# richarddurbin/modimizer

Measured on AMD Instinct MI355X. Metric: Gbp/s hashed+sketched (k=21,d=64), higher is better.
Workload: dtype u64; 1 GPU; BASELINE config 2: 10 Gbp synthetic ONT-like reads (log-normal N50 20 kb, 5% subs, 30x of a 333 Mbp genome), k=21 d=64 seed=17, seqhash scan + modset build (table bits 30); reads_per_gpu=598835, bases_per_gpu=10000000000, modimizers_per_gpu=156043826, modset_entries=102967436, k=21, d=64, table_bits=30, parallelism=reads sharded x1, modset per GPU

## Files before the change

### include/modgpu.h

```cpp
#ifndef MODGPU_H
#define MODGPU_H

#include <stdio.h>
#include <stdint.h>
#include <stdbool.h>
#include <stddef.h>

#if defined (MODGPU_WITH_REFERENCE_HEADERS) || defined (MS_MINOR)
#ifdef __cplusplus
extern "C" {
#endif
void mgSeqhashDestroy (Seqhash *sh) ;
void mgSeqhashRCiteratorDestroy (SeqhashRCiterator *si) ;
#ifdef __cplusplus
}
#endif
#else
#include "modgpu_compat.h"
#endif

#ifdef __cplusplus
extern "C" {
#endif


typedef enum {
  MG_OK = 0,
  MG_ERR_NO_DEVICE = 1,
  MG_ERR_HIP = 2,
  MG_ERR_ARG = 3,
  MG_ERR_CAPACITY = 4,
  MG_ERR_NOMEM = 5
} MgStatus ;

const char *mgLastError (void) ;
int  mgDeviceCount (void) ;
MgStatus mgSetDevice (int device) ;
const char *mgVersion (void) ;
const char *mgSourceHash (void) ;

U64 *mgIterScanHost (const Seqhash *sh, const char *s, int len) ;
void mgReloadKnobs (void) ;
int  mgIterHostBelow (int below) ;

MgStatus mgDeviceAlloc (void **dptr, size_t bytes) ;
MgStatus mgDeviceFree (void *dptr) ;
MgStatus mgMemcpyH2D (void *dst, const void *src, size_t bytes, void *stream) ;
MgStatus mgMemcpyD2H (void *dst, const void *src, size_t bytes, void *stream) ;
MgStatus mgMemsetD (void *dst, int byte, size_t bytes, void *stream) ;
MgStatus mgStreamSynchronize (void *stream) ;
MgStatus mgCopyD2HBig (void *hostDst, const void *devSrc, size_t bytes) ;
MgStatus mgCopyH2DBig (void *devDst, const void *hostSrc, size_t bytes) ;

#define MG_PACK_PAD 8
size_t   mgPackedWords (U64 nBases) ;
void     mgPackHost (const char *bases, U64 nBases, U32 *words) ;
MgStatus mgPackDevice (const U8 *dBases, U64 nBases, U32 *dWords, void *stream) ;
MgStatus mgUnpackDevice (const U32 *dWords, U64 nBases, U8 *dBases, void *stream) ;
MgStatus mgUploadPack (const char *bases, U64 nBases, U32 *dPacked, void *stream) ;

#define MG_POS_MASK 0x7fffffffu
#define MG_FWD_BIT  0x80000000u
size_t   mgScanWorkBytes (U64 totalBases, U32 nReads, U64 capacity) ;
MgStatus seqhashScanBatchDevice (const Seqhash *sh, const U32 *dPacked, U64 totalBases,
                                 const U64 *dReadOffsets, U32 nReads,
                                 U64 *dKmer, U32 *dPosF, U32 *dReadId, U64 capacity,
                                 U64 *dCount, void *dWork, void *stream) ;

int64_t seqhashScanBatch (const Seqhash *sh, const char *bases, const int64_t *readOffsets, int nReads,
                          U64 **kmer, int **pos, bool **isF, int64_t **survStart) ;

MgStatus seqhashMinimizerBatchDevice (const Seqhash *sh, const U32 *dPacked, U64 totalBases,
                                      const U64 *dReadOffsets, U32 nReads,
                                      U64 *dHash, U32 *dPosF, U64 *dReadStart, U64 capacity, U64 *n, void *stream) ;
int64_t seqhashMinimizerBatch (const Seqhash *sh, const char *bases, const int64_t *readOffsets, int nReads,
                               U64 **hash, int **pos, bool **isF, int64_t **start) ;

MgStatus modsetAddBatchDevice (Modset *ms, const U64 *dKmer, U64 n, U32 *dIndexOut, int withDepth, void *stream) ;
MgStatus modsetFindBatchDevice (Modset *ms, const U64 *dKmer, U64 n, U32 *dIndexOut, void *stream) ;

MgStatus modsetSyncToHost (Modset *ms, int wantIndex) ;
int      mgXferThreadCount (void) ;
MgStatus mgModsetDeviceRelease (Modset *ms) ;
void     mgModsetHostChanged (Modset *ms) ;
MgStatus mgModsetClear (Modset *ms, void *stream) ;

U64 mgModsetDeviceSlots (Modset *ms) ;

MgStatus mgTableCheckLayout (Modset *ms, U64 *out6) ;
MgStatus mgTableDiag (Modset *ms, U64 *out9) ;

MgStatus modsetDepthHistogramDevice (Modset *ms, U64 *dHist65536, void *stream) ;

MgStatus mgAddReadsDevice (Modset *ms, const U32 *dPacked, U64 totalBases,
                           const U64 *dReadOffsets, U32 nReads, U64 *nHash, void *stream) ;
MgStatus mgQueryReadsDevice (Modset *ms, const U32 *dPacked, U64 totalBases,
                             const U64 *dReadOffsets, U32 nReads,
                             U32 *dSeedIndex, U32 *dSeedPosF, U32 *dSeedRead, U64 capacity,
                             U64 *nSeeds, void *stream) ;

MgStatus mgQueryReadsDeviceAsync (Modset *ms, const U32 *dPacked, U64 totalBases, const U64 *dReadOffsets, U32 nReads,
                                  U32 *dSeedIndex, U32 *dSeedPosF, U32 *dSeedRead, U64 capacity, void **ticket, void *stream) ;
MgStatus mgQueryReadsDeviceWait (void *ticket, U64 *nSeeds, void *stream) ;

MgStatus mgInsertReadsDevice (Modset *ms, const U32 *dPacked, U64 totalBases,
                              const U64 *dReadOffsets, U32 nReads,
                              U32 *dSeedIndex, U32 *dSeedPosF, U32 *dSeedRead, U64 capacity,
                              U64 *nSeeds, void *stream) ;

bool mgModsetMergeArrays (Modset *ms1, U64 *value2, U16 *depth2, U8 *info2, U32 n2) ;
bool mgModsetMergeDeviceArrays (Modset *ms1, const U64 *dValue2, const U16 *dDepth2, const U8 *dInfo2, U32 n2) ;

typedef struct MgComm MgComm ;
MgStatus mgCommInitAll (MgComm **comms , int nDev, const int *devices ) ;
MgStatus mgCommGetUniqueId (void *id128) ;
MgStatus mgCommInitRank (MgComm **comm, int nRanks, int rank, const void *id128, int device) ;
int      mgCommRank (const MgComm *c) ;
int      mgCommSize (const MgComm *c) ;
void     mgCommDestroy (MgComm *c) ;
MgStatus mgHistogramAllReduce (Modset *ms, U64 *hist65536, MgComm *c) ;
MgStatus mgDepthAllReduce (Modset *ms, MgComm *c) ;
MgStatus mgModsetMergeRankOrder (Modset *ms, MgComm *c, int root) ;

int64_t mgAddSequenceBatch (Modset *ms, const char *bases, const int64_t *readOffsets, int nReads) ;
void    mgDepthHistogram (Modset *ms, FILE *f) ;
int     mgAddSequences (Modset *ms, const char *bases, const int64_t *readOffsets, int nReads, FILE *out) ;
void    mgModsetWriteText (Modset *ms, FILE *f) ;

typedef struct {
  Modset *ms ;
  U32 size ;
  U32 max ;
  U32 *index, *offset, *id ;
  U32 *depth ;
  U32 *rev, *loc ;
  int nSeq ;
  char **names ;
  U32 *len ;
} MgReference ;
MgReference *mgReferenceCreate (Modset *ms, U32 size) ;
void mgReferenceDestroy (MgReference *ref) ;
int  mgReferenceRead (MgReference *ref, const char *bases, const int64_t *offsets, int nSeq,
                      const char **names, bool isAdd, FILE *out) ;
void mgReferenceWrite (MgReference *ref, const char *root) ;
FILE *mgGzipOpenWrite (const char *name) ;
FILE *mgGzipOpenRead (const char *name) ;
FILE *mgFzOpen (const char *name, const char *mode) ;
MgReference *mgReferenceLoad (const char *root) ;
int  mgQueryProcess (MgReference *ref, const char *bases, const int64_t *offsets, int nReads,
                     const char **names, FILE *out) ;
void mgSetVerbose (int on) ;

typedef struct {
  Modset *ms ;
  int nReads, capReads ;
  int *len, *nHit, *nMiss ;
  int (*nCopy)[4] ;
  U64 *hitStart ;
  U32 *hit ; U16 *dx ;
  U64 totHit, capHit ;
  U64 *invStart ;
  U32 *invSpace ;
} MgReadset ;
MgReadset *mgReadsetCreate (Modset *ms) ;
void mgReadsetDestroy (MgReadset *rs) ;
int  mgReadsetRead (MgReadset *rs, const char *bases, const int64_t *offsets, int nReads) ;
int  mgReadsetFileRead (MgReadset *rs, const char *filename) ;
void mgReadsetStats (MgReadset *rs, FILE *out) ;
void mgReadsetWrite (MgReadset *rs, const char *root) ;
MgReadset *mgReadsetLoad (const char *root) ;
int  mgReadsetCleanMods (MgReadset *rs, FILE *out) ;
int  mgReadsetCleanModsPath (void) ;
int  mgReadsetProperties (MgReadset *rs, FILE *out) ;
int  mgReadsetPropertiesPath (void) ;

typedef struct {
  Modset *ms ;
  int len ;
  int *pos ;
  bool *isF ;
  int ownsMs ;
} MgRepRef ;
MgRepRef *mgRepRefCreate (const char *seqFile, const char *modFile, FILE *err) ;
MgRepRef *mgRepRefFromArrays (Modset *ms, const char *bases, int64_t len, FILE *err) ;
void mgRepRefDestroy (MgRepRef *ref) ;

typedef struct MgRepRun MgRepRun ;
typedef struct {
  int nRead, nBad, nGood ;
  int *n, *seqF, *seqR ;
  bool *bad, *isF ;
  U32 max ;
  int *modN, *modNPre ;
  int *goodI, *goodLen ;
  U64 *hitStart ;
  int *hitK, *hitX ;
  int nMod, nDup, tDup, minMax ;
} MgRepResult ;
void mgRepResultFree (MgRepResult *res) ;
MgRepRun *mgRepRunBegin (MgRepRef *ref, Modset *ms) ;
int  mgRepRunAdd (MgRepRun *run, const char *bases, const int64_t *offsets, int nReads, FILE *out) ;
int  mgRepRunFinish (MgRepRun *run, FILE *err, MgRepResult *res) ;
int  mgRepAnalyze3File (MgRepRef *ref, const char *seqFile, const char *modFile, FILE *out, FILE *err, MgRepResult *res) ;
int  mgRepPath (void) ;

typedef struct MgSeqReader MgSeqReader ;
typedef struct { char *bases ; int64_t *offsets ; char **names ; int nSeq ; int64_t total ; int isFastq ; int64_t basesCap ; } MgSeqBatch ;
MgSeqReader *mgSeqOpen (const char *filename) ;
int  mgSeqNextBatch (MgSeqReader *r, int64_t maxBases, MgSeqBatch *out) ;
void mgSeqBatchFree (MgSeqBatch *b) ;
void mgSeqClose (MgSeqReader *r) ;
void mgSeqReleaseBuffers (void) ;
void mgReleaseBuffers (void) ;
int  mgTextParseFileDevice (const char *filename, char **bases, int64_t **offsets, int64_t *nSeq) ;
int  mgAddSequenceFile (Modset *ms, const char *filename, FILE *out) ;
int  mgReferenceFastaRead (MgReference *ref, const char *filename, bool isAdd, FILE *out) ;
int  mgQueryFile (MgReference *ref, const char *filename, FILE *out) ;
int  mgReportDepths (Modset *ms, Modset **others, int nOthers, FILE *f) ;
int  mgRefPaint (Modset *ms, const char *bases, const int64_t *offsets, int nSeq, const char **names, FILE *out) ;
int  mgRefPaintFile (Modset *ms, const char *filename, FILE *out) ;
int     mgModsetWriteTextDevice (Modset *ms, FILE *f) ;
Modset *mgModsetReadText (const char *filename) ;
int     mgModsetReadTextPath (void) ;
int  mgFormatF2 (char *buf64, double x) ;

MgStatus mgSynthGenome (U32 *dPacked, U64 nBases, U64 seed, void *stream) ;
MgStatus mgSynthReads (const U32 *dGenomePacked, U64 genomeBases,
                       const U64 *dReadStart, const U64 *dReadOffsets, const U8 *dStrand, U32 nReads,
                       U64 totalBases, double errRate, U64 seed, U32 *dPackedOut, void *stream) ;

void     mgProfileEnable (int on) ;
void     mgProfileOnly (int kernelId) ;
void     mgProfileReset (void) ;
int      mgProfileKernels (void) ;
MgStatus mgProfileGet (int id, const char **name, double *totalMs, U64 *launches) ;

#ifdef __cplusplus
}
#endif
#endif
```

### modimizer_amd/__init__.py

```python
import contextlib
import ctypes as C
import os
import subprocess

import numpy as np

_HERE = os.path.dirname(os.path.abspath(__file__))
LIB_PATH = os.environ.get("MODGPU_LIB") or os.path.join(_HERE, "libmodgpu.so")
CSRC = os.path.join(_HERE, "csrc")

U64P = C.POINTER(C.c_uint64)
U32P = C.POINTER(C.c_uint32)

MG_POS_MASK = 0x7FFFFFFF
MG_FWD_BIT = 0x80000000


class Seqhash(C.Structure):
    _fields_ = [("seed", C.c_int), ("k", C.c_int), ("w", C.c_int), ("mask", C.c_uint64),
                ("shift1", C.c_int), ("shift2", C.c_int), ("factor1", C.c_uint64),
                ("factor2", C.c_uint64), ("patternRC", C.c_uint64 * 4)]


class SeqhashRCiterator(C.Structure):
    _fields_ = [("sh", C.POINTER(Seqhash)), ("s", C.c_void_p), ("sEnd", C.c_void_p),
                ("h", C.c_uint64), ("hRC", C.c_uint64), ("hashBuf", C.c_void_p), ("fBuf", C.c_void_p),
                ("base", C.c_int), ("iStart", C.c_int), ("iMin", C.c_int), ("isDone", C.c_bool)]


class Modset(C.Structure):
    _fields_ = [("hasher", C.POINTER(Seqhash)), ("tableBits", C.c_int), ("size", C.c_uint32),
                ("tableSize", C.c_uint64), ("tableMask", C.c_uint64), ("index", U32P),
                ("value", U64P), ("depth", C.POINTER(C.c_uint16)), ("info", C.POINTER(C.c_uint8)),
                ("max", C.c_uint32)]


class MgReference(C.Structure):
    _fields_ = [("ms", C.POINTER(Modset)), ("size", C.c_uint32), ("max", C.c_uint32),
                ("index", U32P), ("offset", U32P), ("id", U32P), ("depth", U32P), ("rev", U32P), ("loc", U32P),
                ("nSeq", C.c_int), ("names", C.POINTER(C.c_char_p)), ("len", U32P)]


class MgReadset(C.Structure):
    _fields_ = [("ms", C.POINTER(Modset)), ("nReads", C.c_int), ("capReads", C.c_int),
                ("len", C.POINTER(C.c_int)), ("nHit", C.POINTER(C.c_int)), ("nMiss", C.POINTER(C.c_int)),
                ("nCopy", C.POINTER(C.c_int * 4)), ("hitStart", U64P), ("hit", U32P), ("dx", C.POINTER(C.c_uint16)),
                ("totHit", C.c_uint64), ("capHit", C.c_uint64), ("invStart", U64P), ("invSpace", U32P)]


class MgRepRef(C.Structure):
    _fields_ = [("ms", C.POINTER(Modset)), ("len", C.c_int), ("pos", C.POINTER(C.c_int)), ("isF", C.POINTER(C.c_bool)), ("ownsMs", C.c_int)]


class MgRepResult(C.Structure):
    _fields_ = [("nRead", C.c_int), ("nBad", C.c_int), ("nGood", C.c_int),
                ("n", C.POINTER(C.c_int)), ("seqF", C.POINTER(C.c_int)), ("seqR", C.POINTER(C.c_int)),
                ("bad", C.POINTER(C.c_bool)), ("isF", C.POINTER(C.c_bool)), ("max", C.c_uint32),
                ("modN", C.POINTER(C.c_int)), ("modNPre", C.POINTER(C.c_int)),
                ("goodI", C.POINTER(C.c_int)), ("goodLen", C.POINTER(C.c_int)), ("hitStart", U64P),
                ("hitK", C.POINTER(C.c_int)), ("hitX", C.POINTER(C.c_int)),
                ("nMod", C.c_int), ("nDup", C.c_int), ("tDup", C.c_int), ("minMax", C.c_int)]


class MgSeqBatch(C.Structure):
    _fields_ = [("bases", C.POINTER(C.c_int8)), ("offsets", C.POINTER(C.c_int64)), ("names", C.POINTER(C.c_char_p)),
                ("nSeq", C.c_int), ("total", C.c_int64), ("isFastq", C.c_int), ("basesCap", C.c_int64)]


EXPORTS = [
    "seqhashCreate", "seqhashWrite", "seqhashRead", "seqhashReport", "modRCiterator", "modRCnext",
    "minimizerRCiterator", "minimizerRCnext", "seqString", "mgSeqhashDestroy", "mgSeqhashRCiteratorDestroy",
    "modsetCreate", "modsetDestroy", "modsetWrite", "modsetRead", "modsetIndexFind", "modsetSummary",
    "modsetPack", "modsetDepthPrune", "modsetMerge",
    "mgLastError", "mgDeviceCount", "mgSetDevice", "mgVersion", "mgSourceHash", "mgDeviceAlloc", "mgDeviceFree",
    "mgMemcpyH2D", "mgMemcpyD2H", "mgMemsetD", "mgStreamSynchronize",
    "mgPackedWords", "mgPackHost", "mgPackDevice", "mgUnpackDevice", "mgUploadPack",
    "mgScanWorkBytes", "seqhashScanBatchDevice", "seqhashScanBatch", "seqhashMinimizerBatchDevice", "seqhashMinimizerBatch",
    "modsetAddBatchDevice", "modsetFindBatchDevice", "modsetSyncToHost", "mgXferThreadCount", "mgCopyD2HBig", "mgCopyH2DBig", "mgModsetDeviceRelease",
    "mgModsetHostChanged", "modsetDepthHistogramDevice", "mgTableCheckLayout", "mgTableDiag", "mgAddReadsDevice", "mgQueryReadsDevice", "mgQueryReadsDeviceAsync", "mgQueryReadsDeviceWait",
    "mgAddSequenceBatch", "mgDepthHistogram", "mgSynthGenome", "mgSynthReads",
    "mgInsertReadsDevice", "mgAddSequences", "mgModsetWriteText", "mgReferenceCreate", "mgReferenceDestroy",
    "mgReferenceRead", "mgQueryProcess", "mgReferenceWrite", "mgGzipOpenWrite", "mgFzOpen", "mgGzipOpenRead", "mgReferenceLoad",
    "mgCommInitAll", "mgCommGetUniqueId", "mgCommInitRank", "mgCommRank", "mgCommSize", "mgCommDestroy", "mgHistogramAllReduce", "mgDepthAllReduce", "mgModsetMergeRankOrder",
    "mgReadsetCreate", "mgReadsetDestroy", "mgReadsetRead", "mgReadsetFileRead", "mgReadsetStats", "mgReadsetWrite", "mgReadsetLoad",
    "mgReadsetCleanMods", "mgReadsetCleanModsPath", "mgReadsetProperties", "mgReadsetPropertiesPath",
    "mgRepRefCreate", "mgRepRefFromArrays", "mgRepRefDestroy", "mgRepRunBegin", "mgRepRunAdd", "mgRepRunFinish", "mgRepResultFree", "mgRepAnalyze3File", "mgRepPath",
    "mgSeqOpen", "mgSeqNextBatch", "mgSeqBatchFree", "mgSeqClose", "mgSeqReleaseBuffers", "mgReleaseBuffers", "mgTextParseFileDevice", "mgAddSequenceFile", "mgReferenceFastaRead", "mgQueryFile",
    "mgReportDepths", "mgRefPaint", "mgRefPaintFile", "mgModsetWriteTextDevice", "mgModsetReadText", "mgModsetReadTextPath",
    "mgIterScanHost", "mgIterHostBelow", "mgReloadKnobs", "mgFormatF2", "mgModsetMergeArrays", "mgModsetMergeDeviceArrays", "mgModsetClear", "mgModsetDeviceSlots", "mgSetVerbose", "mgProfileEnable", "mgProfileOnly", "mgProfileReset", "mgProfileKernels", "mgProfileGet",
]


@contextlib.contextmanager
def knobs(**kv):
    old = {}
    for k, v in kv.items():
        name = "MODGPU_" + k
        old[name] = os.environ.get(name)
        if v is None:
            os.environ.pop(name, None)
        else:
            os.environ[name] = str(v)
    lib().mgReloadKnobs()
    try:
        yield
    finally:
        for name, v in old.items():
            if v is None:
                os.environ.pop(name, None)
            else:
                os.environ[name] = v
        lib().mgReloadKnobs()


def source_hash():
    import hashlib
    names = sorted(f for f in os.listdir(CSRC) if f.endswith((".hip", ".c", ".h"))) + ["Makefile", "../../include/modgpu.h", "../../include/modgpu_compat.h"]
    inc = os.path.join(_HERE, "..", "include")
    path = lambda n: os.path.join(inc, os.path.basename(n)) if n.startswith("../") else os.path.join(CSRC, n)
    listing = "".join("%s  %s\n" % (hashlib.sha256(open(path(n), "rb").read()).hexdigest(), n) for n in names)
    return hashlib.sha256(listing.encode()).hexdigest()[:16]


def binary_hash(path=None):
    import re
    try:
        m = re.search(rb"MODGPU_SRC_HASH=([0-9a-f]{16})", open(path or LIB_PATH, "rb").read())
    except OSError:
        return None
    return m.group(1).decode() if m else None


def build(force=False):
    import fcntl
    if os.environ.get("MODGPU_LIB"):
        return LIB_PATH
    def make_if_stale():
        if force or binary_hash() != source_hash():
            subprocess.check_call(["make", "-C", CSRC, "-j8", "-s"] + (["-B"] if force else []))
            if binary_hash() != source_hash():
                raise RuntimeError("libmodgpu.so does not carry the hash of its sources after make: %s != %s" % (binary_hash(), source_hash()))
    try:
        lk = open(os.path.join(CSRC, ".build.lock"), "w")
    except OSError:
        make_if_stale()
        return LIB_PATH
    with lk:
        fcntl.flock(lk, fcntl.LOCK_EX)
        make_if_stale()
    return LIB_PATH


_lib = None


def lib():
    global _lib
    if _lib is not None:
        return _lib
    if os.environ.get("MODGPU_NO_TORCH", "0") != "1":
        try:
            import torch
        except Exception:
            pass
    build()
    L = C.CDLL(LIB_PATH, mode=C.RTLD_GLOBAL)
    if not os.environ.get("MODGPU_LIB"):
        L.mgSourceHash.restype = C.c_char_p
        if L.mgSourceHash().decode() != source_hash():
            raise RuntimeError("the loaded libmodgpu.so was not built from the sources in this tree")
    vp, u64, u32, i32, i64 = C.c_void_p, C.c_uint64, C.c_uint32, C.c_int, C.c_int64
    SH, MS, IT = C.POINTER(Seqhash), C.POINTER(Modset), C.POINTER(SeqhashRCiterator)

    def sig(name, res, *args):
        if os.environ.get("MODGPU_LIB") and not hasattr(L, name):
            return
        f = getattr(L, name); f.restype = res; f.argtypes = list(args)
    sig("seqhashCreate", SH, i32, i32, i32)
    sig("seqhashWrite", None, SH, vp); sig("seqhashRead", SH, vp); sig("seqhashReport", None, SH, vp)
    sig("modRCiterator", IT, SH, vp, i32)
    sig("modRCnext", C.c_bool, IT, U64P, C.POINTER(i32), C.POINTER(C.c_bool))
    sig("minimizerRCiterator", IT, SH, vp, i32)
    sig("mgIterScanHost", vp, SH, vp, i32); sig("mgIterHostBelow", i32, i32); sig("mgReloadKnobs", None)
    sig("mgFormatF2", i32, C.c_char_p, C.c_double)
    sig("minimizerRCnext", C.c_bool, IT, U64P, C.POINTER(i32), C.POINTER(C.c_bool))
    sig("seqString", C.c_char_p, u64, i32)
    sig("mgSeqhashDestroy", None, SH); sig("mgSeqhashRCiteratorDestroy", None, IT)
    sig("modsetCreate", MS, SH, i32, u32); sig("modsetDestroy", None, MS)
    sig("modsetWrite", None, MS, vp); sig("modsetRead", MS, vp)
    sig("modsetIndexFind", u32, MS, u64, i32); sig("modsetSummary", None, MS, vp)
    sig("modsetPack", C.c_bool, MS); sig("modsetDepthPrune", None, MS, i32, i32)
    sig("modsetMerge", C.c_bool, MS, MS)
    sig("mgLastError", C.c_char_p); sig("mgDeviceCount", i32); sig("mgSetDevice", i32, i32)
    sig("mgVersion", C.c_char_p)
    sig("mgSourceHash", C.c_char_p)
    sig("mgDeviceAlloc", i32, C.POINTER(vp), C.c_size_t); sig("mgDeviceFree", i32, vp)
    sig("mgMemcpyH2D", i32, vp, vp, C.c_size_t, vp); sig("mgMemcpyD2H", i32, vp, vp, C.c_size_t, vp)
    sig("mgMemsetD", i32, vp, i32, C.c_size_t, vp); sig("mgStreamSynchronize", i32, vp)
    sig("mgPackedWords", C.c_size_t, u64); sig("mgPackHost", None, vp, u64, vp)
    sig("mgUploadPack", i32, vp, u64, vp, vp); sig("mgPackDevice", i32, vp, u64, vp, vp); sig("mgUnpackDevice", i32, vp, u64, vp, vp)
    sig("mgScanWorkBytes", C.c_size_t, u64, u32, u64)
    sig("seqhashScanBatchDevice", i32, SH, vp, u64, vp, u32, vp, vp, vp, u64, vp, vp, vp)
    sig("seqhashScanBatch", i64, SH, vp, vp, i32, C.POINTER(vp), C.POINTER(vp), C.POINTER(vp), C.POINTER(vp))
    sig("seqhashMinimizerBatchDevice", i32, SH, vp, u64, vp, u32, vp, vp, vp, u64, U64P, vp)
    sig("seqhashMinimizerBatch", i64, SH, vp, vp, i32, C.POINTER(vp), C.POINTER(vp), C.POINTER(vp), C.POINTER(vp))
    sig("modsetAddBatchDevice", i32, MS, vp, u64, vp, i32, vp)
    sig("modsetFindBatchDevice", i32, MS, vp, u64, vp, vp)
    sig("modsetSyncToHost", i32, MS, i32); sig("mgXferThreadCount", i32); sig("mgCopyD2HBig", i32, vp, vp, C.c_size_t); sig("mgCopyH2DBig", i32, vp, vp, C.c_size_t); sig("mgModsetDeviceRelease", i32, MS)
    sig("mgModsetHostChanged", None, MS)
    sig("modsetDepthHistogramDevice", i32, MS, vp, vp); sig("mgTableCheckLayout", i32, MS, U64P); sig("mgTableDiag", i32, MS, U64P)
    sig("mgAddReadsDevice", i32, MS, vp, u64, vp, u32, U64P, vp)
    sig("mgQueryReadsDevice", i32, MS, vp, u64, vp, u32, vp, vp, vp, u64, U64P, vp)
    sig("mgQueryReadsDeviceAsync", i32, MS, vp, u64, vp, u32, vp, vp, vp, u64, C.POINTER(vp), vp); sig("mgQueryReadsDeviceWait", i32, vp, U64P, vp)
    sig("mgAddSequenceBatch", i64, MS, vp, vp, i32); sig("mgDepthHistogram", None, MS, vp)
    sig("mgSynthGenome", i32, vp, u64, u64, vp)
    sig("mgSynthReads", i32, vp, u64, vp, vp, vp, u32, u64, C.c_double, u64, vp, vp)
    sig("mgInsertReadsDevice", i32, MS, vp, u64, vp, u32, vp, vp, vp, u64, U64P, vp)
    sig("mgAddSequences", i32, MS, vp, vp, i32, vp); sig("mgModsetWriteText", None, MS, vp)
    sig("mgReferenceCreate", vp, MS, u32); sig("mgReferenceDestroy", None, vp)
    sig("mgReferenceRead", i32, vp, vp, vp, i32, C.POINTER(C.c_char_p), C.c_bool, vp)
    sig("mgQueryProcess", i32, vp, vp, vp, i32, C.POINTER(C.c_char_p), vp)
    RS = C.POINTER(MgReadset)
    sig("mgReadsetCreate", RS, MS); sig("mgReadsetDestroy", None, RS)
    sig("mgReadsetRead", i32, RS, vp, vp, i32); sig("mgReadsetFileRead", i32, RS, C.c_char_p)
    sig("mgReadsetStats", None, RS, vp); sig("mgReadsetWrite", None, RS, C.c_char_p); sig("mgReadsetLoad", RS, C.c_char_p)
    sig("mgReadsetCleanMods", i32, RS, vp); sig("mgReadsetCleanModsPath", i32); sig("mgReadsetProperties", i32, RS, vp); sig("mgReadsetPropertiesPath", i32)
    RR, RES = C.POINTER(MgRepRef), C.POINTER(MgRepResult)
    sig("mgRepRefCreate", RR, C.c_char_p, C.c_char_p, vp); sig("mgRepRefFromArrays", RR, MS, vp, i64, vp); sig("mgRepRefDestroy", None, RR)
    sig("mgRepRunBegin", vp, RR, MS); sig("mgRepRunAdd", i32, vp, vp, vp, i32, vp); sig("mgRepRunFinish", i32, vp, vp, RES); sig("mgRepResultFree", None, RES)
    sig("mgRepAnalyze3File", i32, RR, C.c_char_p, C.c_char_p, vp, vp, RES); sig("mgRepPath", i32)
    sig("mgSeqOpen", vp, C.c_char_p); sig("mgSeqNextBatch", i32, vp, C.c_int64, C.POINTER(MgSeqBatch))
    sig("mgSeqBatchFree", None, C.POINTER(MgSeqBatch)); sig("mgSeqClose", None, vp); sig("mgSeqReleaseBuffers", None); sig("mgReleaseBuffers", None)
    sig("mgTextParseFileDevice", i32, C.c_char_p, C.POINTER(vp), C.POINTER(vp), C.POINTER(i64))
    sig("mgAddSequenceFile", i32, MS, C.c_char_p, vp); sig("mgReferenceFastaRead", i32, vp, C.c_char_p, C.c_bool, vp)
    sig("mgQueryFile", i32, vp, C.c_char_p, vp)
    sig("mgReportDepths", i32, MS, C.POINTER(MS), i32, vp)
    sig("mgRefPaint", i32, MS, vp, vp, i32, C.POINTER(C.c_char_p), vp); sig("mgRefPaintFile", i32, MS, C.c_char_p, vp)
    sig("mgModsetWriteTextDevice", i32, MS, vp); sig("mgModsetReadText", MS, C.c_char_p); sig("mgModsetReadTextPath", i32)
    sig("mgReferenceWrite", None, vp, C.c_char_p); sig("mgGzipOpenWrite", vp, C.c_char_p); sig("mgGzipOpenRead", vp, C.c_char_p); sig("mgFzOpen", vp, C.c_char_p, C.c_char_p);
    sig("mgCommInitAll", i32, C.POINTER(vp), i32, C.POINTER(i32)); sig("mgCommGetUniqueId", i32, vp); sig("mgCommInitRank", i32, C.POINTER(vp), i32, i32, vp, i32)
    sig("mgCommRank", i32, vp); sig("mgCommSize", i32, vp); sig("mgCommDestroy", None, vp)
    sig("mgHistogramAllReduce", i32, MS, vp, vp); sig("mgDepthAllReduce", i32, MS, vp); sig("mgModsetMergeRankOrder", i32, MS, vp, i32)
    sig("mgReferenceLoad", C.POINTER(MgReference), C.c_char_p)
    sig("mgModsetMergeArrays", C.c_bool, MS, vp, vp, vp, u32)
    sig("mgModsetMergeDeviceArrays", C.c_bool, MS, vp, vp, vp, u32)
    sig("mgModsetClear", i32, MS, vp); sig("mgModsetDeviceSlots", u64, MS); sig("mgSetVerbose", None, i32)
    sig("mgProfileEnable", None, i32); sig("mgProfileOnly", None, i32); sig("mgProfileReset", None); sig("mgProfileKernels", i32)
    sig("mgProfileGet", i32, i32, C.POINTER(C.c_char_p), C.POINTER(C.c_double), U64P)
    _lib = L
    return L


class ModgpuError(RuntimeError):
    pass


def check(status):
    if status != 0:
        raise ModgpuError("libmodgpu status %d: %s" % (status, lib().mgLastError().decode()))


_libc = C.CDLL(None)
_libc.free.argtypes = [C.c_void_p]
_libc.fopen.restype = C.c_void_p
_libc.fopen.argtypes = [C.c_char_p, C.c_char_p]
_libc.fclose.argtypes = [C.c_void_p]


class CFile:

    def __init__(self, path, mode="w"):
        self.f = _libc.fopen(path.encode(), mode.encode())
        if not self.f:
            raise OSError("cannot open " + path)

    def __enter__(self):
        return C.c_void_p(self.f)

    def __exit__(self, *a):
        _libc.fclose(self.f)



def seqhashCreate(k, w, seed=17):
    if k < 1 or k >= 32:
        raise ValueError("seqhash k %d must be between 1 and 32" % k)
    if w < 1:
        raise ValueError("seqhash w %d must be positive" % w)
    return lib().seqhashCreate(k, w, seed)


def modsetCreate(sh, bits, size=0):
    if bits < 20 or bits > 34:
        raise ValueError("table bits %d must be between 20 and 34" % bits)
    if size >= (1 << bits) >> 2:
        raise ValueError("Modset size %u is too big for %d bits" % (size, bits))
    return lib().modsetCreate(sh, bits, size)


def iterate(sh, bases, minimizer=False):
    L = lib()
    bases = np.ascontiguousarray(bases, dtype=np.uint8)
    mk, nx = (L.minimizerRCiterator, L.minimizerRCnext) if minimizer else (L.modRCiterator, L.modRCnext)
    it = mk(sh, bases.ctypes.data, len(bases))
    u = C.c_uint64(); p = C.c_int(); f = C.c_bool()
    ks, ps, fs = [], [], []
    while nx(it, C.byref(u), C.byref(p), C.byref(f)):
        ks.append(u.value); ps.append(p.value); fs.append(int(f.value))
    L.mgSeqhashRCiteratorDestroy(it)
    return np.array(ks, np.uint64), np.array(ps, np.int32), np.array(fs, np.uint8)


def scan_batch(sh, bases, offsets):
    L = lib()
    bases = np.ascontiguousarray(bases, dtype=np.uint8)
    offsets = np.ascontiguousarray(offsets, dtype=np.int64)
    n_reads = len(offsets) - 1
    pk, pp, pf, ps = C.c_void_p(), C.c_void_p(), C.c_void_p(), C.c_void_p()
    n = L.seqhashScanBatch(sh, bases.ctypes.data, offsets.ctypes.data, n_reads,
                           C.byref(pk), C.byref(pp), C.byref(pf), C.byref(ps))
    if n < 0:
        raise ModgpuError("seqhashScanBatch failed: " + L.mgLastError().decode())

    def take(ptr, ctype, count, dtype):
        a = np.ctypeslib.as_array(C.cast(ptr, C.POINTER(ctype)), (max(count, 1),))[:count].astype(dtype, copy=True)
        _libc.free(ptr)
        return a
    kmer = take(pk, C.c_uint64, n, np.uint64)
    pos = take(pp, C.c_int, n, np.int32)
    isf = take(pf, C.c_bool, n, np.uint8)
    st = take(ps, C.c_int64, n_reads + 1, np.int64)
    return kmer, pos, isf, st


def minimizer_batch(sh, bases, offsets):
    L = lib()
    bases = np.ascontiguousarray(bases, dtype=np.uint8)
    offsets = np.ascontiguousarray(offsets, dtype=np.int64)
    n_reads = len(offsets) - 1
    pk, pp, pf, ps = C.c_void_p(), C.c_void_p(), C.c_void_p(), C.c_void_p()
    n = L.seqhashMinimizerBatch(sh, bases.ctypes.data, offsets.ctypes.data, n_reads,
                                C.byref(pk), C.byref(pp), C.byref(pf), C.byref(ps))
    if n < 0:
        raise ModgpuError("seqhashMinimizerBatch failed: " + L.mgLastError().decode())

    def take(ptr, ctype, count, dtype):
        a = np.ctypeslib.as_array(C.cast(ptr, C.POINTER(ctype)), (max(count, 1),))[:count].astype(dtype, copy=True)
        _libc.free(ptr)
        return a
    return (take(pk, C.c_uint64, n, np.uint64), take(pp, C.c_int, n, np.int32), take(pf, C.c_bool, n, np.uint8),
            take(ps, C.c_int64, n_reads + 1, np.int64))


class DeviceBuffer:

    def __init__(self, nbytes):
        self.ptr = C.c_void_p()
        self.nbytes = int(nbytes)
        check(lib().mgDeviceAlloc(C.byref(self.ptr), self.nbytes))

    @classmethod
    def from_numpy(cls, arr):
        arr = np.ascontiguousarray(arr)
# ... 173 lines not shown
```

### modimizer_amd/csrc/mg_api.hip

```cpp
#include <stdarg.h>
#include <stdlib.h>
#include <string.h>
#include <mutex>
#include <unordered_map>
#include "mg_common.h"
#include "mg_internal.h"
#include "mg_xfer.h"


static thread_local char gErr[512] = "";

void mgSetError (const char *fmt, ...)
{ va_list ap; va_start (ap, fmt); vsnprintf (gErr, sizeof (gErr), fmt, ap); va_end (ap); }

extern "C" const char *mgLastError (void) { return gErr; }

MgStatus mgHipFail (hipError_t e, const char *what)
{ mgSetError ("HIP error %d (%s) in %s", (int) e, hipGetErrorString (e), what); return MG_ERR_HIP; }

extern "C" int mgDeviceCount (void)
{ int n = 0; if (hipGetDeviceCount (&n) != hipSuccess) { (void) hipGetLastError (); return 0; } return n; }

MgStatus mgEnsureDevice (void)
{
// ... 703 lines not shown
static MgStatus mgAddChunk (Modset *ms, MgDev *d, const U64 *dKmer, U64 n, U32 *dIndexOut, int withDepth,
                            void *scratch, hipStream_t st, const MgHistReq *counted = 0, const MgSegSrc *segSrc = 0)
{
  MgTable &t = d->t;
  MgStatus s;
  MG_HIP (hipMemsetAsync (t.counters, 0, 16, st));
  if ((s = mgTableAdd (&t, dKmer, n, withDepth, scratch, st, counted, segSrc))) return s;
  volatile U64 *c = d->hPin;
  MG_HIP (hipMemcpyAsync (d->hPin, t.counters, 16, hipMemcpyDeviceToHost, st));
  MG_HIP (hipStreamSynchronize (st));
  U64 newMax = (U64) t.max + c[0];
  if (c[1] || newMax >= t.size)
    {
      if ((s = mgTableRollback (&t, st))) return s;
      mgSetError ("hashTableSize %u is too small for %llu", t.size, (unsigned long long) newMax);
      return MG_ERR_CAPACITY;
    }
  t.max = (U32) newMax;
  ms->max = t.max;
  if (n >= 4096) t.newPct = (int) (c[0] * 100 / n);
  if (dIndexOut && (s = mgTableFind (&t, dKmer, n, dIndexOut, st))) return s;
  return MG_OK;
}

static MgStatus mgAddBatch (Modset *ms, MgDev *d, const U64 *dKmer, U64 n, U32 *dIndexOut, int withDepth,
                            bool arenaLive, hipStream_t st, const MgHistReq *counted, const MgSegSrc *segSrc)
{
  if (!n) return MG_OK;
  if (d->ticketsOut) { mgSetError ("a query batch of this modset is in flight (mgQueryReadsDeviceAsync without its mgQueryReadsDeviceWait)"); return MG_ERR_ARG; }
  U64 chunk = n < MG_ADD_CHUNK ? n : MG_ADD_CHUNK;
  MgStatus s = mgTableEnsure (&d->t, chunk, st); if (s) return s;
  size_t need = mgTableAddScratchBytes (&d->t, chunk) + 4096;
  if (!arenaLive)
    { if ((s = d->arena.reserve (need))) return s;
      d->arena.reset ();
    }
  else if (d->arena.bytes - d->arena.used < need)
    { mgSetError ("internal: arena too small for insert temporaries"); return MG_ERR_NOMEM; }
  void *scratch = d->arena.take (mgTableAddScratchBytes (&d->t, chunk));
  for (U64 off = 0 ; off < n && !s ; off += chunk)
    { U64 m = n - off < chunk ? n - off : chunk;
      if (off) s = mgTableEnsure (&d->t, m, st);
      if (!s) s = mgAddChunk (ms, d, dKmer + off, m, dIndexOut ? dIndexOut + off : 0, withDepth, scratch, st,
                              (counted && n <= chunk) ? counted : 0,
                              n <= chunk ? segSrc : 0);
    }
  return s;
}

extern "C" MgStatus modsetAddBatchDevice (Modset *ms, const U64 *dKmer, U64 n, U32 *dIndexOut, int withDepth, void *stream)
{
  hipStream_t st = (hipStream_t) stream;
  MgDev *d; MgStatus s = mgDevGet (ms, &d, st); if (s) return s;
  return mgAddBatch (ms, d, dKmer, n, dIndexOut, withDepth, false, st);
}

extern "C" MgStatus modsetFindBatchDevice (Modset *ms, const U64 *dKmer, U64 n, U32 *dIndexOut, void *stream)
{
  hipStream_t st = (hipStream_t) stream;
  MgDev *d; MgStatus s = mgDevGet (ms, &d, st); if (s) return s;
  d->t.loadPct = MG_LOOKUP_LOAD_PCT;
  if (d->t.slots && (s = mgTableEnsure (&d->t, 0, st))) return s;
  return mgTableFind (&d->t, dKmer, n, dIndexOut, st);
}

extern "C" MgStatus modsetSyncToHost (Modset *ms, int wantIndex)
{
  MgDev *d = mgDevLookup (ms);
  if (!d) return MG_OK;
  MgOnDevice here (d->device);
  MgTable &t = d->t;
  hipStream_t st = 0;
  MgStatus s;
  MG_HIP (hipDeviceSynchronize ());
  if (d->ticketsOut && (t.pendingDepth || (wantIndex && d->hostIndexMax < t.max)))
    { mgSetError ("a query batch of this modset is in flight (its scratch is what a sync would use)"); return MG_ERR_ARG; }
  if (t.max > t.syncedMax)
    { const U32 first = t.syncedMax + 1;
      if ((s = mgXferD2H (ms->value + first, t.value + first, (size_t) (t.max - first + 1) * sizeof (U64), MG_XFER_COPY))) return s;
      t.syncedMax = t.max;
    }
  ms->max = t.max;
  if (t.max && t.pendingDepth)
    {
      if ((s = d->arena.reserve (mgAl256 ((size_t) t.max * sizeof (U16)) + 4096))) return s;
      d->arena.reset ();
      U16 *dDelta = (U16 *) d->arena.take ((size_t) t.max * sizeof (U16));
      if ((s = mgTableExportDepth (&t, dDelta, st))) return s;
      MG_HIP (hipStreamSynchronize (st));
      if ((s = mgXferD2H (ms->depth + 1, dDelta, (size_t) t.max * sizeof (U16), MG_XFER_SATADD16))) return s;
    }
  if (wantIndex && d->hostIndexMax < t.max)
    { if ((s = d->arena.reserve (mgAl256 (ms->tableSize * sizeof (U32)) + 4096))) return s;
      d->arena.reset ();
      U32 *dIndex = (U32 *) d->arena.take (ms->tableSize * sizeof (U32));
      if ((s = mgTableReplayIndex (&t, mgMakeParams (ms->hasher), ms->tableBits, dIndex, st))) return s;
      MG_HIP (hipStreamSynchronize (st));
      if ((s = mgXferD2H (ms->index, dIndex, ms->tableSize * sizeof (U32), MG_XFER_COPY))) return s;
      d->hostIndexMax = t.max;
    }
  return MG_OK;
}

extern "C" MgStatus mgModsetAdoptDepthDevice (Modset *ms, const U16 *dDepth16)
{
  MgDev *d = mgDevLookup (ms);
  if (!d || !d->built) return MG_OK;
  MgTable &t = d->t;
  if (t.pendingDepth || t.max != ms->max) { mgModsetHostChanged (ms); return MG_OK; }
  MG_HIP (hipMemcpy (t.baseDepth, dDepth16, ((size_t) t.max + 1) * sizeof (U16), hipMemcpyDeviceToDevice));
  t.baseZero = false; t.liveHistValid = false;
  return MG_OK;
}

extern "C" int mgHookDeviceView (Modset *ms, const U64 **dValue1, const U16 **dDepth1, U32 *max)
{
  MgDev *d = mgDevLookup (ms);
  if (!d || !d->built || d->ticketsOut) return -1;
  { int cur = -1; if (hipGetDevice (&cur) != hipSuccess || cur != d->device) return -1; }
  if (hipDeviceSynchronize () != hipSuccess || mgFoldCounts (d, 0, ms)) return -1;
  *dValue1 = d->t.value + 1; *dDepth1 = d->t.baseDepth + 1; *max = d->t.max;
  return 0;
}

extern "C" int mgHookDeviceViewMake (Modset *ms, const U64 **dValue1, const U16 **dDepth1, U32 *max)
{
  MgDev *d; if (mgDevGet (ms, &d, 0)) return -1;
  return mgHookDeviceView (ms, dValue1, dDepth1, max);
}

extern "C" U64 mgModsetDeviceSlots (Modset *ms) { MgDev *d = mgDevLookup (ms); return d && d->built ? d->t.nSlots : 0; }

extern "C" MgStatus mgTableCheckLayout (Modset *ms, U64 *out6)
{
  MgDev *d; MgStatus s = mgDevGet (ms, &d, 0); if (s) return s;
  MgDevScratch scratch ("mgTableCheckLayout");
  U64 *dOut;
  if (scratch.get (&dOut, 4)) return MG_ERR_HIP;
  s = mgTableLayoutCheck (&d->t, dOut, 0);
  if (!s && (hipMemcpy (out6, dOut, 32, hipMemcpyDeviceToHost) || hipMemcpy (out6 + 4, d->t.counters + 4, 16, hipMemcpyDeviceToHost))) s = MG_ERR_HIP;
  return s;
}

extern "C" MgStatus mgTableDiag (Modset *ms, U64 *out9)
{
  memset (out9, 0, 9 * sizeof (U64));
  MgDev *d = mgDevLookup (ms);
  if (!d || !d->built) return MG_OK;
  out9[0] = (U64) d->t.log2NB; out9[1] = d->t.R;
  for (int i = 0 ; i < 7 ; ++i) out9[2 + i] = d->t.diag[i];
  return MG_OK;
}

extern "C" MgStatus modsetDepthHistogramDevice (Modset *ms, U64 *dHist, void *stream)
{
  hipStream_t st = (hipStream_t) stream;
  MgDev *d; MgStatus s = mgDevGet (ms, &d, st); if (s) return s;
  return mgTableHistogram (&d->t, dHist, st);
}


struct MgScanBufs { U64 *kmer; U32 *posF; U32 *rid; void *work; U64 *count; U64 cap; MgHistReq counted;
                    MgSegSrc seg; bool lazy; void *findScratch, *findScratch2; };

struct MgScanReq { const Seqhash *sh; const U32 *dPacked; U64 totalBases; const U64 *dReadOffsets; U32 nReads; bool wantPos; size_t extraPerSurvivor;
                   U32 *outPosF, *outRid; U64 outCap; bool lazy; };
static inline MgArena &mgArenaOf (MgDev *d, int slot) { return slot ? d->arena2 : d->arena; }
static inline U64 *mgCountPin (MgDev *d, int slot) { return d->hPin + 8 + 8 * slot; }

static MgStatus mgScanStart (MgDev *d, int slot, const MgScanReq &q, U64 cap, MgScanBufs *b, hipStream_t st)
{
  b->lazy = false; b->seg.nSegs = 0; b->seg.segKmer = 0; b->findScratch = 0; b->findScratch2 = 0;
  MgArena &ar = mgArenaOf (d, slot);
  const long fp = mgKnobs ()->findPath;
  const bool lookupHist = q.lazy && q.wantPos && !q.extraPerSurvivor && d->t.slots && fp != 'd'
                          && (fp == 'p' || fp == '2' || (cap >= ((U64) 1 << 24) && d->t.nSlots >= ((U64) 1 << 24) && d->t.log2NB > 9));
  const bool lookup2 = lookupHist && fp != 'p';
  MgHashParams p = mgMakeParams (q.sh);
  const size_t perS = 8 + (q.wantPos ? 8 : 0) + q.extraPerSurvivor;
  const size_t need = mgAl256 (cap * perS) + 4 * 4096 + 512 * MG_HIST_STRIDE * 4 + mgAl256 (mgScanWorkBytes (q.totalBases, q.nReads, cap))
                      + (q.extraPerSurvivor ? mgTableAddScratchBytes (&d->t, cap < MG_ADD_CHUNK ? cap : MG_ADD_CHUNK) + 8192 : 0) + 8 * 256
                      + (lookupHist ? mgTableFindPartScratchBytes (cap) + 8192 : 0) + (lookup2 ? mgTableFindPart2ScratchBytes (cap) + 8192 : 0);
  MgStatus s = ar.reserve (need); if (s) return s;
  ar.reset ();
  b->cap = cap;
  b->kmer = (U64 *) ar.take (cap * 8);
  const bool direct = q.wantPos && q.outPosF && q.outRid && q.outCap >= cap;
  b->posF = !q.wantPos ? 0 : (direct ? q.outPosF : (U32 *) ar.take (cap * 4));
  b->rid = !q.wantPos ? 0 : (direct ? q.outRid : (U32 *) ar.take (cap * 4));
  b->work = ar.take (mgScanWorkBytes (q.totalBases, q.nReads, cap));
  b->count = (U64 *) ar.take (8 * MG_COUNT_WORDS);
  b->counted.log2NB = 0; b->counted.kbits = 64; b->counted.binCount = 0; b->counted.hiB = 0;
  if (q.extraPerSurvivor || lookupHist)
    { b->counted.binCount = (U32 *) ar.take (512 * MG_HIST_STRIDE * sizeof (U32));
      b->counted.log2NB = d->t.log2NB; b->counted.kbits = d->t.kbits;
      if (lookupHist) b->counted.hiB = mgTableFindDigitBits (&d->t);
    }
  b->findScratch = lookupHist ? ar.take (mgTableFindPartScratchBytes (cap)) : 0;
  b->findScratch2 = lookup2 ? ar.take (mgTableFindPart2ScratchBytes (cap)) : 0;
  const bool lz = q.lazy && (q.wantPos ? q.extraPerSurvivor == 0 : b->counted.binCount != 0);
  if ((s = mgLaunchScan (p, q.dPacked, q.totalBases, q.dReadOffsets, q.nReads, b->kmer, b->posF, b->rid, cap, b->count, b->work, st,
                         b->counted.binCount ? &b->counted : 0, lz ? &b->seg : 0))) return s;
  b->lazy = lz;
  MG_HIP (hipMemcpyAsync (mgCountPin (d, slot), b->count, MG_COUNT_WORDS * sizeof (U64), hipMemcpyDeviceToHost, st));
  return MG_OK;
}
static MgStatus mgScanFinish (MgDev *d, int slot, const MgScanBufs *b, U64 *nOut, U64 *retryCap, hipStream_t st, hipEvent_t done = 0)
{
  volatile U64 *c = mgCountPin (d, slot);
  if (done) MG_HIP (hipEventSynchronize (done));
  else MG_HIP (hipStreamSynchronize (st));
  *retryCap = 0;
  if (!c[1] && c[0] <= b->cap) { *nOut = c[0]; return MG_OK; }
  *nOut = c[0]; *retryCap = c[3];
  return MG_OK;
}

static MgStatus mgScanIntoArena (MgDev *d, const Seqhash *sh, const U32 *dPacked, U64 totalBases,
                                 const U64 *dReadOffsets, U32 nReads, bool wantPos, size_t extraPerSurvivor,
                                 MgScanBufs *b, U64 *nOut, hipStream_t st,
                                 U32 *outPosF = 0, U32 *outRid = 0, U64 outCap = 0, bool lazy = false)
{
  if (d->ticketsOut) { mgSetError ("a query batch of this modset is in flight (mgQueryReadsDeviceAsync without its mgQueryReadsDeviceWait)"); return MG_ERR_ARG; }
  MgScanReq q = { sh, dPacked, totalBases, dReadOffsets, nReads, wantPos, extraPerSurvivor, outPosF, outRid, outCap, lazy };
  U64 cap = mgSurvivorGuess (sh, totalBases);
  if (extraPerSurvivor)
    {
      U64 expect = totalBases / (U64) (sh->w > 0 ? sh->w : 1) + 1;
      if (expect > MG_ADD_CHUNK) expect = MG_ADD_CHUNK;
      MgStatus es = mgTableEnsure (&d->t, expect, st); if (es) return es;
    }
  for (int attempt = 0 ; attempt < 3 ; ++attempt)
    { MgStatus s = mgScanStart (d, 0, q, cap, b, st); if (s) return s;
      U64 retry = 0;
      if ((s = mgScanFinish (d, 0, b, nOut, &retry, st))) return s;
      if (!retry) return MG_OK;
      cap = retry;
    }
  mgSetError ("scan capacity could not be established");
  return MG_ERR_CAPACITY;
}

extern "C" MgStatus mgAddReadsDevice (Modset *ms, const U32 *dPacked, U64 totalBases,
                                      const U64 *dReadOffsets, U32 nReads, U64 *nHash, void *stream)
{
  hipStream_t st = (hipStream_t) stream;
  MgDev *d; MgStatus s = mgDevGet (ms, &d, st); if (s) return s;
  if (nHash) *nHash = 0;
  if (!totalBases || !nReads) return MG_OK;
  MgScanBufs b; U64 n = 0;
  d->t.loadPct = 75;
  if ((s = mgScanIntoArena (d, ms->hasher, dPacked, totalBases, dReadOffsets, nReads, false, 4, &b, &n, st, 0, 0, 0, true))) return s;
  if (nHash) *nHash = n;
  if (!n) return MG_OK;
  if (b.lazy)
    { const U64 chunk = n < MG_ADD_CHUNK ? n : MG_ADD_CHUNK;
      if ((s = mgTableEnsure (&d->t, chunk, st))) return s;
      if (n <= MG_ADD_CHUNK && mgTableAddTakesSegments (&d->t, n, &b.counted))
        return mgAddBatch (ms, d, 0, n, 0, 1, true, st, &b.counted, &b.seg);
      if ((s = mgLaunchSegCompact (b.seg, b.kmer, b.cap, b.count, st))) return s;
    }
  return mgAddBatch (ms, d, b.kmer, n, 0, 1, true, st, &b.counted);
}

static MgStatus mgSeedReads (Modset *ms, const Seqhash *scanWith, int mode, const U32 *dPacked, U64 totalBases,
                             const U64 *dReadOffsets, U32 nReads,
                             U32 *dSeedIndex, U32 *dSeedPosF, U32 *dSeedRead, U64 capacity,
                             U64 *nSeeds, hipStream_t st)
{
  MgDev *d; MgStatus s = mgDevGet (ms, &d, st); if (s) return s;
  if (nSeeds) *nSeeds = 0;
  if (!scanWith) scanWith = ms->hasher;
  if ((s = mgCheckHasher (scanWith))) return s;
  if (scanWith->k != ms->hasher->k) { mgSetError ("a batch scanned with k %d cannot be looked up in a set of k %d", scanWith->k, ms->hasher->k); return MG_ERR_ARG; }
  if (!totalBases || !nReads) return MG_OK;
  MgScanBufs b; U64 n = 0;
  d->t.loadPct = MG_LOOKUP_LOAD_PCT;
  if (mode == 0 && d->t.slots && (s = mgTableEnsure (&d->t, 0, st))) return s;
  const int timing = mgKnobs ()->seedTiming == 1;
  struct timespec q0, q1, q2; if (timing) clock_gettime (CLOCK_MONOTONIC, &q0);
  if ((s = mgScanIntoArena (d, scanWith, dPacked, totalBases, dReadOffsets, nReads, true, mode ? 4 : 0, &b, &n, st,
                            dSeedPosF, dSeedRead, capacity, mode == 0))) return s;
  if (timing) clock_gettime (CLOCK_MONOTONIC, &q1);
  if (nSeeds) *nSeeds = n;
  if (n > capacity)
    { mgSetError ("%llu seeds exceed the caller's capacity %llu", (unsigned long long) n, (unsigned long long) capacity); return MG_ERR_CAPACITY; }
  if (mode == 0)
    { if (b.lazy && b.findScratch && mgTableFindTakesPartition (&d->t, n, &b.counted))
        s = mgTableFindPartitioned (&d->t, b.seg, n, &b.counted, dSeedIndex, b.kmer, b.findScratch, st, b.findScratch2);
      else s = b.lazy ? mgTableFindSegments (&d->t, b.seg, n, dSeedIndex, st) : mgTableFind (&d->t, b.kmer, n, dSeedIndex, st);
    }
  else s = mgAddBatch (ms, d, b.kmer, n, dSeedIndex, 0, true, st, &b.counted);
  if (s) return s;
  if (dSeedPosF && b.posF != dSeedPosF) MG_HIP (hipMemcpyAsync (dSeedPosF, b.posF, n * 4, hipMemcpyDeviceToDevice, st));
  if (dSeedRead && b.rid != dSeedRead) MG_HIP (hipMemcpyAsync (dSeedRead, b.rid, n * 4, hipMemcpyDeviceToDevice, st));
  MG_HIP (hipStreamSynchronize (st));
  if (timing)
    { clock_gettime (CLOCK_MONOTONIC, &q2);
      fprintf (stderr, "mgSeedReads: scan+count %.2f ms, lookup+sync %.2f ms\n", (q1.tv_sec - q0.tv_sec) * 1e3 + (q1.tv_nsec - q0.tv_nsec) * 1e-6,
               (q2.tv_sec - q1.tv_sec) * 1e3 + (q2.tv_nsec - q1.tv_nsec) * 1e-6);
    }
  return MG_OK;
}

extern "C" MgStatus mgQueryReadsDevice (Modset *ms, const U32 *dPacked, U64 totalBases,
                                        const U64 *dReadOffsets, U32 nReads,
// ... 349 lines not shown
```

### modimizer_amd/csrc/mg_common.h

```cpp
#ifndef MG_COMMON_H
#define MG_COMMON_H
#include "mg_knobs.h"

#include <hip/hip_runtime.h>
#include <stdint.h>
#include <time.h>
#include <algorithm>
#include <vector>
#include "modgpu.h"

#define MG_WAVE 64

#define MG_SCAN_THREADS   256
#define MG_POS_PER_THREAD 64
#define MG_TILE_BASES     (64 * MG_POS_PER_THREAD)
#define MG_TILE_WORDS     (MG_TILE_BASES / 16)

struct MgHashParams {
  U64 factor1;
  U64 mask;
  int k;
  int shift1;
  U32 d;
  int dShift;
// ... 45 lines not shown
  { if (cap >= want) return MG_OK;
    drop ();
    const hipError_t e = hipMalloc ((void **) &p, alloc * sizeof (T)); if (e != hipSuccess) { p = 0; return mgHipFail (e, what); }
    cap = alloc; return MG_OK;
  }
  void drop () { if (p) (void) hipFree (p); p = 0; cap = 0; }
};

#ifdef __HIPCC__
__device__ __forceinline__ bool mgDivisible (U64 x, const MgHashParams &p)
{
  if (x & (((U64) 1 << p.dShift) - 1)) return false;
  return ((x >> p.dShift) * p.dOddInv) <= p.dOddLim;
}

__device__ __forceinline__ bool mgDivisibleOdd32 (U64 h, const MgHashParams &p)
{
  const U32 lo = (U32) h, hi = (U32) (h >> 32);
  const U32 a = __builtin_amdgcn_alignbit (hi, lo, 24);
  const U32 t = __umul24 (a, p.c24) + (lo & 0xffffffu);
  return t * p.inv32 <= p.lim32;
}

__device__ __forceinline__ U32 mgRevComp16 (U32 w)
{
  const U32 x = __brev (w);
  return __builtin_amdgcn_bitop3_b32 (x << 1, x >> 1, 0x55555555u, 0x27);
}

__device__ __forceinline__ U64 mgRevComp (U64 f, int shift1)
{
  const U64 x = ((U64) mgRevComp16 ((U32) f) << 32) | mgRevComp16 ((U32) (f >> 32));
  return x >> shift1;
}
struct MgGeom { U32 R; int log2NB; int kbits; };
__device__ __forceinline__ U64 mgMixBits (U64 x, int b)
{
  if (b <= 32)
    { U32 y = (U32) x;
      const U32 m32 = b >= 32 ? ~0u : (((U32) 1 << b) - 1);
      const int h32 = (b + 1) >> 1;
      y ^= y >> h32; y = (y * 0xed558ccdu) & m32;
      y ^= y >> h32; y = (y * 0x1a85ec53u) & m32;
      y ^= y >> h32;
      return y;
    }
  const U64 mask = b >= 64 ? ~0ull : (((U64) 1 << b) - 1);
  const int h = (b + 1) >> 1;
  x ^= x >> h; x = (x * 0xff51afd7ed558ccdull) & mask;
  x ^= x >> h; x = (x * 0xc4ceb9fe1a85ec53ull) & mask;
  x ^= x >> h;
  return x;
}
#define MG_MIX_TOP 10
#define MG_MIX_MUL 0x9E3779B1u
__device__ __forceinline__ U64 mgMixK (U64 x, int b)
{
  if (b < 24) return mgMixBits (x, b);
  const int lb = b - MG_MIX_TOP;
  const U64 L = x & (((U64) 1 << lb) - 1), A = x >> lb;
  const U32 low = lb >= 32 ? (U32) L : ((U32) L & (((U32) 1 << lb) - 1));
  const U32 g = (low * MG_MIX_MUL) >> (32 - MG_MIX_TOP);
  return ((A ^ (U64) g) << lb) | mgMixBits (L, lb);
}
__device__ __forceinline__ U32 mgMixTopOfKmer (U64 x, int b, int hiB)
{
  const int lb = b - MG_MIX_TOP;
  const U32 low = lb >= 32 ? (U32) x : ((U32) x & (((U32) 1 << lb) - 1));
  return (U32) (x >> (b - hiB)) ^ ((low * MG_MIX_MUL) >> (32 - hiB));
}
__device__ __forceinline__ U32 mgBucketOfM (U64 m, const MgGeom &g)
{
  if (!g.log2NB) return 0u;
  const int s = g.kbits - g.log2NB;
  return s >= 0 ? (U32) (m >> s) : ((U32) m << (-s));
}
__device__ __forceinline__ U32 mgHomeOfM (U64 m, const MgGeom &g)
{
  U32 x = (U32) m;
  if (g.kbits >= 24) x ^= (U32) (m >> (g.kbits - MG_MIX_TOP)) * 0x9E5u;
  return __umulhi (x * 0x85EBCA6Bu, g.R);
}
__device__ __forceinline__ U32 mgNextSlot (U32 at, U32 R) { return at + 1 == R ? 0u : at + 1; }
#endif

static inline unsigned mgGrid (U64 n, unsigned per = 256, unsigned cap = 4096)
{ U64 b = (n + per - 1) / per; if (b > cap) b = cap; if (b < 1) b = 1; return (unsigned) b; }
static inline size_t mgAl256 (size_t n) { return (n + 255) & ~(size_t) 255; }
static inline double mgNowS (void) { struct timespec ts; clock_gettime (CLOCK_MONOTONIC, &ts); return ts.tv_sec + 1e-9 * ts.tv_nsec; }

static inline void mgPartSplit (int log2NB, int *hiB, int *loB)
{ if (log2NB <= 9) { *hiB = log2NB; *loB = 0; } else { *loB = log2NB / 2; *hiB = log2NB - *loB; } }

#define MG_HIST_STRIDE 16
struct MgHistReq { int log2NB; int kbits; U32 *binCount; int hiB; };

struct MgSegSrc { const U64 *segKmer; const U64 *segCount; const U64 *segStart; U64 segCap; U32 nSegs; };


MgStatus mgLaunchPack (const U8 *dBases, U64 nBases, U32 *dWords, hipStream_t st);
MgStatus mgLaunchUnpack (const U32 *dWords, U64 nBases, U8 *dBases, hipStream_t st);
MgStatus mgLaunchScan (const MgHashParams &p, const U32 *dPacked, U64 totalBases,
                       const U64 *dReadOffsets, U32 nReads,
                       U64 *dKmer, U32 *dPosF, U32 *dReadId, U64 capacity,
                       U64 *dCount, void *dWork, hipStream_t st, const MgHistReq *hist = 0, MgSegSrc *lazy = 0);

U64      mgScanTiles (U64 totalBases);
size_t   mgScanInfoBytes (U64 totalBases);
MgStatus mgScanPrepare (const U64 *dReadOffsets, U32 nReads, U64 totalBases, void *dInfo, hipStream_t st);
size_t   mgScanRangeWorkBytes (U64 nTilesRange, U64 capacity);
MgStatus mgLaunchSegCompact (const MgSegSrc &src, U64 *dKmer, U64 capacity, const U64 *dCount, hipStream_t st);
MgStatus mgLaunchScanRange (const MgHashParams &p, const U32 *dPacked, U64 totalBases,
                            const U64 *dReadOffsets, U32 nReads, const void *dInfo, U64 tile0, U64 tile1,
                            U64 *dKmer, U32 *dPosF, U32 *dReadId, U64 capacity,
                            U64 *dCount, void *dWork, hipStream_t st, const MgHistReq *hist = 0, MgSegSrc *lazy = 0);

U64      mgIterMaxBases (void);
U64      mgIterSegEntries (void);
MgStatus mgLaunchIterScan (const MgHashParams &p, const U32 *dPacked, U64 totalBases, const U64 *dReadOff,
                           U64 *dSegKmer, U32 *dSegPosF, U64 *out, U64 capEntries, U64 *flag, U64 seq, hipStream_t st);

MgStatus mgLaunchMinimizers (const MgHashParams &p, U32 w, const U32 *dPacked, const U64 *dReadOffsets, U32 nReads,
                             U64 *dHash, U32 *dPosF, U64 *dReadStart, U64 capacity, U64 *totalOut, hipStream_t st);

struct MgSlot { U64 key; U32 ord; U32 cnt; };
struct MgTable {
  MgSlot *slots; U64 nSlots;
  U64 capSlots;
  U32 capNB;
  U32 R; int log2NB;
  int kbits;
  U32 *occ;
  U64 *value;
  U16 *baseDepth;
  bool baseZero;
  U64 *liveHist;
  bool liveHistValid;
  U32 size;
  U32 max;
  U32 syncedMax;
  U64 *counters;
  bool pendingDepth;
  bool dirty;
  U64 *find8;
  U64 find8Cap;
  U64 find8Version, version;
  bool empty;
  U64 *pin;
  int newPct;
  int loadPct;
  int  maxLog2Slots;
  U32  wantR;
  U64  diag[7];
  int  tightPct;
};
MgStatus mgTableAlloc (MgTable *t, U64 slotsWanted, hipStream_t st);
MgStatus mgTableEnsure (MgTable *t, U64 nIncoming, hipStream_t st);
MgStatus mgTableRollback (MgTable *t, hipStream_t st);
MgStatus mgTableClean (MgTable *t, hipStream_t st);
void     mgTableForget (MgTable *t, hipStream_t st);
size_t   mgTableAddScratchBytes (const MgTable *t, U64 n);
bool     mgTableUseBuckets (const MgTable *t, U64 n);
MgStatus mgTableAdd (MgTable *t, const U64 *dKmer, U64 n, int withDepth, void *scratch, hipStream_t st,
                     const MgHistReq *counted = 0,
                     const MgSegSrc *segSrc = 0);
bool     mgTableAddTakesSegments (const MgTable *t, U64 n, const MgHistReq *counted);
MgStatus mgTableMarkOccupied (MgTable *t, const U64 *dKmer, U64 n, hipStream_t st);
MgStatus mgTableFind (MgTable *t, const U64 *dKmer, U64 n, U32 *dIndexOut, hipStream_t st);
MgStatus mgTableLayoutCheck (MgTable *t, U64 *dOut4, hipStream_t st);
enum { MG_DIAG_FIND_DIRECT = 0, MG_DIAG_FIND_PART1, MG_DIAG_FIND_PART2_16, MG_DIAG_FIND_PART2_8, MG_DIAG_PACK8, MG_DIAG_REHASH_BUCKET, MG_DIAG_REHASH_ATOMIC };
size_t   mgTableFindPartScratchBytes (U64 n);
int      mgTableFindDigitBits (const MgTable *t);
bool     mgTableFindTakesPartition (const MgTable *t, U64 n, const MgHistReq *counted);
size_t   mgTableFindPart2ScratchBytes (U64 n);
MgStatus mgTableFindPartitioned (MgTable *t, const MgSegSrc &segSrc, U64 n, const MgHistReq *counted, U32 *dIndexOut, U64 *el, void *scratch, hipStream_t st,
                                 void *scratch2 = 0);
MgStatus mgTableFindSegments (MgTable *t, const MgSegSrc &src, U64 n, U32 *dIndexOut, hipStream_t st);
MgStatus mgTableLoadHost (MgTable *t, const U64 *dValue, U32 first, U32 last, hipStream_t st);
MgStatus mgTableExportDepth (MgTable *t, U16 *dDelta, hipStream_t st);
MgStatus mgTableHistogram (MgTable *t, U64 *dHist, hipStream_t st);
MgStatus mgTableReplayIndex (MgTable *t, const MgHashParams &p, int tableBits, U32 *dIndex, hipStream_t st);
MgStatus mgTableMergeApply (const U32 *dIdx, const U16 *dDepth2, const U8 *dInfo2, U32 n2, U16 *dBaseDepth, U8 *dInfo1, hipStream_t st);
size_t   mgTablePruneScratchBytes (U32 n);
MgStatus mgTablePrune (MgTable *t, const U8 *dInfo, int lo, int hi, U64 *dNewValue, U16 *dNewDepth, U8 *dNewInfo,
                       void *scratch, hipStream_t st);
#define MG_COUNT_WORDS 4

MgStatus mgLaunchSynthGenome (U32 *dPacked, U64 nBases, U64 seed, hipStream_t st);
MgStatus mgLaunchSynthReads (const U32 *dGenome, U64 genomeBases, const U64 *dReadStart,
                             const U64 *dReadOffsets, const U8 *dStrand, U32 nReads, U64 totalBases,
                             double errRate, U64 seed, U32 *dOut, hipStream_t st);

#endif
```

### modimizer_amd/csrc/mg_knobs.c

```c
#define _GNU_SOURCE
#include <pthread.h>
#include <sched.h>
#include <stdio.h>
#include <stdlib.h>
#include <string.h>
#include <unistd.h>
#include <sys/mman.h>
#include "mg_knobs.h"

static MgKnobs gKnobs;
static pthread_once_t gOnce = PTHREAD_ONCE_INIT;

static long num (const char *name)
{ const char *e = getenv (name); return e && *e ? atol (e) : MG_KNOB_UNSET; }

static void readAll (void)
{
  MgKnobs k;
  const char *e = getenv ("MODGPU_TABLE_PATH");
  k.tablePath = e && *e ? (long) e[0] : MG_KNOB_UNSET;
  e = getenv ("MODGPU_FIND_PATH");
  k.findPath = e && *e ? (long) e[0] : MG_KNOB_UNSET;
  k.partPacked = num ("MODGPU_PART_PACKED");       k.partBig = num ("MODGPU_PART_BIG");
  k.addChunk = num ("MODGPU_ADD_CHUNK");           k.scanGrid = num ("MODGPU_SCAN_GRID");
  k.scanGeneric = num ("MODGPU_SCAN_GENERIC");     k.scanHist = num ("MODGPU_SCAN_HIST");
  k.scanDiv64 = num ("MODGPU_SCAN_DIV64");        k.minTiled = num ("MODGPU_MIN_TILED");
  k.minTile = num ("MODGPU_MIN_TILE");
  k.noSegmentInput = num ("MODGPU_NO_SEGMENT_INPUT");
  k.rankSliceShift = num ("MODGPU_RANK_SLICE_SHIFT");
  k.flagPolarity = num ("MODGPU_FLAG_POLARITY");   k.mergeSlots = num ("MODGPU_MERGE_SLOTS");
  k.mergePlace = num ("MODGPU_MERGE_PLACE");
  k.bucketR = num ("MODGPU_BUCKET_R");             k.bucketT = num ("MODGPU_BUCKET_T");
  e = getenv ("MODGPU_HOT_SPLIT");
  k.hotSplit = e && *e ? atol (e) : MG_KNOB_UNSET;
  { const char *c = e ? strchr (e, ',') : 0; k.hotChunk = c ? atol (c + 1) : MG_KNOB_UNSET; }
  k.noAvx2 = num ("MODGPU_NO_AVX2");               k.textHost = num ("MODGPU_TEXT_HOST");
  k.textWindowKb = num ("MODGPU_TEXT_WINDOW_KB");
  k.fileBatchMbp = num ("MODGPU_FILE_BATCH_MBP");  k.fileBatchBases = num ("MODGPU_FILE_BATCH_BASES");
  k.queryHostChain = num ("MODGPU_QUERY_HOST_CHAIN");
  k.iterHostBelow = num ("MODGPU_ITER_HOST_BELOW");
  k.readsetHost = num ("MODGPU_READSET_HOST");
  k.segSlack = num ("MODGPU_SEG_SLACK");
  k.partDigits = num ("MODGPU_PART_DIGITS");
  k.findBits = num ("MODGPU_FIND_BITS");
  k.scatterGrid = num ("MODGPU_SCATTER_GRID");     k.tableLoad = num ("MODGPU_TABLE_LOAD");
  k.tightLoad = num ("MODGPU_TIGHT_LOAD");         k.find8 = num ("MODGPU_FIND8");
  k.packThreads = num ("MODGPU_PACK_THREADS");     k.parseThreads = num ("MODGPU_PARSE_THREADS");
  k.xferThreads = num ("MODGPU_XFER_THREADS");       k.gzipThreads = num ("MODGPU_GZIP_THREADS");
  k.xferPieceKb = num ("MODGPU_XFER_PIECE_KB");      k.xferStreams = num ("MODGPU_XFER_STREAMS");
  k.seedTiming = num ("MODGPU_SEED_TIMING");       k.uploadTiming = num ("MODGPU_UPLOAD_TIMING");
  k.textTiming = num ("MODGPU_TEXT_TIMING");       k.parseTiming = getenv ("MODGPU_PARSE_TIMING") ? 1 : MG_KNOB_UNSET;
  k.scanDebug = num ("MODGPU_SCAN_DEBUG");         k.bucketDebug = num ("MODGPU_BUCKET_DEBUG");
  gKnobs = k;
}

const MgKnobs *mgKnobs (void) { pthread_once (&gOnce, readAll); return &gKnobs; }
void mgIterKnobsReloaded (void) __attribute__ ((weak));
void mgReloadKnobs (void) { pthread_once (&gOnce, readAll); readAll (); if (mgIterKnobsReloaded) mgIterKnobsReloaded (); }

static int gCpuBudget;
static pthread_once_t gCpuOnce = PTHREAD_ONCE_INIT;
static void cpuBudgetOnce (void)
{
  long v = sysconf (_SC_NPROCESSORS_ONLN);
  cpu_set_t set;
  if (sched_getaffinity (0, sizeof (set), &set) == 0 && CPU_COUNT (&set) < v) v = CPU_COUNT (&set);
  FILE *q = fopen ("/sys/fs/cgroup/cpu.max", "r");
  if (q)
    { char a[64]; long per = 0;
      if (fscanf (q, "%63s %ld", a, &per) == 2 && strcmp (a, "max") && per > 0) { const long c = (atol (a) + per - 1) / per; if (c < v) v = c; }
      fclose (q);
    }
  gCpuBudget = v < 1 ? 1 : (int) v;
}
int mgCpuBudget (void) { pthread_once (&gCpuOnce, cpuBudgetOnce); return gCpuBudget; }

void mgHugeHint (void *p, size_t n)
{
#ifdef MADV_HUGEPAGE
  if (p && n >= ((size_t) 8 << 20))
    { const size_t pg = 4096;
      char *a = (char *) (((size_t) p + pg - 1) & ~(pg - 1)), *e = (char *) (((size_t) p + n) & ~(pg - 1));
      if (e > a) (void) madvise (a, (size_t) (e - a), MADV_HUGEPAGE);
    }
#else
  (void) p; (void) n;
#endif
}
void *mgAllocBig (size_t n) { void *p = malloc (n ? n : 1); mgHugeHint (p, n); return p; }
```

### modimizer_amd/csrc/mg_knobs.h

```cpp
#ifndef MG_KNOBS_H
#define MG_KNOBS_H
#include <limits.h>
#ifdef __cplusplus
extern "C" {
#endif
#define MG_KNOB_UNSET LONG_MIN
typedef struct {
  long findPath;
  long tablePath;
  long partPacked;
  long partBig;
  long addChunk;
  long scanGrid;
  long scanGeneric;
  long minTile;
  long minTiled;
  long scanDiv64;
  long scanHist;
  long noSegmentInput;
  long rankSliceShift;
  long flagPolarity;
  long mergeSlots;
  long mergePlace;
  long bucketR, bucketT;
  long hotSplit, hotChunk;
  long noAvx2;
  long textHost;
  long textWindowKb;
  long fileBatchMbp;
  long fileBatchBases;
  long readsetHost;
  long queryHostChain;
  long iterHostBelow;
  long scatterGrid;
  long segSlack;
  long partDigits;
  long findBits;
  long tableLoad;
  long find8;
  long tightLoad;
  long packThreads;
  long parseThreads;
  long gzipThreads;
  long xferPieceKb;
  long xferStreams;
  long xferThreads;
  long seedTiming, uploadTiming, textTiming, parseTiming;
  long scanDebug, bucketDebug;
} MgKnobs;
const MgKnobs *mgKnobs (void);
void mgReloadKnobs (void);
int mgCpuBudget (void);
#include <stddef.h>
void mgHugeHint (void *p, size_t n);
void *mgAllocBig (size_t n);
#ifdef __cplusplus
}
#endif
#endif
```

### modimizer_amd/csrc/mg_table.hip

```cpp
#include <stdlib.h>
#include <string.h>
#include "mg_prefix.h"

#define MG_ASSIGNED 0x80000000u
#define MG_R_QUANTUM 64u
#ifdef MG_BUILD_PRIO
#define MG_BUILD_PRIO() __builtin_amdgcn_s_setprio (3)
#else
#define MG_BUILD_PRIO() do { } while (0)
#endif
#ifdef MG_ABLATE
#define MG_ABLATE_AND(x) && (x)
#else
#define MG_ABLATE_AND(x)
#endif
__device__ __forceinline__ U32 mgToken (U64 o) { return 0x7fffffffu - (U32) o; }
__device__ __forceinline__ bool mgIsAssigned (U32 v) { return (v & MG_ASSIGNED) != 0; }
__device__ __forceinline__ U64 mgKeyOf (const uint4 &v) { return ((U64) v.y << 32) | v.x; }
__device__ __forceinline__ U32 mgIndexOf (U32 ordWord) { return mgIsAssigned (ordWord) ? (ordWord & ~MG_ASSIGNED) : 0; }
__device__ __forceinline__ bool mgLiveEntry (const uint4 &v, U32 keepMax) { return (v.x | v.y) && mgIsAssigned (v.z) && (v.z & ~MG_ASSIGNED) <= keepMax; }




// ... 562 lines not shown
      __syncthreads ();
    }
  if (t < nBins)
    { U64 st = segStart[seg] + (sS[t] - c);
      binStart[(U64) seg * nBins + t] = st;
      cursor[((U64) seg * nBins + t) * cstride] = st;
    }
  if (seg == nSeg - 1 && t == 0) binStart[(U64) nSeg * nBins] = n;
}

#ifndef MG_PART_THREADS
#define MG_PART_THREADS 1024
#endif
#define MG_PART_SUB_BIG (2 * MG_PART_SUB)
#define MG_PART_BIG_BINS 256
template <int INMODE, int SUB>
__device__ __forceinline__ void mgPartFetch (U64 *km, U32 *tk, const U64 *__restrict__ kIn, const U32 *__restrict__ tIn,
                                             const MgSegSrc &src, const MgSubSeg *__restrict__ subSeg, U64 sub, U64 subHi, int tid)
{
  if (INMODE == MG_EL_SEG)
    { const U32 wave = (U32) __builtin_amdgcn_readfirstlane (tid >> 6);
      const int lane = tid & 63;
      MgSegCursor cur;
      mgSegCursorFrom (subSeg, sub / MG_PART_SUB, &cur);
#pragma unroll
      for (int j = 0 ; j < SUB / MG_PART_THREADS ; ++j)
        { const U64 o0 = sub + (U64) j * MG_PART_THREADS + (U64) wave * 64;
          if (o0 >= subHi) break;
          mgSegCursorSeek (src, &cur, o0);
          const U64 i = o0 + (U64) lane;
          const U64 *at = mgSegAddr (src, cur, i, o0 + 63 < subHi ? o0 + 63 : subHi - 1);
          if (i < subHi) km[j] = *at;
        }
      return;
    }
#pragma unroll
  for (int j = 0 ; j < SUB / MG_PART_THREADS ; ++j)
    { U64 i = sub + (U64) j * MG_PART_THREADS + tid;
      if (i < subHi) { km[j] = kIn[i]; if (INMODE == MG_EL_WIDE) tk[j] = tIn[i]; }
    }
}

template <int INMODE, bool PACKOUT, int SUB>
__global__ __launch_bounds__ (MG_PART_THREADS)
void mgPartScatterKernel (const U64 *__restrict__ kIn, const U32 *__restrict__ tIn, const MgSegSrc src, const MgSubSeg *__restrict__ subSeg,
                          MgGeom g, MgPartFmt f, int shift, U32 nBins,
                          const U64 *__restrict__ segStart, const U32 *__restrict__ chunkBase, U32 nSeg, U32 chunkElems,
                          unsigned long long *__restrict__ cursor, U32 cstride, U64 *__restrict__ kOut, U32 *__restrict__ tOut,
                          unsigned long long *__restrict__ runTab, int runMode, unsigned char *__restrict__ dOut, int dShift, U32 dMask)
{
  MG_BUILD_PRIO ();
  constexpr bool WIDE = !PACKOUT;
  constexpr bool BIG = SUB > MG_PART_SUB;
  constexpr int PER = SUB / MG_PART_THREADS;
  constexpr int BINS = BIG ? MG_PART_BIG_BINS : MG_PART_MAXBINS;
  static_assert (!BIG || PACKOUT, "large sub-chunks: packed elements only");
  typedef typename std::conditional<BIG, unsigned char, unsigned short>::type Digit;
  __shared__ U64 stK[SUB];
  __shared__ U32 stT[WIDE ? SUB : 1];
  __shared__ Digit stB[SUB];
  __shared__ U32 sH[BINS], sOff[BINS];
  __shared__ unsigned long long sBase[BINS];
  __shared__ U32 sWave[MG_PART_THREADS / 64];
  const int tid = threadIdx.x, lane = tid & 63, wave = tid >> 6;
  const U64 remMask = f.remBits >= 64 ? ~0ull : (((U64) 1 << f.remBits) - 1);
  U32 c = blockIdx.x, seg; U64 lo, hi;
  bool have = mgChunkRange (segStart, chunkBase, nSeg, chunkElems, c, &seg, &lo, &hi);
  U64 sub = have ? lo : 0;
  U64 km[PER]; U32 tk[PER];
#pragma unroll
  for (int j = 0 ; j < PER ; ++j) { km[j] = 0; tk[j] = 0; }
  if (have)
    { const U64 subHi = sub + SUB < hi ? sub + SUB : hi;
      mgPartFetch<INMODE, SUB> (km, tk, kIn, tIn, src, subSeg, sub, subHi, tid);
    }
  while (have)
    { const U64 subHi = sub + SUB < hi ? sub + SUB : hi;
      const U32 cnt = (U32) (subHi - sub);
      U32 nc = c, nseg = seg; U64 nlo = lo, nhi = hi, nsub = sub + SUB; bool nhave = true;
      if (nsub >= hi) { nc = c + gridDim.x; nhave = mgChunkRange (segStart, chunkBase, nSeg, chunkElems, nc, &nseg, &nlo, &nhi); nsub = nlo; }
      for (U32 b = tid ; b < nBins ; b += MG_PART_THREADS) sH[b] = 0;
      __syncthreads ();
      U32 dr[PER];
#pragma unroll
      for (int j = 0 ; j < PER ; ++j)
        { U64 i = sub + (U64) j * MG_PART_THREADS + tid;
          dr[j] = 0xffffffffu;
          if (i < subHi)
            { constexpr bool FIRST = INMODE == MG_EL_DENSE || INMODE == MG_EL_SEG;
              if (FIRST)
                { km[j] = mgMixK (km[j], g.kbits); tk[j] = (U32) i; }
              U32 d = mgDigitOf<(FIRST ? MG_EL_WIDE : INMODE)> (km[j], g, f, shift, nBins - 1);
              dr[j] = (d << 16) | atomicAdd (&sH[d], 1u);
              if (FIRST && PACKOUT) km[j] = ((km[j] & remMask) << f.ordBits) | (U64) tk[j];
              if (INMODE == MG_EL_PACKED && runMode == 1) km[j] = ((km[j] >> f.ordBits) << f.ordBits) | i;
            }
        }
      __syncthreads ();
      unsigned long long base0 = 0, base1 = 0;
      { U32 c0 = (U32) (2 * tid) < nBins ? sH[2 * tid] : 0, c1 = (U32) (2 * tid + 1) < nBins ? sH[2 * tid + 1] : 0;
        const U32 pair = c0 + c1, incl = mgWaveInclusiveSum (pair);
        if (lane == 63) sWave[wave] = incl;
        __syncthreads ();
        U32 wb = 0;
#pragma unroll
        for (int w = 0 ; w < MG_PART_THREADS / 64 ; ++w) if (w < wave) wb += sWave[w];
        U32 ex = wb + incl - pair;
        if ((U32) (2 * tid) < nBins)
          { sOff[2 * tid] = ex;
            if (c0) base0 = atomicAdd (&cursor[((U64) seg * nBins + 2 * tid) * cstride], (unsigned long long) c0);
          }
        if ((U32) (2 * tid + 1) < nBins)
          { sOff[2 * tid + 1] = ex + c0;
            if (c1) base1 = atomicAdd (&cursor[((U64) seg * nBins + 2 * tid + 1) * cstride], (unsigned long long) c1);
          }
      }
      __syncthreads ();
#pragma unroll
      for (int j = 0 ; j < PER ; ++j)
        if (dr[j] != 0xffffffffu)
          { U32 d = dr[j] >> 16, p = sOff[d] + (dr[j] & 0xffffu);
            stK[p] = km[j]; if (WIDE) stT[p] = tk[j]; stB[p] = (Digit) d;
          }
      if ((U32) (2 * tid) < nBins) sBase[2 * tid] = base0;
      if ((U32) (2 * tid + 1) < nBins) sBase[2 * tid + 1] = base1;
      if (runTab)
        { const U64 row = (runMode == 1 ? 2 * (U64) c + (sub - lo) / SUB : sub / SUB) * nBins;
          if ((U32) (2 * tid) < nBins) runTab[row + 2 * tid] = base0 | ((unsigned long long) sH[2 * tid] << 40);
          if ((U32) (2 * tid + 1) < nBins) runTab[row + 2 * tid + 1] = base1 | ((unsigned long long) sH[2 * tid + 1] << 40);
        }
      if (nhave)
        { const U64 nsubHi = nsub + SUB < nhi ? nsub + SUB : nhi;
          mgPartFetch<INMODE, SUB> (km, tk, kIn, tIn, src, subSeg, nsub, nsubHi, tid);
        }
      __syncthreads ();
      for (U32 p = tid ; p < cnt ; p += MG_PART_THREADS)
        { U32 d = stB[p];
          U64 at = sBase[d] + (p - sOff[d]);
          kOut[at] = stK[p];
          if (WIDE) tOut[at] = stT[p];
          if (dOut) dOut[at] = (unsigned char) mgDigitOf<(PACKOUT ? MG_EL_PACKED : MG_EL_WIDE)> (stK[p], g, f, dShift, dMask);
        }
      __syncthreads ();
      c = nc; seg = nseg; lo = nlo; hi = nhi; sub = nsub; have = nhave;
    }
}



struct MgBucketArgs {
  MgSlot *slots; MgGeom g; U32 nBuckets;
  const U64 *bucketStart;
  U64 *pK; U32 *pT; U32 *pC;
  MgPartFmt f;
  U32 *uniqCount;
  U32 *occ;
  unsigned char *flags;
  const MgRankGrp *grp; U32 baseMax; U32 size;
  unsigned short *sliceOff;
  U32 nSlices; int sliceShift;
  int slotShift;
  int place;
  int markDup;
  int withDepth;
  U64 *counters;
  U32 hotSplit, hotChunk;
  U64 *hotItems; unsigned long long *hotCount;
  U32 *hotBuckets;
#ifdef MG_ABLATE
  int debug;
#endif
  unsigned long long *liveHist;
};

extern __shared__ __attribute__ ((aligned (16))) unsigned char mgDynLds[];

__device__ __forceinline__ U32 mgLdsClaim (unsigned long long *sKey, U32 R, U32 home, unsigned long long key)
{
  U32 at = home;
  for (U32 probes = 0 ; probes < R ; ++probes)
    { const unsigned long long cur = atomicCAS (&sKey[at], 0ull, key);
      if (cur == 0 || cur == key) return at;
      at = mgNextSlot (at, R);
    }
  return R;
}

#ifndef MG_BUCKET_PREFETCH
#define MG_BUCKET_PREFETCH 3
#endif
#ifndef MG_MERGE_PREFETCH
#define MG_MERGE_PREFETCH 2
#endif
#ifndef MG_HOT_DEPTH
#define MG_HOT_DEPTH 4
#endif
#define MG_PLACE_KEEP 4
#define MG_RANK_GROUPS 64
#define MG_SLOT_SHIFT 48
#define MG_DEDUP_PER 4
#define MG_DEDUP_PER_BIG 8
#define MG_LIVE_BINS 256

template <bool PACKED>
__device__ __forceinline__ void mgOccurrence (const MgBucketArgs &a, U32 b, U64 x, U32 t, U64 *m, U32 *ord)
{
  if (PACKED)
    { *ord = (U32) (x & (((U64) 1 << a.f.ordBits) - 1));
      *m = ((U64) (b >> a.f.loB) << a.f.remBits) | (x >> a.f.ordBits);
    }
  else { *m = x; *ord = t; }
}

__device__ __forceinline__ void mgDedupCount (const MgBucketArgs &a, U32 *sOrd, U32 *sCnt, U32 at, U32 ord)
{
  const U32 tok = mgToken (ord);
  if (a.markDup)
    { const U32 old = atomicMax (&sOrd[at], tok);
      const U32 loser = old > tok ? tok : old;
      if (loser MG_ABLATE_AND (!(a.debug & 1))) a.flags[0x7fffffffu - loser] = 0;
    }
  else atomicMax (&sOrd[at], tok);
  atomicAdd (&sCnt[at], 1u);
}
__device__ __forceinline__ U32 mgWavePrefixMax (U32 v)
{
#define MG_MAX_DPP(ctrl, rows) do { const U32 o_ = (U32) __builtin_amdgcn_update_dpp (0, (int) v, ctrl, rows, 0xf, false); v = o_ > v ? o_ : v; } while (0)
  MG_MAX_DPP (0x111, 0xf); MG_MAX_DPP (0x112, 0xf); MG_MAX_DPP (0x114, 0xf); MG_MAX_DPP (0x118, 0xf); MG_MAX_DPP (0x142, 0xa); MG_MAX_DPP (0x143, 0xc);
#undef MG_MAX_DPP
  return v;
}
__device__ __forceinline__ U32 mgWaveMax (U32 v) { return (U32) __builtin_amdgcn_readlane ((int) mgWavePrefixMax (v), 63); }
__device__ __forceinline__ void mgDedupCountWave (const MgBucketArgs &a, U32 *sOrd, U32 *sCnt, U32 R, bool live, U32 at, U32 ord)
{
  live = live && at < R;
  const U32 at0 = (U32) __builtin_amdgcn_readfirstlane ((int) at);
  const bool mine = live && at == at0;
  const U32 n = (U32) __popcll (__ballot (mine));
  if (n > 1)
    { const U32 tok = mgToken (ord);
      const U32 best = mgWaveMax (mine ? tok : 0u);
      if (mine)
        { if (tok == best)
            { const U32 old = atomicMax (&sOrd[at], tok);
              if (a.markDup) { const U32 loser = old > tok ? tok : old; if (loser) a.flags[0x7fffffffu - loser] = 0; }
              atomicAdd (&sCnt[at], n);
            }
          else if (a.markDup) a.flags[ord] = 0;
        }
      else if (live) mgDedupCount (a, sOrd, sCnt, at, ord);
    }
  else if (live) mgDedupCount (a, sOrd, sCnt, at, ord);
}

template <bool PACKED>
__device__ __forceinline__ void mgDedupRun (const MgBucketArgs &a, U32 b, unsigned long long *sKey, U32 *sOrd, U32 *sCnt,
                                            U32 R, U32 T, U32 tid, U64 from, U64 hi)
{
  for (U64 i0 = from ; i0 < hi ; i0 += (U64) MG_HOT_DEPTH * T)
    { U64 x[MG_HOT_DEPTH]; U32 tx[MG_HOT_DEPTH]; bool live[MG_HOT_DEPTH];
#pragma unroll
      for (int j = 0 ; j < MG_HOT_DEPTH ; ++j)
        { const U64 i = i0 + (U64) j * T + tid;
          live[j] = i < hi;
          x[j] = live[j] ? a.pK[i] : 0; tx[j] = (!PACKED && live[j]) ? a.pT[i] : 0;
        }
      const int kShift = PACKED ? a.f.ordBits : 0;
      const U64 x0 = mgUniform64 (x[0]); const U32 tx0 = (U32) __builtin_amdgcn_readfirstlane ((int) tx[0]);
      bool same = true;
#pragma unroll
      for (int j = 0 ; j < MG_HOT_DEPTH ; ++j) if (live[j] && (x[j] >> kShift) != (x0 >> kShift)) same = false;
      const bool first = __builtin_amdgcn_readfirstlane ((int) live[0]) != 0;
      bool done = false;
      if (first && __ballot (!same) == 0 MG_ABLATE_AND (!(a.debug & 6)))
        { U64 m; U32 o0; mgOccurrence<PACKED> (a, b, x0, tx0, &m, &o0);
          const U32 at = mgLdsClaim (sKey, R, mgHomeOfM (m, a.g), m + 1);
          if (at < R)
            { U32 tok[MG_HOT_DEPTH], tmax = 0, cnt = 0;
#pragma unroll
              for (int j = 0 ; j < MG_HOT_DEPTH ; ++j)
                { const U32 ord = PACKED ? (U32) (x[j] & (((U64) 1 << a.f.ordBits) - 1)) : tx[j];
                  tok[j] = live[j] ? mgToken (ord) : 0u;
                  if (tok[j] > tmax) tmax = tok[j];
                  cnt += live[j] ? 1u : 0u;
                }
              const U32 best = mgWaveMax (tmax);
              const U32 total = (U32) __builtin_amdgcn_readlane ((int) mgWaveInclusiveSum (cnt), 63);
              if (cnt && tmax == best)
                { const U32 old = atomicMax (&sOrd[at], best);
                  if (a.markDup) { const U32 loser = old > best ? best : old; if (loser) a.flags[0x7fffffffu - loser] = 0; }
                  atomicAdd (&sCnt[at], total);
                }
              if (a.markDup)
                {
#pragma unroll
                  for (int j = 0 ; j < MG_HOT_DEPTH ; ++j) if (live[j] && tok[j] != best) a.flags[0x7fffffffu - tok[j]] = 0;
                }
              done = true;
            }
        }
      if (!done)
        {
#pragma unroll
          for (int j = 0 ; j < MG_HOT_DEPTH ; ++j)
            { U64 m = 0; U32 ord = 0, at = R;
              if (live[j])
                { mgOccurrence<PACKED> (a, b, x[j], tx[j], &m, &ord);
#ifdef MG_ABLATE
                  if (a.debug & 4) { at = mgHomeOfM (m, a.g); sKey[at] = m + 1; } else
#endif
                  at = mgLdsClaim (sKey, R, mgHomeOfM (m, a.g), m + 1);
                  if (at == R) a.counters[1] = 1;
                }
#ifdef MG_ABLATE
              if (a.debug & 2) { if (live[j] && at < R) { sOrd[at] = mgToken (ord); sCnt[at] = 1; } continue; }
#endif
              mgDedupCountWave (a, sOrd, sCnt, R, live[j], at, ord);
            }
        }
    }
}

#define MG_HOT_SPLIT_DEFAULT 16384u
#define MG_HOT_CHUNK_DEFAULT 4096u
#define MG_HOT_MAXCHUNKS 1024u
__host__ __device__ __forceinline__ U64 mgHotChunkLen (U64 cnt, U32 minChunk)
{ const U64 L = (cnt + MG_HOT_MAXCHUNKS - 1) / MG_HOT_MAXCHUNKS; return L < minChunk ? minChunk : L; }

__global__ __launch_bounds__ (256)
void mgHotPlanKernel (const MgBucketArgs a)
{
  const U32 b = blockIdx.x * 256 + threadIdx.x;
  if (b >= a.nBuckets) return;
  const U64 cnt = a.bucketStart[b + 1] - a.bucketStart[b];
  if (cnt <= a.hotSplit) return;
  const U64 L = mgHotChunkLen (cnt, a.hotChunk);
  const U32 nCh = (U32) ((cnt + L - 1) / L);
  const U64 at = atomicAdd (a.hotCount, (unsigned long long) nCh);
  for (U32 j = 0 ; j < nCh ; ++j) a.hotItems[at + j] = ((U64) b << 32) | j;
  a.hotBuckets[atomicAdd (a.hotCount + 1, 1ull)] = b;
}

template <bool PACKED>
__global__ __launch_bounds__ (1024)
void mgHotReduceKernel (const MgBucketArgs a)
{
  const U32 R = a.g.R, T = blockDim.x, tid = threadIdx.x;
  unsigned long long *sKey = reinterpret_cast<unsigned long long *> (mgDynLds);
  U32 *sOrd = reinterpret_cast<U32 *> (mgDynLds + (size_t) R * 8);
  U32 *sCnt = sOrd + R;
  U32 *sN = sCnt + R;
  const U64 nItems = *a.hotCount;
  if (blockIdx.x >= nItems) return;
  for (U32 i = tid ; i < R ; i += T) { sKey[i] = 0; sOrd[i] = 0; sCnt[i] = 0; }
  if (tid == 0) sN[0] = 0;
  __syncthreads ();
  for (U64 w = blockIdx.x ; w < nItems ; w += gridDim.x)
    { const U64 item = a.hotItems[w];
      const U32 b = (U32) (item >> 32), j = (U32) item;
      const U64 lo = a.bucketStart[b], hi = a.bucketStart[b + 1];
      const U64 L = mgHotChunkLen (hi - lo, a.hotChunk);
      const U64 cs = lo + (U64) j * L, ce = cs + L < hi ? cs + L : hi;
      mgDedupRun<PACKED> (a, b, sKey, sOrd, sCnt, R, T, tid, cs, ce);
      __syncthreads ();
      for (U32 i = tid ; i < R ; i += T)
        { const unsigned long long key = sKey[i];
          if (key)
            { const U32 tok = sOrd[i], c = sCnt[i];
              sKey[i] = 0; sOrd[i] = 0; sCnt[i] = 0;
              const U32 at = atomicAdd (&sN[0], 1u);
              const U32 ord = 0x7fffffffu - tok;
              if (PACKED) a.pK[cs + at] = (((key - 1) & (((U64) 1 << a.f.remBits) - 1)) << a.f.ordBits) | ord;
              else { a.pK[cs + at] = key - 1; a.pT[cs + at] = ord; }
              a.pC[cs + at] = c;
            }
        }
      __syncthreads ();
      if (tid == 0) { const U32 nc = sN[0]; if (cs + nc < ce) a.pC[cs + nc] = 0; sN[0] = 0; }
      __syncthreads ();
    }
}

template <bool PACKED>
__device__ __forceinline__ void mgDedupHotBucket (const MgBucketArgs &a, U32 b, unsigned long long *sKey, U32 *sOrd, U32 *sCnt,
                                                  U32 R, U32 T, U32 tid, U64 lo, U64 hi)
{
  const U64 L = mgHotChunkLen (hi - lo, a.hotChunk);
  const U32 nCh = (U32) ((hi - lo + L - 1) / L);
  const U32 lane = tid & 63;
  for (U32 j = tid >> 6 ; j < nCh ; j += T >> 6)
    { const U64 cs = lo + (U64) j * L, ce = cs + L < hi ? cs + L : hi;
      for (U64 base = cs ; base < ce ; base += 64)
        { const U64 i = base + lane;
          const U32 c = i < ce ? a.pC[i] : 0u;
          const unsigned long long ended = __ballot (c == 0);
          const bool live = c != 0 && (ended == 0 || lane < (U32) __builtin_ctzll (ended));
          if (live)
            { U64 m; U32 ord;
              mgOccurrence<PACKED> (a, b, a.pK[i], PACKED ? 0u : a.pT[i], &m, &ord);
              const U32 at = mgLdsClaim (sKey, R, mgHomeOfM (m, a.g), m + 1);
              if (at == R) a.counters[1] = 1;
              else
                { const U32 tok = mgToken (ord);
                  const U32 old = atomicMax (&sOrd[at], tok);
                  if (a.markDup) { const U32 loser = old > tok ? tok : old; if (loser) a.flags[0x7fffffffu - loser] = 0; }
                  atomicAdd (&sCnt[at], c);
                }
            }
          if (ended) break;
        }
    }
}

template <bool PACKED, bool SLOT, int PER, bool HOT>
__global__ __launch_bounds__ (1024) __attribute__ ((amdgpu_waves_per_eu (PER == MG_DEDUP_PER ? 8 : 4)))
void mgBucketDedupKernel (const MgBucketArgs a, U32 bucketsPerBlock)
{
  MG_BUILD_PRIO ();
  const U32 R = a.g.R, T = blockDim.x, tid = threadIdx.x;
  unsigned long long *sKey = reinterpret_cast<unsigned long long *> (mgDynLds);
  U32 *sOrd = reinterpret_cast<U32 *> (mgDynLds + (size_t) R * 8);
  U32 *sCnt = sOrd + R;
  U32 *sGrp = sCnt + R;
  const U32 nGrp = a.nSlices + 1;
  U32 b = blockIdx.x * bucketsPerBlock, bEnd = b + bucketsPerBlock;
  U64 hotAt = blockIdx.x; const U64 nHot = HOT ? a.hotCount[1] : 0;
  if (HOT) { if (hotAt >= nHot) return; }
  else
    { if (bEnd > a.nBuckets) bEnd = a.nBuckets;
      if (b >= bEnd) return;
    }
  for (U32 i = tid ; i < R ; i += T) { sKey[i] = 0; sOrd[i] = 0; sCnt[i] = 0; }
  if (tid < MG_RANK_GROUPS) sGrp[tid] = 0;
  for ( ; ; )
  {
  if (HOT) { b = a.hotBuckets[hotAt]; bEnd = b + 1; }
  U64 lo = a.bucketStart[b], hi = a.bucketStart[b + 1];
  U32 occNow = a.occ[b];
  U64 ck[MG_BUCKET_PREFETCH]; U32 ct[MG_BUCKET_PREFETCH];
#pragma unroll
  for (int j = 0 ; j < MG_BUCKET_PREFETCH ; ++j)
    { U64 i = lo + (U64) j * T + tid; ck[j] = 0; ct[j] = 0; if (!HOT && i < hi) { ck[j] = __builtin_nontemporal_load (&a.pK[i]); if (!PACKED) ct[j] = __builtin_nontemporal_load (&a.pT[i]); } }
  __syncthreads ();
  for ( ; b < bEnd ; ++b)
    {
      U64 nlo = hi, nhi = hi;
      U64 nk[MG_BUCKET_PREFETCH]; U32 nt[MG_BUCKET_PREFETCH];
#pragma unroll
      for (int j = 0 ; j < MG_BUCKET_PREFETCH ; ++j) { nk[j] = 0; nt[j] = 0; }
      U32 occNext = 0;
      if (b + 1 < bEnd)
        { nhi = a.bucketStart[b + 2];
          occNext = a.occ[b + 1];
#pragma unroll
          for (int j = 0 ; j < MG_BUCKET_PREFETCH ; ++j)
            { U64 i = nlo + (U64) j * T + tid; if (i < nhi) { nk[j] = __builtin_nontemporal_load (&a.pK[i]); if (!PACKED) nt[j] = __builtin_nontemporal_load (&a.pT[i]); } }
        }
      if (hi == lo)
        { if (tid == 0) a.uniqCount[b] = 0;
          if (tid < nGrp + 1) a.sliceOff[(U64) b * (nGrp + 1) + tid] = 0;
        }
      else if (!HOT && hi - lo > a.hotSplit) { }
      else
        { if (occNow)
            { for (U32 i = tid ; i < R ; i += T)
                { uint4 v = *reinterpret_cast<const uint4 *> (&a.slots[(U64) b * R + i]);
                  sKey[i] = mgKeyOf (v); sOrd[i] = v.z;
                }
              __syncthreads ();
            }
          if (HOT) mgDedupHotBucket<PACKED> (a, b, sKey, sOrd, sCnt, R, T, tid, lo, hi);
          else
          {
#pragma unroll
          for (int j = 0 ; j < MG_BUCKET_PREFETCH ; ++j)
            if (lo + (U64) j * T + tid < hi)
              { U64 m; U32 ord; mgOccurrence<PACKED> (a, b, ck[j], ct[j], &m, &ord);
                U32 at;
#ifdef MG_ABLATE
                if (a.debug & 4) { at = mgHomeOfM (m, a.g); sKey[at] = m + 1; } else
#endif
                at = mgLdsClaim (sKey, R, mgHomeOfM (m, a.g), m + 1);
                if (at == R) a.counters[1] = 1;
#ifdef MG_ABLATE
                else if (a.debug & 2) { sOrd[at] = mgToken (ord); sCnt[at] = 1; }
#endif
                else { mgDedupCount (a, sOrd, sCnt, at, ord); }
              }
          mgDedupRun<PACKED> (a, b, sKey, sOrd, sCnt, R, T, tid, lo + (U64) MG_BUCKET_PREFETCH * T, hi);
          }
          __syncthreads ();
          unsigned long long rk[PER]; U32 rc[PER], ro[PER], rp[PER];
#pragma unroll
          for (int j = 0 ; j < PER ; ++j)
            { const U32 i = (U32) j * T + tid;
              rk[j] = 0; rc[j] = 0; ro[j] = 0; rp[j] = 0;
              if (i < R) rk[j] = sKey[i];
              if (rk[j])
                { rc[j] = sCnt[i]; ro[j] = sOrd[i];
                  sKey[i] = 0; sOrd[i] = 0; sCnt[i] = 0;
                  rk[j] = (rk[j] - 1) | (SLOT ? (unsigned long long) i << MG_SLOT_SHIFT : 0ull);
                  if (rc[j]) rp[j] = atomicAdd (&sGrp[mgIsAssigned (ro[j]) ? a.nSlices : ((0x7fffffffu - ro[j]) >> a.sliceShift)], 1u);
                }
            }
          __syncthreads ();
          const int lane = (int) (tid & 63);
          const U32 gv = (U32) lane < nGrp ? sGrp[lane] : 0;
          const U32 gIncl = mgWaveInclusiveSum (gv);
          const U32 gBase = gIncl - gv;
          const U32 total = (U32) __builtin_amdgcn_readlane ((int) gIncl, 63);
          if (tid < 64)
            { if ((U32) lane <= nGrp) a.sliceOff[(U64) b * (nGrp + 1) + lane] = (unsigned short) gBase;
              if (lane == 0) a.uniqCount[b] = total;
            }
#pragma unroll
          for (int j = 0 ; j < PER ; ++j)
            { const U32 grp = mgIsAssigned (ro[j]) ? a.nSlices : ((0x7fffffffu - ro[j]) >> a.sliceShift);
              const U32 at = (U32) __shfl ((int) gBase, (int) (rc[j] ? grp : 0)) + rp[j];
              if (rc[j]) { sKey[at] = rk[j]; sOrd[at] = ro[j]; sCnt[at] = rc[j]; }
            }
          __syncthreads ();
          if (tid < MG_RANK_GROUPS) sGrp[tid] = 0;
          for (U32 i = tid ; i < total ; i += T)
            { const U64 k = sKey[i]; const U32 ord = sOrd[i], c = sCnt[i];
              sKey[i] = 0; sOrd[i] = 0; sCnt[i] = 0;
              if (true MG_ABLATE_AND (!(a.debug & 8)))
                { __builtin_nontemporal_store (k, &a.pK[lo + i]); __builtin_nontemporal_store (ord, &a.pT[lo + i]); __builtin_nontemporal_store (c, &a.pC[lo + i]); }
              if (!a.markDup && !mgIsAssigned (ord) MG_ABLATE_AND (!(a.debug & 1))) a.flags[0x7fffffffu - ord] = 1;
            }
          __syncthreads ();
        }
      lo = nlo; hi = nhi; occNow = occNext;
#pragma unroll
      for (int j = 0 ; j < MG_BUCKET_PREFETCH ; ++j) { ck[j] = nk[j]; ct[j] = nt[j]; }
    }
  if (!HOT) break;
  hotAt += gridDim.x;
  if (hotAt >= nHot) break;
  }
}

__device__ __forceinline__ U32 mgPlaceStarts (U32 *cnt, unsigned short *sStart, int *sWave, U32 R, U32 T, U32 tid, U32 n)
{
  const U32 per = (R + 4 * T - 1) / (4 * T) * 4;
  const U32 j0 = tid * per, j1 = j0 + per < R ? j0 + per : R;
  U32 vS = 0; int vM = 0;
  for (U32 j = j0 ; j < j1 ; j += 4)
    { const uint4 c = *reinterpret_cast<const uint4 *> (&cnt[j]);
      int m = (int) j - (int) vS;               vM = m > vM ? m : vM; vS += c.x;
      m = (int) (j + 1) - (int) vS;             vM = m > vM ? m : vM; vS += c.y;
      m = (int) (j + 2) - (int) vS;             vM = m > vM ? m : vM; vS += c.z;
      m = (int) (j + 3) - (int) vS;             vM = m > vM ? m : vM; vS += c.w;
    }
  const int lane = (int) (tid & 63);
  const U32 wave = (U32) __builtin_amdgcn_readfirstlane ((int) (tid >> 6));
  const U32 inS = mgWaveInclusiveSum (vS), exS = inS - vS;
  const U32 inM = mgWavePrefixMax (vM > (int) exS ? (U32) vM - exS : 0u);
  if (lane == 63) { sWave[2 * wave] = (int) inS; sWave[2 * wave + 1] = (int) inM; }
  U32 exM = (U32) __shfl_up ((int) inM, 1);
  if (lane == 0) exM = 0;
  __syncthreads ();
  U32 wS = 0, wM = 0;
  if ((U32) lane < (T + 63) / 64) { wS = (U32) sWave[2 * lane]; wM = (U32) sWave[2 * lane + 1]; }
  const U32 wInS = mgWaveInclusiveSum (wS), wExS = wInS - wS;
  const U32 wInM = mgWavePrefixMax (wM > wExS ? wM - wExS : 0u);
  const int mAll = __builtin_amdgcn_readlane ((int) wInM, 63);
  U32 beforeS = 0, beforeM = 0;
  if (wave) { beforeS = (U32) __builtin_amdgcn_readlane ((int) wInS, (int) wave - 1); beforeM = (U32) __builtin_amdgcn_readlane ((int) wInM, (int) wave - 1); }
  { const U32 m = exM > beforeS ? exM - beforeS : 0u; beforeM = beforeM > m ? beforeM : m; beforeS += exS; }
  const int over = mAll + (int) n - (int) R;
  const U32 carry = over > 0 ? (U32) over : 0u;
  U32 c = beforeS; int e = beforeM > carry ? (int) beforeM : (int) carry;
  for (U32 j = j0 ; j < j1 ; j += 4)
    { const uint4 k = *reinterpret_cast<const uint4 *> (&cnt[j]);
      *reinterpret_cast<uint4 *> (&cnt[j]) = make_uint4 (0, 0, 0, 0);
      U32 s0, s1, s2, s3; int m;
      m = (int) j - (int) c;       e = m > e ? m : e; s0 = c + (U32) e; c += k.x;
      m = (int) (j + 1) - (int) c; e = m > e ? m : e; s1 = c + (U32) e; c += k.y;
      m = (int) (j + 2) - (int) c; e = m > e ? m : e; s2 = c + (U32) e; c += k.z;
      m = (int) (j + 3) - (int) c; e = m > e ? m : e; s3 = c + (U32) e; c += k.w;
      *reinterpret_cast<uint2 *> (&sStart[j]) = make_uint2 (s0 | (s1 << 16), s2 | (s3 << 16));
    }
  return carry;
}
static inline size_t mgMergeLdsBytes (U32 R) { return (size_t) R * 16 + 16 + MG_LIVE_BINS * 4 + 128 + (size_t) R * 2; }

template <int KEEP>
__global__ __launch_bounds__ (1024) __attribute__ ((amdgpu_waves_per_eu (8)))
void mgBucketMergeKernel (const MgBucketArgs a, U32 bucketsPerBlock)
{
  MG_BUILD_PRIO ();
  const U32 R = a.g.R, T = blockDim.x, tid = threadIdx.x;
  unsigned long long *sKey = reinterpret_cast<unsigned long long *> (mgDynLds);
  U32 *sOrd = reinterpret_cast<U32 *> (mgDynLds + (size_t) R * 8);
  U32 *sCnt = sOrd + R;
  U32 b = blockIdx.x * bucketsPerBlock, bEnd = b + bucketsPerBlock;
  if (bEnd > a.nBuckets) bEnd = a.nBuckets;
  if (b >= bEnd) return;
  for (U32 i = tid ; i < R ; i += T) { sKey[i] = 0; sOrd[i] = 0; sCnt[i] = 0; }
  U32 *sLive = sCnt + R + 4;
  for (U32 i = tid ; i < MG_LIVE_BINS ; i += T) sLive[i] = 0;
  int *sWave = reinterpret_cast<int *> (sLive + MG_LIVE_BINS);
  unsigned short *sStart = reinterpret_cast<unsigned short *> (sWave + 32);
  U32 *sPlaced = sCnt + R;
  if (tid < 2) sPlaced[tid] = 0;
  U32 n1 = 0, n2 = 0;
  U32 nu = a.uniqCount[b];
  U32 nNew = a.sliceOff[(U64) b * (a.nSlices + 2) + a.nSlices];
  U32 occNow = a.occ[b];
  U64 lo = a.bucketStart[b];
  U64 ck[MG_MERGE_PREFETCH]; U32 co[MG_MERGE_PREFETCH], cc[MG_MERGE_PREFETCH];
#pragma unroll
  for (int j = 0 ; j < MG_MERGE_PREFETCH ; ++j)
    { const U32 i = (U32) j * T + tid; ck[j] = 0; co[j] = 0; cc[j] = 0;
      if (i < nu) { ck[j] = __builtin_nontemporal_load (&a.pK[lo + i]); co[j] = __builtin_nontemporal_load (&a.pT[lo + i]); cc[j] = __builtin_nontemporal_load (&a.pC[lo + i]); }
    }
  __syncthreads ();
  for ( ; b < bEnd ; ++b)
    { U32 nnu = 0; U64 nlo = 0; U64 nk[MG_MERGE_PREFETCH]; U32 no[MG_MERGE_PREFETCH], ncc[MG_MERGE_PREFETCH], occNext = 0, nNewNext = 0;
#pragma unroll
      for (int j = 0 ; j < MG_MERGE_PREFETCH ; ++j) { nk[j] = 0; no[j] = 0; ncc[j] = 0; }
      if (b + 1 < bEnd)
        { nnu = a.uniqCount[b + 1]; nlo = a.bucketStart[b + 1]; occNext = a.occ[b + 1];
          nNewNext = a.sliceOff[(U64) (b + 1) * (a.nSlices + 2) + a.nSlices];
#pragma unroll
          for (int j = 0 ; j < MG_MERGE_PREFETCH ; ++j)
            { const U32 i = (U32) j * T + tid;
              if (i < nnu) { nk[j] = __builtin_nontemporal_load (&a.pK[nlo + i]); no[j] = __builtin_nontemporal_load (&a.pT[nlo + i]); ncc[j] = __builtin_nontemporal_load (&a.pC[nlo + i]); }
            }
        }
      if (nu)
        {
          if (occNow)
            { for (U32 i = tid ; i < R ; i += T)
                { uint4 v = *reinterpret_cast<const uint4 *> (&a.slots[(U64) b * R + i]);
                  sKey[i] = mgKeyOf (v); sOrd[i] = v.z; sCnt[i] = v.w;
                }
              __syncthreads ();
            }
          if (!occNow && a.place && !a.slotShift)
            {
              const U32 nScan = nu < (U32) KEEP * T ? nu : (U32) KEEP * T;
              if (nu >= R) { a.counters[1] = 1; }
              else
                { U32 hr[KEEP];
#pragma unroll
                  for (int j = 0 ; j < KEEP ; ++j)
                    { const U32 i = (U32) j * T + tid;
                      hr[j] = 0;
                      if (i < nScan MG_ABLATE_AND (!(a.debug & 512)))
                        { const U64 km = j < MG_MERGE_PREFETCH ? ck[j < MG_MERGE_PREFETCH ? j : 0] : __builtin_nontemporal_load (&a.pK[lo + i]);
                          const U32 home = mgHomeOfM (km, a.g); hr[j] = (home << 16) | atomicAdd (&sOrd[home], 1u);
                        }
                    }
                  __syncthreads ();
                  U32 carry = 0;
#ifdef MG_ABLATE
                  if (a.debug & 1024) { for (U32 i = tid ; i < R ; i += T) { sStart[i] = (unsigned short) i; sOrd[i] = 0; } } else
#endif
                  carry = mgPlaceStarts (sOrd, sStart, sWave, R, T, tid, nScan);
                  if (tid == 0) { ++sPlaced[0]; if (carry) ++sPlaced[1]; }
                  __syncthreads ();
#pragma unroll
                  for (int j = 0 ; j < KEEP ; ++j)
                    { const U32 i = (U32) j * T + tid;
                      if (i < nScan MG_ABLATE_AND (!(a.debug & 2048)))
                        { U64 km; U32 ord, c;
                          if (j < MG_MERGE_PREFETCH) { km = ck[j < MG_MERGE_PREFETCH ? j : 0]; ord = co[j < MG_MERGE_PREFETCH ? j : 0]; c = cc[j < MG_MERGE_PREFETCH ? j : 0]; }
                          else { km = __builtin_nontemporal_load (&a.pK[lo + i]); ord = __builtin_nontemporal_load (&a.pT[lo + i]); c = __builtin_nontemporal_load (&a.pC[lo + i]); }
                          U32 at = (U32) sStart[hr[j] >> 16] + (hr[j] & 0xffffu);
                          if (at >= R) at -= R;
                          sKey[at] = km + 1; sOrd[at] = ord; sCnt[at] = a.withDepth ? c : 0;
                        }
                    }
                  if (nu > nScan)
                    { __syncthreads ();
                      for (U32 i = nScan + tid ; i < nu ; i += T)
                        { const U64 km = __builtin_nontemporal_load (&a.pK[lo + i]);
                          const U32 at = mgLdsClaim (sKey, R, mgHomeOfM (km, a.g), km + 1);
                          if (at == R) { a.counters[1] = 1; continue; }
                          sOrd[at] = __builtin_nontemporal_load (&a.pT[lo + i]); sCnt[at] = a.withDepth ? __builtin_nontemporal_load (&a.pC[lo + i]) : 0;
                        }
                    }
                }
            }
          else
          for (U32 i = tid, jj = 0 ; i < nu ; i += T, ++jj)
            { U64 km; U32 ord, c;
              if (jj < MG_MERGE_PREFETCH)
                { km = ck[0]; ord = co[0]; c = cc[0];
#pragma unroll
                  for (int j = 1 ; j < MG_MERGE_PREFETCH ; ++j) if (jj == (U32) j) { km = ck[j]; ord = co[j]; c = cc[j]; }
                }
              else { km = __builtin_nontemporal_load (&a.pK[lo + i]); ord = __builtin_nontemporal_load (&a.pT[lo + i]); c = __builtin_nontemporal_load (&a.pC[lo + i]); }
              if (!a.withDepth) c = 0;
              U32 at;
              if (a.slotShift)
                { at = (U32) (km >> MG_SLOT_SHIFT); km &= ((U64) 1 << MG_SLOT_SHIFT) - 1;
                  if (i < nNew) { sKey[at] = km + 1; sOrd[at] = ord; sCnt[at] = c; }
                  else if (c) sCnt[at] += c;
                  continue;
                }
#ifdef MG_ABLATE
              if (a.debug & 32) { at = mgHomeOfM (km, a.g); sKey[at] = km + 1; } else
#endif
              at = mgLdsClaim (sKey, R, mgHomeOfM (km, a.g), km + 1);
              if (at == R) { a.counters[1] = 1; continue; }
              if (i < nNew) { sOrd[at] = ord; sCnt[at] = c; }
              else if (c) atomicAdd (&sCnt[at], c);
            }
          __syncthreads ();
          for (U32 i0 = 0 ; i0 < R ; i0 += T)
            { const U32 i = i0 + tid;
              unsigned long long k = 0; U32 dep = 0;
              if (i < R)
                { k = sKey[i];
                  uint4 v; v.x = (U32) k; v.y = (U32) (k >> 32); v.z = sOrd[i]; v.w = sCnt[i];
                  { typedef unsigned v4u __attribute__ ((ext_vector_type (4)));
                    v4u vv = { v.x, v.y, v.z, v.w };
                    if (true MG_ABLATE_AND (!(a.debug & 64)))
                    __builtin_nontemporal_store (vv, reinterpret_cast<v4u *> (&a.slots[(U64) b * R + i]));
                  }
                  dep = v.w > 0xffffu ? 0xffffu : v.w;
                  if (k) { sKey[i] = 0; sOrd[i] = 0; sCnt[i] = 0; }
                }
              if (a.liveHist)
                { n1 += (U32) __popcll (__ballot (k && dep == 1));
                  n2 += (U32) __popcll (__ballot (k && dep == 2));
                  if (k && dep != 1 && dep != 2)
                    { if (dep < MG_LIVE_BINS) atomicAdd (&sLive[dep], 1u); else atomicAdd (&a.liveHist[dep], 1ull); }
                }
            }
          __syncthreads ();
          if (tid == 0 && nNew) a.occ[b] += nNew;
        }
      nu = nnu; lo = nlo; occNow = occNext; nNew = nNewNext;
#pragma unroll
      for (int j = 0 ; j < MG_MERGE_PREFETCH ; ++j) { ck[j] = nk[j]; co[j] = no[j]; cc[j] = ncc[j]; }
    }
  if (tid == 0 && sPlaced[0]) { atomicAdd ((unsigned long long *) &a.counters[4], (unsigned long long) sPlaced[0]); if (sPlaced[1]) atomicAdd ((unsigned long long *) &a.counters[5], (unsigned long long) sPlaced[1]); }
  if (a.liveHist)
    { __syncthreads ();
      if ((tid & 63) == 0) { if (n1) atomicAdd (&sLive[1], n1); if (n2) atomicAdd (&sLive[2], n2); }
      __syncthreads ();
      for (U32 i = tid ; i < MG_LIVE_BINS ; i += T) if (sLive[i]) atomicAdd (&a.liveHist[i], (unsigned long long) sLive[i]);
    }
}

#define MG_LOOKUP_UNROLL 4
__global__ __launch_bounds__ (256)
void mgRankLookupKernel (const MgBucketArgs a, U32 groupsPerSlice)
{
  MG_BUILD_PRIO ();
  const int lane = threadIdx.x & 63;
  const U32 blocksPerSlice = (groupsPerSlice + 3) / 4;
  const U32 xcd = blockIdx.x & 7, k = blockIdx.x >> 3;
  const U32 s = xcd + 8 * (k / blocksPerSlice), g = (k % blocksPerSlice) * 4 + (threadIdx.x >> 6);
  if (s >= a.nSlices || g >= groupsPerSlice) return;
  const U32 b = g * 64 + (U32) lane;
  U64 lo = 0; U32 n = 0;
  if (b < a.nBuckets)
    { const unsigned short *o = a.sliceOff + (U64) b * (a.nSlices + 2) + s;
      const U32 o0 = o[0], o1 = o[1];
      n = o1 - o0; lo = a.bucketStart[b] + o0;
    }
  auto indexOf = [&] (U32 tok, const uint4 &r) -> U32
    { const U64 bits = ((U64) r.y << 32) | r.x;
      const U64 idx = (U64) a.baseMax + 1 + r.z + (U32) __popcll (bits & (((U64) 1 << (tok & 63)) - 1));
      return idx < a.size ? ((U32) idx | MG_ASSIGNED) : 0;
    };
  for (int j = 0 ; j < 64 ; j += MG_LOOKUP_UNROLL)
    { U64 l[MG_LOOKUP_UNROLL]; U32 m[MG_LOOKUP_UNROLL], tok[MG_LOOKUP_UNROLL]; uint4 r[MG_LOOKUP_UNROLL];
#pragma unroll
      for (int u = 0 ; u < MG_LOOKUP_UNROLL ; ++u)
        { l[u] = ((U64) (U32) __shfl ((int) (U32) (lo >> 32), j + u) << 32) | (U32) __shfl ((int) (U32) lo, j + u);
          m[u] = (U32) __shfl ((int) n, j + u);
        }
#pragma unroll
      for (int u = 0 ; u < MG_LOOKUP_UNROLL ; ++u)
        { tok[u] = 0; if ((U32) lane < m[u] MG_ABLATE_AND (!(a.debug & 256))) tok[u] = 0x7fffffffu - __builtin_nontemporal_load (&a.pT[l[u] + lane]); }
#pragma unroll
      for (int u = 0 ; u < MG_LOOKUP_UNROLL ; ++u)
        { r[u] = make_uint4 (0, 0, 0, 0); if ((U32) lane < m[u] MG_ABLATE_AND (!(a.debug & 16))) r[u] = *reinterpret_cast<const uint4 *> (&a.grp[tok[u] >> 6]); }
#pragma unroll
      for (int u = 0 ; u < MG_LOOKUP_UNROLL ; ++u) asm volatile ("" : "+v" (r[u].x), "+v" (r[u].y), "+v" (r[u].z));
#pragma unroll
      for (int u = 0 ; u < MG_LOOKUP_UNROLL ; ++u)
        if ((U32) lane < m[u] MG_ABLATE_AND (!(a.debug & 128))) a.pT[l[u] + lane] = indexOf (tok[u], r[u]);
#pragma unroll
      for (int u = 0 ; u < MG_LOOKUP_UNROLL ; ++u)
        for (U32 i = 64 + (U32) lane ; i < m[u] ; i += 64)
          { const U32 t = 0x7fffffffu - __builtin_nontemporal_load (&a.pT[l[u] + i]);
            const uint4 rr = *reinterpret_cast<const uint4 *> (&a.grp[t >> 6]);
            a.pT[l[u] + i] = indexOf (t, rr);
          }
    }
}

__global__ __launch_bounds__ (256)
void mgBinFindKernel (const MgSlot *__restrict__ slots, MgGeom g, MgPartFmt f, U64 *__restrict__ el, const U64 *__restrict__ binStart,
                      U32 nBins, U32 wgPerXcd)
{
  const U32 xcd = blockIdx.x & 7, j = blockIdx.x >> 3;
  const U64 ordMask = ((U64) 1 << f.ordBits) - 1;
  for (U32 b = xcd ; b < nBins ; b += 8)
    { const U64 lo = binStart[b], hi = binStart[b + 1];
      for (U64 i = lo + (U64) j * 256 + threadIdx.x ; i < hi ; i += (U64) wgPerXcd * 256)
        { const U64 x = __builtin_nontemporal_load (&el[i]);
          const U64 m = ((U64) b << f.remBits) | (x >> f.ordBits), key = m + 1;
          const U64 base = (U64) mgBucketOfM (m, g) * g.R;
          const U32 res = mgProbeFind (MgTableSlots { slots + base }, mgHomeOfM (m, g), g.R, key);
          __builtin_nontemporal_store (((x & ordMask) << 32) | res, &el[i]);
        }
    }
}

template <int SUB, bool NT, class Decode>
__device__ __forceinline__ void mgPullTile (const unsigned long long *__restrict__ runRow, U32 nBins, const Decode &dec, U32 cnt, U32 *__restrict__ out)
{
  __shared__ U32 sTile[SUB];
  __shared__ unsigned long long sRun[MG_PART_MAXBINS];
  const U32 tid = threadIdx.x, lane = tid & 63, wave = tid >> 6;
  for (U32 b = tid ; b < nBins ; b += 1024) sRun[b] = runRow[b];
  __syncthreads ();
  for (U32 b = wave ; b < nBins ; b += 16)
    { const unsigned long long r = sRun[b];
      const U64 base = r & (((U64) 1 << 40) - 1); const U32 len = (U32) (r >> 40);
      for (U32 i = lane ; i < len ; i += 64) { U32 pos, val; dec (base + i, &pos, &val); sTile[pos] = val; }
    }
  __syncthreads ();
  for (U32 i = tid ; i < cnt ; i += 1024) { if (NT) __builtin_nontemporal_store (sTile[i], &out[i]); else out[i] = sTile[i]; }
  __syncthreads ();
}

template <int SUB>
__global__ __launch_bounds__ (1024)
void mgUnpartKernel (const U64 *__restrict__ el, const unsigned long long *__restrict__ runTab, U32 nBins, U64 n, U32 *__restrict__ out)
{
  const U64 nSub = (n + SUB - 1) / SUB;
  for (U64 s = blockIdx.x ; s < nSub ; s += gridDim.x)
    { const U64 o0 = s * SUB;
      const auto dec = [=] (U64 at, U32 *pos, U32 *val) { const U64 v = __builtin_nontemporal_load (&el[at]); *pos = (U32) ((v >> 32) - o0); *val = (U32) v; };
      mgPullTile<SUB, true> (runTab + s * nBins, nBins, dec, (U32) (o0 + SUB < n ? SUB : n - o0), out + o0);
    }
}

template <bool WORD8>
__global__ __launch_bounds__ (1024)
void mgBucketFindKernel (const MgSlot *__restrict__ slots, const U64 *__restrict__ find8, const U32 *__restrict__ occ, MgGeom g, MgPartFmt f, U32 nBuckets, int remB,
                         const U64 *__restrict__ bucketStart, U64 *__restrict__ el, U32 bucketsPerBlock)
{
// ... 380 lines not shown
          t->log2NB = lg; t->R = R; t->nSlots = (U64) R << lg;
        }
      if ((s = mgTableAllocGeom (t, st))) break;
      U64 over = 0;
      if ((s = mgRehashPass (t, o, keepMax, st, &over))) break;
      if (!over)
        { MG_HIP (hipFree (o.slots)); MG_HIP (hipFree (o.occ));
          t->empty = false; ++t->version;
          return MG_OK;
        }
      (void) hipFree (t->slots); (void) hipFree (t->occ);
      t->slots = 0; t->occ = 0; t->capSlots = 0; t->capNB = 0;
      if (attempt) { mgSetError ("internal: the device table's fitted geometry (2^%d x %u) does not hold its entries", t->log2NB, t->R); s = MG_ERR_CAPACITY; }
    }
  mgTablePutOld (t, o, st);
  return s;
}
static MgStatus mgTableRehashTo (MgTable *t, U64 want, hipStream_t st) { return mgTableRehash (t, want, false, 0, 0, 0x7fffffffu, st); }
static MgStatus mgTableRehashExact (MgTable *t, int log2NB, U32 R, hipStream_t st) { return mgTableRehash (t, (U64) R << log2NB, true, log2NB, R, 0x7fffffffu, st); }

MgStatus mgTableRollback (MgTable *t, hipStream_t st)
{
  t->liveHistValid = false;
  if (!t->slots) return MG_OK;
  return mgTableRehash (t, t->nSlots, true, t->log2NB, t->R, t->max, st);
}

MgStatus mgTableEnsure (MgTable *t, U64 nIncoming, hipStream_t st)
{
  U64 want = mgSlotsFor (t, (U64) t->max + nIncoming);
  if (t->slots && want <= t->nSlots) return MG_OK;
  if (!t->slots || !t->max) return mgTableAlloc (t, want, st);
  if (nIncoming && want < 2 * t->nSlots) want = 2 * t->nSlots;
  if (want > ((U64) 1 << t->maxLog2Slots)) want = (U64) 1 << t->maxLog2Slots;
  if (want <= t->nSlots) return MG_OK;
  return mgTableRehashTo (t, want, st);
}


#define MG_RANK_UNITS 8192
static inline U64 mgRankRowsPerUnit (U64 n, U32 *nBlocks)
{
  U64 nRows = (n + 63) / 64;
  U64 per = (nRows + MG_RANK_UNITS - 1) / MG_RANK_UNITS; if (!per) per = 1;
  U64 units = (nRows + per - 1) / per; if (!units) units = 1;
  *nBlocks = (U32) ((units + 3) / 4);
  return per;
}

static void mgHotKnobs (U32 *split, U32 *chunk)
{
  const MgKnobs *k = mgKnobs ();
  U32 a = MG_HOT_SPLIT_DEFAULT, b = MG_HOT_CHUNK_DEFAULT;
  if (k->hotSplit != MG_KNOB_UNSET && k->hotSplit > 0)
    { a = (U32) k->hotSplit; b = k->hotChunk != MG_KNOB_UNSET && k->hotChunk > 0 ? (U32) k->hotChunk : a / 4; }
  if (b < 64) b = 64;
  if (a < b) a = b;
  *split = a; *chunk = b;
}
static U64 mgHotItemsCap (U64 n) { U32 sp, ch; mgHotKnobs (&sp, &ch); return n / ch + n / sp + 16; }

size_t mgTableAddScratchBytes (const MgTable *t, U64 n)
{
  (void) t;
  U64 NB = (U64) 1 << 18;
  size_t rank = mgAl256 (n)  + 2 * mgAl256 ((MG_RANK_UNITS + 8) * 8) + mgAl256 ((n / 64 + 2) * sizeof (MgRankGrp));
  size_t direct = mgAl256 (n * 4);
  size_t part = 2 * (mgAl256 (n * 8) + mgAl256 (n * 4)) + mgAl256 (n * 4)
              + mgAl256 ((NB + 2) * 8) * 3 + mgAl256 ((NB + 2) * 4) * 2 + mgAl256 (((U64) MG_PART_MAXBINS + 2) * 8) * 3 + 2 * mgAl256 ((U64) MG_PART_MAXBINS * 16 * 8 + 4096)
              + mgAl256 ((MG_PART_MAXBINS + 2) * 4) + mgAl256 ((MG_PART_MAXBINS + 2 + n / MG_PART_CHUNK + MG_PART_MAXBINS + 2) * 4)
              + mgAl256 ((size_t) (MG_RANK_GROUPS + 2) * NB * sizeof (unsigned short)) + mgAl256 ((n / MG_PART_SUB + 2) * 24)
              + mgAl256 (mgHotItemsCap (n) * 8) + mgAl256 (mgHotItemsCap (n) * 4) + 256;
  return rank + (direct > part ? direct : part) + 4096;
}

static int mgPathOverride (void)
{
  const long c = mgKnobs ()->tablePath;
  return c == 'd' ? 1 : (c == 'b' ? 2 : 0);
}

bool mgTableUseBuckets (const MgTable *t, U64 n)
{
  int ov = mgPathOverride ();
  if (ov == 1) return false;
  if (ov == 2) return true;
  if (n < 1500000) return false;
  return n >= t->nSlots / 16;
}

bool mgTableAddTakesSegments (const MgTable *t, U64 n, const MgHistReq *counted)
{
  const int off = mgKnobs ()->noSegmentInput == 1;
  return !off && n && mgTableUseBuckets (t, n) && counted && counted->binCount && counted->log2NB == t->log2NB && counted->kbits == t->kbits && !counted->hiB;
}

struct MgPartPassArgs {
  int inMode; bool packed; MgPartFmt f;
  const U64 *kIn; const U32 *tIn; U64 n;
  const U64 *segStart; U32 nSeg;
  int shift; U32 nBins;
  U64 *kOut; U32 *tOut; U64 *binStart;
  unsigned long long *cursor; U32 *binCount, *chunkBase;
  const U32 *counted;
  const MgSegSrc *segSrc; MgSubSeg *subSeg;
  unsigned long long *runTab; int runMode;
  unsigned char *digitOut; int nextShift; U32 nextBins;
  const unsigned char *digitIn;
  U32 subElems, maxChunks;
};
static MgStatus mgPartPass (const MgTable *t, MgPartPassArgs &p, hipStream_t st)
{
  MgGeom g = mgGeomOf (t);
  MgSegSrc src = {};
  if (p.inMode == MG_EL_SEG)
    { if (!p.segSrc || !p.subSeg || !p.counted) { mgSetError ("internal: segment input needs its counts"); return MG_ERR_ARG; }
      src = *p.segSrc;
      const U64 nSub = (p.n + MG_PART_SUB - 1) / MG_PART_SUB;
      MG_LAUNCH (MG_K_PART, st, mgSubSegKernel, dim3 ((unsigned) ((nSub + 255) / 256)), dim3 (256), 0, st, src, p.n, (U32) MG_PART_SUB, p.subSeg);
    }
  if (p.counted) MG_HIP (hipMemcpy2DAsync (p.binCount, sizeof (U32), p.counted, MG_HIST_STRIDE * sizeof (U32), sizeof (U32), p.nBins, hipMemcpyDeviceToDevice, st));
  else MG_HIP (hipMemsetAsync (p.binCount, 0, (size_t) p.nSeg * p.nBins * sizeof (U32), st));
  const int bigEnv = mgKnobs ()->partBig == MG_KNOB_UNSET ? 1 : (int) mgKnobs ()->partBig;
  const bool big = bigEnv && p.packed && p.nBins <= MG_PART_BIG_BINS && MG_PART_THREADS == 1024;
  p.subElems = (U32) (big ? MG_PART_SUB_BIG : MG_PART_SUB);
  const U32 chunkElems = 2u * p.subElems;
  MG_LAUNCH (MG_K_PART, st, mgPartChunksKernel, dim3 (1), dim3 (MG_PART_MAXBINS), 0, st, p.segStart, p.nSeg, chunkElems, p.chunkBase);
  const unsigned maxChunks = p.maxChunks = (unsigned) (p.n / chunkElems + p.nSeg + 1);
  const int sgEnv = mgKnobs ()->scatterGrid == MG_KNOB_UNSET ? 0 : (int) mgKnobs ()->scatterGrid;
  unsigned scatterGrid = maxChunks < (unsigned) (sgEnv > 0 ? sgEnv : 1024) ? maxChunks : (unsigned) (sgEnv > 0 ? sgEnv : 1024);
  const dim3 hg (maxChunks < 4096 ? maxChunks : 4096), sg (scatterGrid);
  if (!p.counted && p.digitIn)
    MG_LAUNCH (MG_K_PART_HIST, st, mgPartHistBytesKernel, hg, dim3 (256), 0, st, p.digitIn, p.nBins, p.segStart, p.chunkBase, p.nSeg, chunkElems, p.binCount);
  else if (!p.counted)
    {
#define MG_HIST(IN) MG_LAUNCH (MG_K_PART_HIST, st, mgPartHistKernel<IN>, hg, dim3 (256), 0, st, p.kIn, g, p.f, p.shift, p.nBins, p.segStart, p.chunkBase, p.nSeg, chunkElems, p.binCount)
      if (p.inMode == MG_EL_DENSE) MG_HIST (MG_EL_DENSE); else if (p.inMode == MG_EL_WIDE) MG_HIST (MG_EL_WIDE); else MG_HIST (MG_EL_PACKED);
#undef MG_HIST
    }
  const U32 cstride = p.nSeg == 1 ? 16u : 1u;
  MG_LAUNCH (MG_K_PART, st, mgPartScanKernel, dim3 (p.nSeg), dim3 (MG_PART_MAXBINS), 0, st, p.binCount, p.nBins, p.segStart, p.binStart, p.cursor, cstride, p.nSeg, p.n);
#define MG_SCATTER(IN, PK, SUB) MG_LAUNCH (MG_K_PART_SCATTER, st, (mgPartScatterKernel<IN, PK, SUB>), sg, dim3 (MG_PART_THREADS), 0, st, \
                                           p.kIn, p.tIn, src, p.subSeg, g, p.f, p.shift, p.nBins, p.segStart, p.chunkBase, p.nSeg, chunkElems, p.cursor, cstride, p.kOut, p.tOut, p.runTab, p.runMode, \
                                           p.digitOut, p.nextShift, p.nextBins ? p.nextBins - 1 : 0u)
#define MG_SCATTER_P(IN) mgForSub (p.subElems, [&] (auto S) { MG_SCATTER (IN, true, decltype (S)::value); })
  if (p.inMode == MG_EL_DENSE) { if (p.packed) MG_SCATTER_P (MG_EL_DENSE); else MG_SCATTER (MG_EL_DENSE, false, MG_PART_SUB); }
  else if (p.inMode == MG_EL_SEG) { if (p.packed) MG_SCATTER_P (MG_EL_SEG); else MG_SCATTER (MG_EL_SEG, false, MG_PART_SUB); }
  else if (p.inMode == MG_EL_WIDE) MG_SCATTER (MG_EL_WIDE, false, MG_PART_SUB);
  else MG_SCATTER_P (MG_EL_PACKED);
#undef MG_SCATTER_P
#undef MG_SCATTER
  MG_HIP (hipGetLastError ());
  return MG_OK;
}

__global__ __launch_bounds__ (256)
void mgUniqStatsKernel (const U32 *__restrict__ uniqCount, U32 nBuckets, unsigned long long *__restrict__ out)
{
  unsigned long long sum = 0; U32 mx = 0;
  for (U32 b = blockIdx.x * 256 + threadIdx.x ; b < nBuckets ; b += gridDim.x * 256) { const U32 c = uniqCount[b]; sum += c; mx = c > mx ? c : mx; }
  sum = mgWaveReduce<MgSum> ((U64) sum); mx = mgWaveReduce<MgMax> (mx);
  if ((threadIdx.x & 63) == 0) { if (sum) atomicAdd (&out[0], sum); if (mx) atomicMax (&out[1], (unsigned long long) mx); }
}

#define MG_TIGHT_PCT_DEFAULT 70
#define MG_TIGHT_PCT_CLAIMS 50
#define MG_TIGHT_MIN_R 1024u

MgStatus mgTableAdd (MgTable *t, const U64 *dKmer, U64 n, int withDepth, void *scratch, hipStream_t st,
                     const MgHistReq *counted, const MgSegSrc *segSrc)
{
  if (!n) return MG_OK;
  if (segSrc && !mgTableAddTakesSegments (t, n, counted)) { mgSetError ("internal: this insert needs the dense k-mers"); return MG_ERR_ARG; }
  const MgSegSrc noSrc = {};
  t->liveHistValid = false;
  if (withDepth) t->pendingDepth = true;
  const bool wasEmpty = t->empty && t->max == 0;
  t->empty = false; ++t->version;
  MgGeom g = mgGeomOf (t);
  char *wb = (char *) scratch;
  unsigned char *flags = (unsigned char *) wb;       wb += mgAl256 (n);
  U64 *blockCount = (U64 *) wb;                      wb += mgAl256 ((MG_RANK_UNITS + 8) * 8);
  U64 *blockBase = (U64 *) wb;                       wb += mgAl256 ((MG_RANK_UNITS + 8) * 8);
  MgRankGrp *grp = (MgRankGrp *) wb;                 wb += mgAl256 ((n / 64 + 2) * sizeof (MgRankGrp));
  U32 nRankBlocks; U64 rankTiles = mgRankRowsPerUnit (n, &nRankBlocks);
  MG_HIP (hipMemsetAsync (blockCount, 0, (MG_RANK_UNITS + 8) * 8, st));

  if (!mgTableUseBuckets (t, n))
    { U32 *slotId = (U32 *) wb;
      { MgStatus cs = mgTableClean (t, st); if (cs) return cs; }
      MG_LAUNCH (MG_K_TABLE_INSERT, st, mgTableInsertKernel, dim3 (mgGridWide (n)), dim3 (256), 0, st, t->slots, g, dKmer, n, slotId, withDepth, t->counters);
      MG_LAUNCH (MG_K_TABLE_FLAG, st, mgDirectFlagKernel, dim3 (mgGridWide (n)), dim3 (256), 0, st, t->slots, slotId, n, flags);
      MG_LAUNCH (MG_K_RANK_COUNT, st, mgRankCountKernel, dim3 (nRankBlocks), dim3 (256), 0, st, flags, n, rankTiles, blockCount);
      MG_LAUNCH (MG_K_RANK_SCAN, st, (mgGroupSumKernel<U64, U64>), dim3 (1), dim3 (MG_GROUP_THREADS), 0, st, blockCount, blockBase, nRankBlocks * 4, t->counters);
      MG_LAUNCH (MG_K_TABLE_ASSIGN, st, (mgRankAssignKernel<true, false>), dim3 (nRankBlocks), dim3 (256), 0, st,
                 flags, dKmer, noSrc, (const MgSubSeg *) 0, n, rankTiles, blockBase, t->max, t->size, t->value, t->slots, slotId, grp);
      MG_HIP (hipGetLastError ());
      return mgTableMarkOccupied (t, dKmer, n, st);
    }

  const U64 NB = (U64) 1 << t->log2NB;
  U64 *kA = (U64 *) wb;  wb += mgAl256 (n * 8);
  U32 *tA = (U32 *) wb;  wb += mgAl256 (n * 4);
  U64 *kB = (U64 *) wb;  wb += mgAl256 (n * 8);
  U32 *tB = (U32 *) wb;  wb += mgAl256 (n * 4);
  U32 *cB = (U32 *) wb;  wb += mgAl256 (n * 4);
  U64 *fineStart = (U64 *) wb;                wb += mgAl256 ((NB + 2) * 8);
  unsigned long long *fineCursor = (unsigned long long *) wb; wb += mgAl256 ((NB + 2 + (U64) MG_PART_MAXBINS * 16) * 8);
  U64 *spare64 = (U64 *) wb;                  wb += mgAl256 ((NB + 2) * 8);
  U32 *fineCount = (U32 *) wb;                wb += mgAl256 ((NB + 2) * 4);
  U32 *uniqCount = (U32 *) wb;                wb += mgAl256 ((NB + 2) * 4);
  U64 *coarseStart = (U64 *) wb;              wb += mgAl256 (((U64) MG_PART_MAXBINS + 2) * 8);
  unsigned long long *coarseCursor = (unsigned long long *) wb; wb += mgAl256 (((U64) MG_PART_MAXBINS + 2) * 8 * 16);
  U64 *whole = (U64 *) wb;                    wb += mgAl256 (((U64) MG_PART_MAXBINS + 2) * 8);
  U32 *coarseCount = (U32 *) wb;              wb += mgAl256 ((MG_PART_MAXBINS + 2) * 4);
  U32 *chunkBase = (U32 *) wb;                wb += mgAl256 ((MG_PART_MAXBINS + 2 + n / MG_PART_CHUNK + MG_PART_MAXBINS + 2) * 4);
  unsigned short *sliceOff = (unsigned short *) wb;   wb += mgAl256 ((size_t) (MG_RANK_GROUPS + 2) * NB * sizeof (unsigned short));
  MgSubSeg *subSeg = (MgSubSeg *) wb;         wb += mgAl256 ((n / MG_PART_SUB + 2) * sizeof (MgSubSeg));
  U64 *hotItems = (U64 *) wb;                 wb += mgAl256 (mgHotItemsCap (n) * 8);
  U32 *hotBuckets = (U32 *) wb;               wb += mgAl256 (mgHotItemsCap (n) * 4);
  unsigned long long *hotCount = (unsigned long long *) wb; wb += 256;
  (void) spare64;

  const int j = t->log2NB;
  int hiB, loB;
  mgPartSplit (j, &hiB, &loB);
  const U32 *pre = (counted && counted->binCount && counted->log2NB == j && counted->kbits == t->kbits && !counted->hiB) ? counted->binCount : 0;
  U64 segInit[2] = { 0, n };
  MG_HIP (hipMemcpyAsync (whole, segInit, 16, hipMemcpyHostToDevice, st));
  const MgPartFmt f = mgPartFmtOf (t, n, hiB);
  const int packEnv = mgKnobs ()->partPacked == MG_KNOB_UNSET ? 1 : (int) mgKnobs ()->partPacked;
  const bool packed = packEnv && mgPartFmtFits (t, f);
  MgStatus s;
  const U64 *bucketStart = fineStart;
  MgPartPassArgs p1 = {};
  p1.inMode = segSrc ? MG_EL_SEG : MG_EL_DENSE; p1.packed = packed; p1.f = f; p1.kIn = dKmer; p1.n = n; p1.segStart = whole; p1.nSeg = 1;
  p1.nBins = (U32) 1 << hiB; p1.chunkBase = chunkBase; p1.counted = pre; p1.segSrc = segSrc; p1.subSeg = subSeg;
  if (!loB)
    { p1.kOut = kB; p1.tOut = tB; p1.binStart = fineStart; p1.cursor = fineCursor; p1.binCount = fineCount;
      if ((s = mgPartPass (t, p1, st))) return s;
    }
  else
    {
      unsigned char *digits = (loB <= 8 && mgKnobs ()->partDigits != 0) ? reinterpret_cast<unsigned char *> (cB) : 0;
      p1.shift = loB; p1.kOut = kA; p1.tOut = tA; p1.binStart = coarseStart; p1.cursor = coarseCursor; p1.binCount = coarseCount;
      p1.digitOut = digits; p1.nextBins = (U32) 1 << loB;
      if ((s = mgPartPass (t, p1, st))) return s;
      MgPartPassArgs p2 = {};
      p2.inMode = packed ? MG_EL_PACKED : MG_EL_WIDE; p2.packed = packed; p2.f = f; p2.kIn = kA; p2.tIn = tA; p2.n = n; p2.segStart = coarseStart; p2.nSeg = (U32) 1 << hiB;
      p2.nBins = (U32) 1 << loB; p2.kOut = kB; p2.tOut = tB; p2.binStart = fineStart; p2.cursor = fineCursor; p2.binCount = fineCount; p2.chunkBase = chunkBase;
      p2.digitIn = digits;
      if ((s = mgPartPass (t, p2, st))) return s;
    }

  MgBucketArgs a;
  { const int polEnv = mgKnobs ()->flagPolarity == MG_KNOB_UNSET ? -1 : (int) mgKnobs ()->flagPolarity;
    a.markDup = polEnv >= 0 ? (polEnv ? 1 : 0) : (t->newPct > 50 ? 1 : 0);
  }
  MG_HIP (hipMemsetAsync (flags, a.markDup ? 1 : 0, n, st));
  const U64 expectNew = t->newPct > 0 ? n * (U64) t->newPct / 100 : n;
  { const int slotEnv = mgKnobs ()->mergeSlots == MG_KNOB_UNSET ? -1 : (int) mgKnobs ()->mergeSlots;
    const bool dense = ((U64) t->max + expectNew) * 2 > t->nSlots;
    a.slotShift = (t->kbits <= MG_SLOT_SHIFT && (slotEnv >= 0 ? slotEnv != 0 : dense)) ? MG_SLOT_SHIFT : 0;
  }
  int tightPct = t->tightPct ? t->tightPct : MG_TIGHT_PCT_CLAIMS;
  { const long tk = mgKnobs ()->tightLoad; if (tk != MG_KNOB_UNSET && tk >= 0 && tk <= 95) tightPct = (int) tk; }
  bool tighten = wasEmpty && tightPct > 0 && t->log2NB > 0 && t->pin;
  if (tighten && mgKnobs ()->tightLoad == MG_KNOB_UNSET)
    tighten = expectNew * 100 / (U64) tightPct < t->nSlots - t->nSlots / 4;
  { const long pk = mgKnobs ()->mergePlace;
    a.place = pk == MG_KNOB_UNSET ? 1 : (pk != 0);
    if (pk == MG_KNOB_UNSET && expectNew / NB * 115 / 100 > (U64) MG_MERGE_PREFETCH * mgBucketThreads (t->R, 0)) a.place = 0;
    if (a.place && wasEmpty) a.slotShift = 0;
    if (a.place && mgKnobs ()->tightLoad == MG_KNOB_UNSET)
      { if (!t->tightPct) tightPct = MG_TIGHT_PCT_DEFAULT;
        tighten = wasEmpty && tightPct > 0 && t->log2NB > 0 && t->pin;
      }
  }
  if (tighten) a.slotShift = 0;
  a.slots = t->slots; a.g = g; a.nBuckets = (U32) NB; a.bucketStart = bucketStart;
  a.pK = kB; a.pT = tB; a.pC = cB; a.uniqCount = uniqCount; a.occ = t->occ; a.flags = flags;
  a.grp = grp; a.baseMax = t->max; a.size = t->size; a.withDepth = withDepth;
  { a.sliceShift = 22;
    while (a.sliceShift > 16 && ((n - 1) >> a.sliceShift) + 1 < 32) --a.sliceShift;
    if (mgKnobs ()->rankSliceShift != MG_KNOB_UNSET) a.sliceShift = (int) mgKnobs ()->rankSliceShift;
    while (((n - 1) >> a.sliceShift) + 1 > (U64) (MG_RANK_GROUPS - 1)) ++a.sliceShift;
    a.nSlices = (U32) (((n - 1) >> a.sliceShift) + 1);
    a.sliceOff = sliceOff;
  }
  a.counters = t->counters; a.f = f;
#ifdef MG_ABLATE
  { const long dbg = mgKnobs ()->bucketDebug; a.debug = dbg != MG_KNOB_UNSET ? (int) dbg : 0; }
#endif
  const bool track = t->max == 0 && t->baseZero;
  a.liveHist = 0;
  if (track)
    { if (!t->liveHist) MG_HIP (hipMalloc ((void **) &t->liveHist, 65536 * sizeof (U64)));
      MG_HIP (hipMemsetAsync (t->liveHist, 0, 65536 * sizeof (U64), st));
      a.liveHist = (unsigned long long *) t->liveHist;
    }
  t->liveHistValid = track;
  size_t lds = mgMergeLdsBytes (t->R);
  { const size_t ldsDedup = (size_t) t->R * 16 + MG_RANK_GROUPS * 4; if (ldsDedup > lds) lds = ldsDedup; }
  const bool bigR = t->R > MG_DEDUP_PER * 1024u;
  if (t->R > MG_DEDUP_PER_BIG * 1024u) { mgSetError ("internal: bucket of %u slots", t->R); return MG_ERR_ARG; }
  if (lds > 48 * 1024)
    {
#define MG_DEDUP_ATTR(PK, SL, PER) do { MG_HIP (hipFuncSetAttribute ((const void *) mgBucketDedupKernel<PK, SL, PER, false>, hipFuncAttributeMaxDynamicSharedMemorySize, (int) lds)); \
                                        MG_HIP (hipFuncSetAttribute ((const void *) mgBucketDedupKernel<PK, SL, PER, true>, hipFuncAttributeMaxDynamicSharedMemorySize, (int) lds)); } while (0)
      if (bigR) { MG_DEDUP_ATTR (true, true, MG_DEDUP_PER_BIG); MG_DEDUP_ATTR (true, false, MG_DEDUP_PER_BIG); MG_DEDUP_ATTR (false, true, MG_DEDUP_PER_BIG); MG_DEDUP_ATTR (false, false, MG_DEDUP_PER_BIG); }
      else      { MG_DEDUP_ATTR (true, true, MG_DEDUP_PER); MG_DEDUP_ATTR (true, false, MG_DEDUP_PER); MG_DEDUP_ATTR (false, true, MG_DEDUP_PER); MG_DEDUP_ATTR (false, false, MG_DEDUP_PER); }
#undef MG_DEDUP_ATTR
      MG_HIP (hipFuncSetAttribute ((const void *) mgBucketMergeKernel<MG_MERGE_PREFETCH>, hipFuncAttributeMaxDynamicSharedMemorySize, (int) lds));
      MG_HIP (hipFuncSetAttribute ((const void *) mgBucketMergeKernel<MG_PLACE_KEEP>, hipFuncAttributeMaxDynamicSharedMemorySize, (int) lds));
    }
  const int bThreadsEnv = mgKnobs ()->bucketT == MG_KNOB_UNSET ? 0 : (int) mgKnobs ()->bucketT;
  const unsigned bThreads = mgBucketThreads (t->R, bThreadsEnv);
  U32 perBlock;
  const unsigned bGrid = mgBucketGrid (NB, &perBlock);
  if ((U64) bThreads * (bigR ? MG_DEDUP_PER_BIG : MG_DEDUP_PER) < t->R)
    { mgSetError ("internal: %u threads for a bucket of %u slots", bThreads, t->R); return MG_ERR_ARG; }
  mgHotKnobs (&a.hotSplit, &a.hotChunk);
  a.hotItems = hotItems; a.hotCount = hotCount; a.hotBuckets = hotBuckets;
  MG_HIP (hipMemsetAsync (hotCount, 0, 16, st));
  MG_LAUNCH (MG_K_HOT_REDUCE, st, mgHotPlanKernel, dim3 ((unsigned) ((NB + 255) / 256)), dim3 (256), 0, st, a);
  { const size_t ldsHot = (size_t) t->R * 16 + 16;
    if (packed) { if (ldsHot > 48 * 1024) MG_HIP (hipFuncSetAttribute ((const void *) mgHotReduceKernel<true>, hipFuncAttributeMaxDynamicSharedMemorySize, (int) ldsHot));
                  MG_LAUNCH (MG_K_HOT_REDUCE, st, mgHotReduceKernel<true>, dim3 (1024), dim3 (bThreads), ldsHot, st, a); }
    else        { if (ldsHot > 48 * 1024) MG_HIP (hipFuncSetAttribute ((const void *) mgHotReduceKernel<false>, hipFuncAttributeMaxDynamicSharedMemorySize, (int) ldsHot));
                  MG_LAUNCH (MG_K_HOT_REDUCE, st, mgHotReduceKernel<false>, dim3 (1024), dim3 (bThreads), ldsHot, st, a); }
  }
#define MG_DEDUP_LAUNCH(PK, SL, PER) do { MG_LAUNCH (MG_K_BUCKET_DEDUP, st, (mgBucketDedupKernel<PK, SL, PER, false>), dim3 (bGrid), dim3 (bThreads), lds, st, a, perBlock); \
                                          MG_LAUNCH (MG_K_HOT_REDUCE, st, (mgBucketDedupKernel<PK, SL, PER, true>), dim3 (64), dim3 (bThreads), lds, st, a, perBlock); } while (0)
#define MG_DEDUP_PICK(PER) do { if (packed) { if (a.slotShift) MG_DEDUP_LAUNCH (true, true, PER); else MG_DEDUP_LAUNCH (true, false, PER); } \
                                else        { if (a.slotShift) MG_DEDUP_LAUNCH (false, true, PER); else MG_DEDUP_LAUNCH (false, false, PER); } } while (0)
  if (bigR) MG_DEDUP_PICK (MG_DEDUP_PER_BIG); else MG_DEDUP_PICK (MG_DEDUP_PER);
#undef MG_DEDUP_PICK
#undef MG_DEDUP_LAUNCH
  U64 fullest = t->R;
  if (tighten)
    { unsigned long long *st2 = (unsigned long long *) (t->counters + 2);
      MG_HIP (hipMemsetAsync (st2, 0, 16, st));
      MG_LAUNCH (MG_K_RANK_SCAN, st, mgUniqStatsKernel, dim3 ((unsigned) (NB / 256 < 256 ? (NB + 255) / 256 : 256)), dim3 (256), 0, st, uniqCount, (U32) NB, st2);
      MG_HIP (hipMemcpyAsync (t->pin, t->counters + 1, 24, hipMemcpyDeviceToHost, st));
      MG_HIP (hipStreamSynchronize (st));
      const U64 over = t->pin[0], U = t->pin[1], M = t->pin[2];
      if (!over)
        { fullest = M;
          U64 Rn = (U * 100 / ((U64) NB * (U64) tightPct) + 1 + MG_R_QUANTUM - 1) / MG_R_QUANTUM * MG_R_QUANTUM;
          const U64 Rfit = (M + M / 8 + 16 + MG_R_QUANTUM - 1) / MG_R_QUANTUM * MG_R_QUANTUM;
          if (Rn < Rfit) Rn = Rfit;
          if (Rn < MG_TIGHT_MIN_R) Rn = MG_TIGHT_MIN_R;
          if (Rn < t->R)
            { t->R = (U32) Rn; t->nSlots = (U64) NB * Rn; a.g = mgGeomOf (t);
              lds = mgMergeLdsBytes (t->R);
            }
        }
    }
  MG_LAUNCH (MG_K_RANK_COUNT, st, mgRankCountKernel, dim3 (nRankBlocks), dim3 (256), 0, st, flags, n, rankTiles, blockCount);
  MG_LAUNCH (MG_K_RANK_SCAN, st, (mgGroupSumKernel<U64, U64>), dim3 (1), dim3 (MG_GROUP_THREADS), 0, st, blockCount, blockBase, nRankBlocks * 4, t->counters);
  if (segSrc)
    MG_LAUNCH (MG_K_TABLE_ASSIGN, st, (mgRankAssignKernel<false, true>), dim3 (nRankBlocks), dim3 (256), 0, st,
               flags, (const U64 *) 0, *segSrc, subSeg, n, rankTiles, blockBase, t->max, t->size, t->value, t->slots, (const U32 *) 0, grp);
  else
    MG_LAUNCH (MG_K_TABLE_ASSIGN, st, (mgRankAssignKernel<false, false>), dim3 (nRankBlocks), dim3 (256), 0, st,
               flags, dKmer, noSrc, (const MgSubSeg *) 0, n, rankTiles, blockBase, t->max, t->size, t->value, t->slots, (const U32 *) 0, grp);
  { const U32 groupsPerSlice = (U32) ((NB + 63) / 64);
    const U32 blocksPerSlice = (groupsPerSlice + 3) / 4, rounds = (a.nSlices + 7) / 8;
    MG_LAUNCH (MG_K_RANK_LOOKUP, st, mgRankLookupKernel, dim3 (8 * rounds * blocksPerSlice), dim3 (256), 0, st, a, groupsPerSlice);
  }
  if (fullest <= (U64) MG_MERGE_PREFETCH * bThreads)
    MG_LAUNCH (MG_K_BUCKET_MERGE, st, mgBucketMergeKernel<MG_MERGE_PREFETCH>, dim3 (bGrid), dim3 (bThreads), lds, st, a, perBlock);
  else
    MG_LAUNCH (MG_K_BUCKET_MERGE, st, mgBucketMergeKernel<MG_PLACE_KEEP>, dim3 (bGrid), dim3 (bThreads), lds, st, a, perBlock);
  MG_HIP (hipGetLastError ());
  return MG_OK;
}

__global__ void mgMarkOccKernel (MgGeom g, const U64 *__restrict__ kmer, U64 n, U32 *__restrict__ occ)
{
  U64 o = (U64) blockIdx.x * blockDim.x + threadIdx.x;
  const U64 stride = (U64) gridDim.x * blockDim.x;
  for ( ; o < n ; o += stride)
    { U32 b = mgBucketOfM (mgMixK (kmer[o], g.kbits), g);
      if (!occ[b]) occ[b] = 1;
    }
}

MgStatus mgTableMarkOccupied (MgTable *t, const U64 *dKmer, U64 n, hipStream_t st)
{
  MG_LAUNCH (MG_K_TABLE_FLAG, st, mgMarkOccKernel, dim3 (mgGridWide (n)), dim3 (256), 0, st, mgGeomOf (t), dKmer, n, t->occ);
  MG_HIP (hipGetLastError ());
  return MG_OK;
}

MgStatus mgTableFind (MgTable *t, const U64 *dKmer, U64 n, U32 *dIndexOut, hipStream_t st)
{
  if (!n) return MG_OK;
  { MgStatus cs = mgTableClean (t, st); if (cs) return cs; }
  const unsigned fgrid = mgGridWide ((n + MG_FIND_PER - 1) / MG_FIND_PER);
  ++t->diag[MG_DIAG_FIND_DIRECT];
  MG_LAUNCH (MG_K_TABLE_FIND, st, mgTableFindKernel<false>, dim3 (fgrid), dim3 (256), 0, st, t->slots, t->occ, mgGeomOf (t), dKmer, n, dIndexOut);
  MG_HIP (hipGetLastError ());
  return MG_OK;
}

__global__ __launch_bounds__ (256)
void mgTableCheckLayoutKernel (const MgSlot *__restrict__ slots, MgGeom g, U64 nSlots, unsigned long long *__restrict__ out)
{
  const U64 stride = (U64) gridDim.x * blockDim.x;
  U32 broken = 0, stray = 0, dup = 0, keys = 0;
  for (U64 o = (U64) blockIdx.x * blockDim.x + threadIdx.x ; o < nSlots ; o += stride)
    { const uint4 v = *reinterpret_cast<const uint4 *> (&slots[o]);
      const U64 key = mgKeyOf (v);
      if (!key) continue;
      ++keys;
      const U32 bkt = (U32) (o / g.R), me = (U32) (o - (U64) bkt * g.R);
      const U64 m = key - 1;
      if (mgBucketOfM (m, g) != bkt) { ++stray; continue; }
      const U64 base = (U64) bkt * g.R;
      for (U32 at = mgHomeOfM (m, g) ; at != me ; at = mgNextSlot (at, g.R))
        { const uint4 w = *reinterpret_cast<const uint4 *> (&slots[base + at]);
          const U64 k2 = mgKeyOf (w);
          if (!k2) { ++broken; break; }
          if (k2 == key) { ++dup; break; }
        }
    }
  if (broken) atomicAdd (&out[0], (unsigned long long) broken);
  if (stray) atomicAdd (&out[1], (unsigned long long) stray);
  if (dup) atomicAdd (&out[2], (unsigned long long) dup);
  if (keys) atomicAdd (&out[3], (unsigned long long) keys);
}

MgStatus mgTableLayoutCheck (MgTable *t, U64 *dOut, hipStream_t st)
{
  { MgStatus cs = mgTableClean (t, st); if (cs) return cs; }
  MG_HIP (hipMemsetAsync (dOut, 0, 32, st));
  MG_LAUNCH (MG_K_TABLE_FIND, st, mgTableCheckLayoutKernel, dim3 (mgGridWide (t->nSlots)), dim3 (256), 0, st, t->slots, mgGeomOf (t), t->nSlots, (unsigned long long *) dOut);
  MG_HIP (hipGetLastError ());
  return MG_OK;
}

MgStatus mgTableFindSegments (MgTable *t, const MgSegSrc &src, U64 n, U32 *dIndexOut, hipStream_t st)
{
  if (!n) return MG_OK;
  { MgStatus cs = mgTableClean (t, st); if (cs) return cs; }
  const U64 nRows = (n + 63) / 64;
  U64 waves = 256ull * 4 * 8;
  if (waves > nRows) waves = nRows;
  const U64 rowsPerWave = (nRows + waves - 1) / waves;
  waves = (nRows + rowsPerWave - 1) / rowsPerWave;
  ++t->diag[MG_DIAG_FIND_DIRECT];
  MG_LAUNCH (MG_K_TABLE_FIND_SEG, st, mgTableFindSegKernel, dim3 ((unsigned) ((waves + 3) / 4)), dim3 (256), 0, st, t->slots, mgGeomOf (t), src, n, rowsPerWave, dIndexOut);
  MG_HIP (hipGetLastError ());
  return MG_OK;
}

size_t mgTableFindPartScratchBytes (U64 n)
{
  return mgAl256 ((n / MG_PART_SUB + 2) * (size_t) MG_PART_MAXBINS * 8) + mgAl256 (((U64) MG_PART_MAXBINS + 2) * 8) * 2
       + mgAl256 (((U64) MG_PART_MAXBINS + 2) * 8 * 16) + mgAl256 ((MG_PART_MAXBINS + 2) * 4)
       + mgAl256 ((MG_PART_MAXBINS + 2 + n / MG_PART_CHUNK + MG_PART_MAXBINS + 2) * 4) + mgAl256 ((n / MG_PART_SUB + 2) * sizeof (MgSubSeg)) + 4096;
}

size_t mgTableFindPart2ScratchBytes (U64 n)
{
  const U64 NB = (U64) 1 << 18;
  return mgAl256 (n * 8) + mgAl256 (n * 4) + mgAl256 ((2 * (n / (2 * (U64) MG_PART_SUB) + MG_PART_MAXBINS + 2)) * (size_t) MG_PART_MAXBINS * 8)
       + mgAl256 ((NB + 2) * 8) + mgAl256 ((NB + 2 + (U64) MG_PART_MAXBINS * 16) * 8) + mgAl256 ((NB + 2) * 4)
       + mgAl256 ((MG_PART_MAXBINS + 2 + n / MG_PART_CHUNK + MG_PART_MAXBINS + 2) * 4) + 4096;
}

int mgTableFindDigitBits (const MgTable *t)
{
  const long kb = mgKnobs ()->findBits;
  int hiB, loB; mgPartSplit (t->log2NB, &hiB, &loB);
  int bits = kb != MG_KNOB_UNSET && kb >= 3 && kb <= 9 ? (int) kb : hiB;
  if (bits > t->log2NB) bits = t->log2NB;
  return bits;
}

bool mgTableFindTakesPartition (const MgTable *t, U64 n, const MgHistReq *counted)
{
  const long kp = mgKnobs ()->findPath;
  if (kp == 'd') return false;
  if (!n || !counted || !counted->binCount || counted->log2NB != t->log2NB || counted->kbits != t->kbits) return false;
  const int hiB = counted->hiB;
  if (hiB != mgTableFindDigitBits (t)) return false;
  if (!mgPartFmtFits (t, mgPartFmtOf (t, n, hiB)) || hiB < 3) return false;
  if (t->kbits < 24 || mgKnobs ()->scanHist == 0) return false;
  if (kp == 'p' || kp == '2') return true;
  return n >= ((U64) 1 << 24) && t->nSlots >= ((U64) 1 << 24) && t->log2NB > 9;
}

MgStatus mgTableFindPartitioned (MgTable *t, const MgSegSrc &segSrc, U64 n, const MgHistReq *counted, U32 *dIndexOut, U64 *el, void *scratch, hipStream_t st,
                                 void *scratch2)
{
  if (!n) return MG_OK;
  { MgStatus cs = mgTableClean (t, st); if (cs) return cs; }
  char *wb = (char *) scratch;
  unsigned long long *runTab = (unsigned long long *) wb;    wb += mgAl256 ((n / MG_PART_SUB + 2) * (size_t) MG_PART_MAXBINS * 8);
  U64 *binStart = (U64 *) wb;                                wb += mgAl256 (((U64) MG_PART_MAXBINS + 2) * 8);
  U64 *whole = (U64 *) wb;                                   wb += mgAl256 (((U64) MG_PART_MAXBINS + 2) * 8);
  unsigned long long *cursor = (unsigned long long *) wb;    wb += mgAl256 (((U64) MG_PART_MAXBINS + 2) * 8 * 16);
  U32 *binCount = (U32 *) wb;                                wb += mgAl256 ((MG_PART_MAXBINS + 2) * 4);
  U32 *chunkBase = (U32 *) wb;                               wb += mgAl256 ((MG_PART_MAXBINS + 2 + n / MG_PART_CHUNK + MG_PART_MAXBINS + 2) * 4);
  MgSubSeg *subSeg = (MgSubSeg *) wb;                        wb += mgAl256 ((n / MG_PART_SUB + 2) * sizeof (MgSubSeg));
  const int hiB = counted->hiB, loB = t->log2NB - hiB;
  const MgPartFmt f = mgPartFmtOf (t, n, hiB);
  const U32 nBins = (U32) 1 << hiB;
  U64 segInit[2] = { 0, n };
  MG_HIP (hipMemcpyAsync (whole, segInit, 16, hipMemcpyHostToDevice, st));
  const bool twoLevels = scratch2 && loB > 0 && ((U32) 1 << loB) <= MG_PART_MAXBINS;
  unsigned char *digits = (twoLevels && loB <= 8 && mgKnobs ()->partDigits != 0) ? reinterpret_cast<unsigned char *> ((char *) scratch2 + mgAl256 (n * 8)) : 0;
  MgPartPassArgs p1 = {};
  p1.inMode = MG_EL_SEG; p1.packed = true; p1.f = f; p1.n = n; p1.segStart = whole; p1.nSeg = 1; p1.shift = loB; p1.nBins = nBins;
  p1.kOut = el; p1.binStart = binStart; p1.cursor = cursor; p1.binCount = binCount; p1.chunkBase = chunkBase;
  p1.counted = counted->binCount; p1.segSrc = &segSrc; p1.subSeg = subSeg; p1.runTab = runTab; p1.digitOut = digits; p1.nextBins = (U32) 1 << loB;
  MgStatus s = mgPartPass (t, p1, st);
  if (s) return s;
  const U32 subElems = p1.subElems;
  if (twoLevels)
    { char *w2 = (char *) scratch2;
      const U64 NB = (U64) 1 << t->log2NB;
      U64 *el2 = (U64 *) w2;                                   w2 += mgAl256 (n * 8);
      U32 *idxA = (U32 *) w2;                                  w2 += mgAl256 (n * 4);
      unsigned long long *runTab2 = (unsigned long long *) w2; w2 += mgAl256 ((2 * (n / (2 * (U64) MG_PART_SUB) + MG_PART_MAXBINS + 2)) * (size_t) MG_PART_MAXBINS * 8);
// ... 211 lines not shown
```

Before: 1241 Gbp/s.

## Pack dedup counts into spare key bits and fold uniq stats into dedup

The bucket dedup kernel now stores each k-mer's count in the unused high bits of its 64-bit key word. A separate count is written to pC only when the count saturates that field. The merge kernel masks the key and reads the inline count, so the separate count array is neither loaded nor stored in the common case. The standalone uniq-stats reduction kernel is also removed; its sum and max are accumulated inside the dedup kernel with atomics. This trades extra masking and branching, plus an escape path for large counts, for less global memory traffic and one fewer launch.

```diff
diff --git a/include/modgpu.h b/include/modgpu.h
--- a/include/modgpu.h
+++ b/include/modgpu.h
@@ -89,6 +89,7 @@
 
 MgStatus mgTableCheckLayout (Modset *ms, U64 *out6) ;
 MgStatus mgTableDiag (Modset *ms, U64 *out9) ;
+MgStatus mgTableListDiag (Modset *ms, U64 *out4) ;
 
 MgStatus modsetDepthHistogramDevice (Modset *ms, U64 *dHist65536, void *stream) ;
 
diff --git a/modimizer_amd/__init__.py b/modimizer_amd/__init__.py
--- a/modimizer_amd/__init__.py
+++ b/modimizer_amd/__init__.py
@@ -77,7 +77,7 @@
     "mgPackedWords", "mgPackHost", "mgPackDevice", "mgUnpackDevice", "mgUploadPack",
     "mgScanWorkBytes", "seqhashScanBatchDevice", "seqhashScanBatch", "seqhashMinimizerBatchDevice", "seqhashMinimizerBatch",
     "modsetAddBatchDevice", "modsetFindBatchDevice", "modsetSyncToHost", "mgXferThreadCount", "mgCopyD2HBig", "mgCopyH2DBig", "mgModsetDeviceRelease",
-    "mgModsetHostChanged", "modsetDepthHistogramDevice", "mgTableCheckLayout", "mgTableDiag", "mgAddReadsDevice", "mgQueryReadsDevice", "mgQueryReadsDeviceAsync", "mgQueryReadsDeviceWait",
+    "mgModsetHostChanged", "modsetDepthHistogramDevice", "mgTableCheckLayout", "mgTableDiag", "mgTableListDiag", "mgAddReadsDevice", "mgQueryReadsDevice", "mgQueryReadsDeviceAsync", "mgQueryReadsDeviceWait",
     "mgAddSequenceBatch", "mgDepthHistogram", "mgSynthGenome", "mgSynthReads",
     "mgInsertReadsDevice", "mgAddSequences", "mgModsetWriteText", "mgReferenceCreate", "mgReferenceDestroy",
     "mgReferenceRead", "mgQueryProcess", "mgReferenceWrite", "mgGzipOpenWrite", "mgFzOpen", "mgGzipOpenRead", "mgReferenceLoad",
@@ -208,7 +208,7 @@
     sig("modsetFindBatchDevice", i32, MS, vp, u64, vp, vp)
     sig("modsetSyncToHost", i32, MS, i32); sig("mgXferThreadCount", i32); sig("mgCopyD2HBig", i32, vp, vp, C.c_size_t); sig("mgCopyH2DBig", i32, vp, vp, C.c_size_t); sig("mgModsetDeviceRelease", i32, MS)
     sig("mgModsetHostChanged", None, MS)
-    sig("modsetDepthHistogramDevice", i32, MS, vp, vp); sig("mgTableCheckLayout", i32, MS, U64P); sig("mgTableDiag", i32, MS, U64P)
+    sig("modsetDepthHistogramDevice", i32, MS, vp, vp); sig("mgTableCheckLayout", i32, MS, U64P); sig("mgTableDiag", i32, MS, U64P); sig("mgTableListDiag", i32, MS, U64P)
     sig("mgAddReadsDevice", i32, MS, vp, u64, vp, u32, U64P, vp)
     sig("mgQueryReadsDevice", i32, MS, vp, u64, vp, u32, vp, vp, vp, u64, U64P, vp)
     sig("mgQueryReadsDeviceAsync", i32, MS, vp, u64, vp, u32, vp, vp, vp, u64, C.POINTER(vp), vp); sig("mgQueryReadsDeviceWait", i32, vp, U64P, vp)
diff --git a/modimizer_amd/csrc/mg_api.hip b/modimizer_amd/csrc/mg_api.hip
--- a/modimizer_amd/csrc/mg_api.hip
+++ b/modimizer_amd/csrc/mg_api.hip
@@ -879,6 +879,16 @@
   return MG_OK;
 }
 
+extern "C" MgStatus mgTableListDiag (Modset *ms, U64 *out4)
+{
+  memset (out4, 0, 4 * sizeof (U64));
+  MgDev *d = mgDevLookup (ms);
+  if (!d || !d->built) return MG_OK;
+  if (hipDeviceSynchronize () != hipSuccess || hipMemcpy (out4 + 2, d->t.counters + 6, 8, hipMemcpyDeviceToHost) != hipSuccess) return MG_ERR_HIP;
+  out4[0] = d->t.listAdds[0]; out4[1] = d->t.listAdds[1]; out4[3] = (U64) d->t.listCntBits;
+  return MG_OK;
+}
+
 extern "C" MgStatus modsetDepthHistogramDevice (Modset *ms, U64 *dHist, void *stream)
 {
   hipStream_t st = (hipStream_t) stream;
diff --git a/modimizer_amd/csrc/mg_common.h b/modimizer_amd/csrc/mg_common.h
--- a/modimizer_amd/csrc/mg_common.h
+++ b/modimizer_amd/csrc/mg_common.h
@@ -221,6 +221,8 @@
   int  maxLog2Slots;
   U32  wantR;
   U64  diag[7];
+  U64  listAdds[2];
+  int  listCntBits;
   int  tightPct;
 };
 MgStatus mgTableAlloc (MgTable *t, U64 slotsWanted, hipStream_t st);
diff --git a/modimizer_amd/csrc/mg_knobs.c b/modimizer_amd/csrc/mg_knobs.c
--- a/modimizer_amd/csrc/mg_knobs.c
+++ b/modimizer_amd/csrc/mg_knobs.c
@@ -29,7 +29,7 @@
   k.noSegmentInput = num ("MODGPU_NO_SEGMENT_INPUT");
   k.rankSliceShift = num ("MODGPU_RANK_SLICE_SHIFT");
   k.flagPolarity = num ("MODGPU_FLAG_POLARITY");   k.mergeSlots = num ("MODGPU_MERGE_SLOTS");
-  k.mergePlace = num ("MODGPU_MERGE_PLACE");
+  k.mergePlace = num ("MODGPU_MERGE_PLACE");       k.listCount = num ("MODGPU_LIST_COUNT");
   k.bucketR = num ("MODGPU_BUCKET_R");             k.bucketT = num ("MODGPU_BUCKET_T");
   e = getenv ("MODGPU_HOT_SPLIT");
   k.hotSplit = e && *e ? atol (e) : MG_KNOB_UNSET;
diff --git a/modimizer_amd/csrc/mg_knobs.h b/modimizer_amd/csrc/mg_knobs.h
--- a/modimizer_amd/csrc/mg_knobs.h
+++ b/modimizer_amd/csrc/mg_knobs.h
@@ -23,6 +23,7 @@
   long mergeSlots;
   long mergePlace;
   long bucketR, bucketT;
+  long listCount;
   long hotSplit, hotChunk;
   long noAvx2;
   long textHost;
diff --git a/modimizer_amd/csrc/mg_table.hip b/modimizer_amd/csrc/mg_table.hip
--- a/modimizer_amd/csrc/mg_table.hip
+++ b/modimizer_amd/csrc/mg_table.hip
@@ -738,6 +738,7 @@
   MgSlot *slots; MgGeom g; U32 nBuckets;
   const U64 *bucketStart;
   U64 *pK; U32 *pT; U32 *pC;
+  int cntShift, cntBits;
   MgPartFmt f;
   U32 *uniqCount;
   U32 *occ;
@@ -750,6 +751,7 @@
   int markDup;
   int withDepth;
   U64 *counters;
+  unsigned long long *uniqStats;
   U32 hotSplit, hotChunk;
   U64 *hotItems; unsigned long long *hotCount;
   U32 *hotBuckets;
@@ -770,6 +772,15 @@
       at = mgNextSlot (at, R);
     }
   return R;
+}
+
+__device__ __forceinline__ U32 mgListCntMax (const MgBucketArgs &a) { return a.cntBits ? (U32) ((1ull << a.cntBits) - 1) : 0u; }
+__device__ __forceinline__ U64 mgListKeyMask (const MgBucketArgs &a) { return a.cntBits ? ((U64) 1 << a.cntShift) - 1 : ~(U64) 0; }
+__device__ __forceinline__ U32 mgListCount (const MgBucketArgs &a, U64 w, U64 i)
+{
+  const U32 cMax = mgListCntMax (a);
+  const U32 c = (U32) (w >> a.cntShift) & cMax;
+  return c == cMax ? __builtin_nontemporal_load (&a.pC[i]) : c;
 }
 
 #ifndef MG_BUCKET_PREFETCH
@@ -784,6 +795,8 @@
 #define MG_PLACE_KEEP 4
 #define MG_RANK_GROUPS 64
 #define MG_SLOT_SHIFT 48
+#define MG_LIST_CNT_MIN 8
+#define MG_CTR_LIST_ESCAPES 6
 #define MG_DEDUP_PER 4
 #define MG_DEDUP_PER_BIG 8
 #define MG_LIVE_BINS 256
@@ -1018,6 +1031,9 @@
     }
   for (U32 i = tid ; i < R ; i += T) { sKey[i] = 0; sOrd[i] = 0; sCnt[i] = 0; }
   if (tid < MG_RANK_GROUPS) sGrp[tid] = 0;
+  const U32 cMax = SLOT ? 0u : mgListCntMax (a);
+  U32 uSum = 0, uMax = 0;
+  U32 nEsc = 0;
   for ( ; ; )
   {
   if (HOT) { b = a.hotBuckets[hotAt]; bEnd = b + 1; }
@@ -1085,7 +1101,7 @@
               if (rk[j])
                 { rc[j] = sCnt[i]; ro[j] = sOrd[i];
                   sKey[i] = 0; sOrd[i] = 0; sCnt[i] = 0;
-                  rk[j] = (rk[j] - 1) | (SLOT ? (unsigned long long) i << MG_SLOT_SHIFT : 0ull);
+                  rk[j] = (rk[j] - 1) | (SLOT ? (unsigned long long) i << MG_SLOT_SHIFT : (unsigned long long) (rc[j] < cMax ? rc[j] : cMax) << a.cntShift);
                   if (rc[j]) rp[j] = atomicAdd (&sGrp[mgIsAssigned (ro[j]) ? a.nSlices : ((0x7fffffffu - ro[j]) >> a.sliceShift)], 1u);
                 }
             }
@@ -1099,19 +1115,25 @@
             { if ((U32) lane <= nGrp) a.sliceOff[(U64) b * (nGrp + 1) + lane] = (unsigned short) gBase;
               if (lane == 0) a.uniqCount[b] = total;
             }
+          uSum += total; uMax = total > uMax ? total : uMax;
 #pragma unroll
           for (int j = 0 ; j < PER ; ++j)
             { const U32 grp = mgIsAssigned (ro[j]) ? a.nSlices : ((0x7fffffffu - ro[j]) >> a.sliceShift);
               const U32 at = (U32) __shfl ((int) gBase, (int) (rc[j] ? grp : 0)) + rp[j];
-              if (rc[j]) { sKey[at] = rk[j]; sOrd[at] = ro[j]; sCnt[at] = rc[j]; }
+              if (rc[j]) { sKey[at] = rk[j]; sOrd[at] = ro[j]; if (rc[j] >= cMax) sCnt[at] = rc[j]; }
             }
           __syncthreads ();
           if (tid < MG_RANK_GROUPS) sGrp[tid] = 0;
           for (U32 i = tid ; i < total ; i += T)
-            { const U64 k = sKey[i]; const U32 ord = sOrd[i], c = sCnt[i];
-              sKey[i] = 0; sOrd[i] = 0; sCnt[i] = 0;
+            { const U64 k = sKey[i]; const U32 ord = sOrd[i];
+              sKey[i] = 0; sOrd[i] = 0;
               if (true MG_ABLATE_AND (!(a.debug & 8)))
-                { __builtin_nontemporal_store (k, &a.pK[lo + i]); __builtin_nontemporal_store (ord, &a.pT[lo + i]); __builtin_nontemporal_store (c, &a.pC[lo + i]); }
+                { __builtin_nontemporal_store (k, &a.pK[lo + i]); __builtin_nontemporal_store (ord, &a.pT[lo + i]); }
+              if (((U32) (k >> a.cntShift) & cMax) == cMax)
+                { const U32 c = sCnt[i]; sCnt[i] = 0;
+                  if (true MG_ABLATE_AND (!(a.debug & 8))) __builtin_nontemporal_store (c, &a.pC[lo + i]);
+                }
+              if (cMax) nEsc += (U32) __popcll (__ballot (((U32) (k >> a.cntShift) & cMax) == cMax));
               if (!a.markDup && !mgIsAssigned (ord) MG_ABLATE_AND (!(a.debug & 1))) a.flags[0x7fffffffu - ord] = 1;
             }
           __syncthreads ();
@@ -1124,6 +1146,8 @@
   hotAt += gridDim.x;
   if (hotAt >= nHot) break;
   }
+  if (nEsc && (tid & 63) == 0) atomicAdd ((unsigned long long *) &a.counters[MG_CTR_LIST_ESCAPES], (unsigned long long) nEsc);
+  if (tid == 0 && a.uniqStats && uSum) { atomicAdd (&a.uniqStats[0], (unsigned long long) uSum); atomicMax (&a.uniqStats[1], (unsigned long long) uMax); }
 }
 
 __device__ __forceinline__ U32 mgPlaceStarts (U32 *cnt, unsigned short *sStart, int *sWave, U32 R, U32 T, U32 tid, U32 n)
@@ -1171,7 +1195,7 @@
 }
 static inline size_t mgMergeLdsBytes (U32 R) { return (size_t) R * 16 + 16 + MG_LIVE_BINS * 4 + 128 + (size_t) R * 2; }
 
-template <int KEEP>
+template <int KEEP, bool INWORD>
 __global__ __launch_bounds__ (1024) __attribute__ ((amdgpu_waves_per_eu (8)))
 void mgBucketMergeKernel (const MgBucketArgs a, U32 bucketsPerBlock)
 {
@@ -1195,11 +1219,13 @@
   U32 nNew = a.sliceOff[(U64) b * (a.nSlices + 2) + a.nSlices];
   U32 occNow = a.occ[b];
   U64 lo = a.bucketStart[b];
+  const U64 kMask = INWORD ? mgListKeyMask (a) : ~(U64) 0;
+  constexpr bool inWord = INWORD;
   U64 ck[MG_MERGE_PREFETCH]; U32 co[MG_MERGE_PREFETCH], cc[MG_MERGE_PREFETCH];
 #pragma unroll
   for (int j = 0 ; j < MG_MERGE_PREFETCH ; ++j)
     { const U32 i = (U32) j * T + tid; ck[j] = 0; co[j] = 0; cc[j] = 0;
-      if (i < nu) { ck[j] = __builtin_nontemporal_load (&a.pK[lo + i]); co[j] = __builtin_nontemporal_load (&a.pT[lo + i]); cc[j] = __builtin_nontemporal_load (&a.pC[lo + i]); }
+      if (i < nu) { ck[j] = __builtin_nontemporal_load (&a.pK[lo + i]); co[j] = __builtin_nontemporal_load (&a.pT[lo + i]); if (!inWord) cc[j] = __builtin_nontemporal_load (&a.pC[lo + i]); }
     }
   __syncthreads ();
   for ( ; b < bEnd ; ++b)
@@ -1212,7 +1238,7 @@
 #pragma unroll
           for (int j = 0 ; j < MG_MERGE_PREFETCH ; ++j)
             { const U32 i = (U32) j * T + tid;
-              if (i < nnu) { nk[j] = __builtin_nontemporal_load (&a.pK[nlo + i]); no[j] = __builtin_nontemporal_load (&a.pT[nlo + i]); ncc[j] = __builtin_nontemporal_load (&a.pC[nlo + i]); }
+              if (i < nnu) { nk[j] = __builtin_nontemporal_load (&a.pK[nlo + i]); no[j] = __builtin_nontemporal_load (&a.pT[nlo + i]); if (!inWord) ncc[j] = __builtin_nontemporal_load (&a.pC[nlo + i]); }
             }
         }
       if (nu)
@@ -1235,7 +1261,7 @@
                     { const U32 i = (U32) j * T + tid;
                       hr[j] = 0;
                       if (i < nScan MG_ABLATE_AND (!(a.debug & 512)))
-                        { const U64 km = j < MG_MERGE_PREFETCH ? ck[j < MG_MERGE_PREFETCH ? j : 0] : __builtin_nontemporal_load (&a.pK[lo + i]);
+                        { const U64 km = (j < MG_MERGE_PREFETCH ? ck[j < MG_MERGE_PREFETCH ? j : 0] : __builtin_nontemporal_load (&a.pK[lo + i])) & kMask;
                           const U32 home = mgHomeOfM (km, a.g); hr[j] = (home << 16) | atomicAdd (&sOrd[home], 1u);
                         }
                     }
@@ -1252,20 +1278,20 @@
                     { const U32 i = (U32) j * T + tid;
                       if (i < nScan MG_ABLATE_AND (!(a.debug & 2048)))
                         { U64 km; U32 ord, c;
-                          if (j < MG_MERGE_PREFETCH) { km = ck[j < MG_MERGE_PREFETCH ? j : 0]; ord = co[j < MG_MERGE_PREFETCH ? j : 0]; c = cc[j < MG_MERGE_PREFETCH ? j : 0]; }
-                          else { km = __builtin_nontemporal_load (&a.pK[lo + i]); ord = __builtin_nontemporal_load (&a.pT[lo + i]); c = __builtin_nontemporal_load (&a.pC[lo + i]); }
+                          if (j < MG_MERGE_PREFETCH) { km = ck[j < MG_MERGE_PREFETCH ? j : 0]; ord = co[j < MG_MERGE_PREFETCH ? j : 0]; c = inWord ? (INWORD ? mgListCount (a, km, lo + i) : __builtin_nontemporal_load (&a.pC[lo + i])) : cc[j < MG_MERGE_PREFETCH ? j : 0]; }
+                          else { km = __builtin_nontemporal_load (&a.pK[lo + i]); ord = __builtin_nontemporal_load (&a.pT[lo + i]); c = (INWORD ? mgListCount (a, km, lo + i) : __builtin_nontemporal_load (&a.pC[lo + i])); }
                           U32 at = (U32) sStart[hr[j] >> 16] + (hr[j] & 0xffffu);
                           if (at >= R) at -= R;
-                          sKey[at] = km + 1; sOrd[at] = ord; sCnt[at] = a.withDepth ? c : 0;
+                          sKey[at] = (km & kMask) + 1; sOrd[at] = ord; sCnt[at] = a.withDepth ? c : 0;
                         }
                     }
                   if (nu > nScan)
                     { __syncthreads ();
                       for (U32 i = nScan + tid ; i < nu ; i += T)
-                        { const U64 km = __builtin_nontemporal_load (&a.pK[lo + i]);
+                        { const U64 w = __builtin_nontemporal_load (&a.pK[lo + i]), km = w & kMask;
                           const U32 at = mgLdsClaim (sKey, R, mgHomeOfM (km, a.g), km + 1);
                           if (at == R) { a.counters[1] = 1; continue; }
-                          sOrd[at] = __builtin_nontemporal_load (&a.pT[lo + i]); sCnt[at] = a.withDepth ? __builtin_nontemporal_load (&a.pC[lo + i]) : 0;
+                          sOrd[at] = __builtin_nontemporal_load (&a.pT[lo + i]); sCnt[at] = a.withDepth ? (INWORD ? mgListCount (a, w, lo + i) : __builtin_nontemporal_load (&a.pC[lo + i])) : 0;
                         }
                     }
                 }
@@ -1277,12 +1303,14 @@
                 { km = ck[0]; ord = co[0]; c = cc[0];
 #pragma unroll
                   for (int j = 1 ; j < MG_MERGE_PREFETCH ; ++j) if (jj == (U32) j) { km = ck[j]; ord = co[j]; c = cc[j]; }
+                  if (inWord) c = (INWORD ? mgListCount (a, km, lo + i) : __builtin_nontemporal_load (&a.pC[lo + i]));
                 }
-              else { km = __builtin_nontemporal_load (&a.pK[lo + i]); ord = __builtin_nontemporal_load (&a.pT[lo + i]); c = __builtin_nontemporal_load (&a.pC[lo + i]); }
+              else { km = __builtin_nontemporal_load (&a.pK[lo + i]); ord = __builtin_nontemporal_load (&a.pT[lo + i]); c = (INWORD ? mgListCount (a, km, lo + i) : __builtin_nontemporal_load (&a.pC[lo + i])); }
               if (!a.withDepth) c = 0;
+              km &= kMask;
               U32 at;
               if (a.slotShift)
-                { at = (U32) (km >> MG_SLOT_SHIFT); km &= ((U64) 1 << MG_SLOT_SHIFT) - 1;
+                { at = (U32) (km >> a.slotShift); km &= ((U64) 1 << a.slotShift) - 1;
                   if (i < nNew) { sKey[at] = km + 1; sOrd[at] = ord; sCnt[at] = c; }
                   else if (c) sCnt[at] += c;
                   continue;
@@ -1969,15 +1997,6 @@
 #undef MG_SCATTER
   MG_HIP (hipGetLastError ());
   return MG_OK;
-}
-
-__global__ __launch_bounds__ (256)
-void mgUniqStatsKernel (const U32 *__restrict__ uniqCount, U32 nBuckets, unsigned long long *__restrict__ out)
-{
-  unsigned long long sum = 0; U32 mx = 0;
-  for (U32 b = blockIdx.x * 256 + threadIdx.x ; b < nBuckets ; b += gridDim.x * 256) { const U32 c = uniqCount[b]; sum += c; mx = c > mx ? c : mx; }
-  sum = mgWaveReduce<MgSum> ((U64) sum); mx = mgWaveReduce<MgMax> (mx);
-  if ((threadIdx.x & 63) == 0) { if (sum) atomicAdd (&out[0], sum); if (mx) atomicMax (&out[1], (unsigned long long) mx); }
 }
 
 #define MG_TIGHT_PCT_DEFAULT 70
@@ -2095,6 +2114,16 @@
       }
   }
   if (tighten) a.slotShift = 0;
+  { const int room = a.slotShift ? 0 : (64 - t->kbits > 32 ? 32 : 64 - t->kbits);
+    const long lc = mgKnobs ()->listCount;
+    a.cntShift = t->kbits; a.cntBits = room >= MG_LIST_CNT_MIN ? room : 0;
+    if (lc == 0) a.cntBits = 0;
+    else if (lc >= 2 && lc <= 32) a.cntBits = room >= 2 ? (int) (lc < room ? lc : room) : 0;
+    if (!a.cntBits) a.cntShift = 0;
+    ++t->listAdds[a.cntBits ? 0 : 1]; t->listCntBits = a.cntBits;
+  }
+  a.uniqStats = tighten ? (unsigned long long *) (t->counters + 2) : 0;
+  if (tighten) MG_HIP (hipMemsetAsync (t->counters + 2, 0, 16, st));
   a.slots = t->slots; a.g = g; a.nBuckets = (U32) NB; a.bucketStart = bucketStart;
   a.pK = kB; a.pT = tB; a.pC = cB; a.uniqCount = uniqCount; a.occ = t->occ; a.flags = flags;
   a.grp = grp; a.baseMax = t->max; a.size = t->size; a.withDepth = withDepth;
@@ -2128,8 +2157,10 @@
       if (bigR) { MG_DEDUP_ATTR (true, true, MG_DEDUP_PER_BIG); MG_DEDUP_ATTR (true, false, MG_DEDUP_PER_BIG); MG_DEDUP_ATTR (false, true, MG_DEDUP_PER_BIG); MG_DEDUP_ATTR (false, false, MG_DEDUP_PER_BIG); }
       else      { MG_DEDUP_ATTR (true, true, MG_DEDUP_PER); MG_DEDUP_ATTR (true, false, MG_DEDUP_PER); MG_DEDUP_ATTR (false, true, MG_DEDUP_PER); MG_DEDUP_ATTR (false, false, MG_DEDUP_PER); }
 #undef MG_DEDUP_ATTR
-      MG_HIP (hipFuncSetAttribute ((const void *) mgBucketMergeKernel<MG_MERGE_PREFETCH>, hipFuncAttributeMaxDynamicSharedMemorySize, (int) lds));
-      MG_HIP (hipFuncSetAttribute ((const void *) mgBucketMergeKernel<MG_PLACE_KEEP>, hipFuncAttributeMaxDynamicSharedMemorySize, (int) lds));
+      MG_HIP (hipFuncSetAttribute ((const void *) mgBucketMergeKernel<MG_MERGE_PREFETCH, true>, hipFuncAttributeMaxDynamicSharedMemorySize, (int) lds));
+      MG_HIP (hipFuncSetAttribute ((const void *) mgBucketMergeKernel<MG_PLACE_KEEP, true>, hipFuncAttributeMaxDynamicSharedMemorySize, (int) lds));
+      MG_HIP (hipFuncSetAttribute ((const void *) mgBucketMergeKernel<MG_MERGE_PREFETCH, false>, hipFuncAttributeMaxDynamicSharedMemorySize, (int) lds));
+      MG_HIP (hipFuncSetAttribute ((const void *) mgBucketMergeKernel<MG_PLACE_KEEP, false>, hipFuncAttributeMaxDynamicSharedMemorySize, (int) lds));
     }
   const int bThreadsEnv = mgKnobs ()->bucketT == MG_KNOB_UNSET ? 0 : (int) mgKnobs ()->bucketT;
   const unsigned bThreads = mgBucketThreads (t->R, bThreadsEnv);
@@ -2156,9 +2187,7 @@
 #undef MG_DEDUP_LAUNCH
   U64 fullest = t->R;
   if (tighten)
-    { unsigned long long *st2 = (unsigned long long *) (t->counters + 2);
-      MG_HIP (hipMemsetAsync (st2, 0, 16, st));
-      MG_LAUNCH (MG_K_RANK_SCAN, st, mgUniqStatsKernel, dim3 ((unsigned) (NB / 256 < 256 ? (NB + 255) / 256 : 256)), dim3 (256), 0, st, uniqCount, (U32) NB, st2);
+    {
       MG_HIP (hipMemcpyAsync (t->pin, t->counters + 1, 24, hipMemcpyDeviceToHost, st));
       MG_HIP (hipStreamSynchronize (st));
       const U64 over = t->pin[0], U = t->pin[1], M = t->pin[2];
@@ -2186,10 +2215,10 @@
     const U32 blocksPerSlice = (groupsPerSlice + 3) / 4, rounds = (a.nSlices + 7) / 8;
     MG_LAUNCH (MG_K_RANK_LOOKUP, st, mgRankLookupKernel, dim3 (8 * rounds * blocksPerSlice), dim3 (256), 0, st, a, groupsPerSlice);
   }
-  if (fullest <= (U64) MG_MERGE_PREFETCH * bThreads)
-    MG_LAUNCH (MG_K_BUCKET_MERGE, st, mgBucketMergeKernel<MG_MERGE_PREFETCH>, dim3 (bGrid), dim3 (bThreads), lds, st, a, perBlock);
-  else
-    MG_LAUNCH (MG_K_BUCKET_MERGE, st, mgBucketMergeKernel<MG_PLACE_KEEP>, dim3 (bGrid), dim3 (bThreads), lds, st, a, perBlock);
+#define MG_MERGE_LAUNCH(KEEP) do { if (a.cntBits) MG_LAUNCH (MG_K_BUCKET_MERGE, st, (mgBucketMergeKernel<KEEP, true>), dim3 (bGrid), dim3 (bThreads), lds, st, a, perBlock); \
+                                   else           MG_LAUNCH (MG_K_BUCKET_MERGE, st, (mgBucketMergeKernel<KEEP, false>), dim3 (bGrid), dim3 (bThreads), lds, st, a, perBlock); } while (0)
+  if (fullest <= (U64) MG_MERGE_PREFETCH * bThreads) MG_MERGE_LAUNCH (MG_MERGE_PREFETCH); else MG_MERGE_LAUNCH (MG_PLACE_KEEP);
+#undef MG_MERGE_LAUNCH
   MG_HIP (hipGetLastError ());
   return MG_OK;
 }
```

Result: no change. 1248 Gbp/s, median of 6 (+0.6%).
